# JoelTankard/web-rwkv-gguf

Hardware: AMD Instinct MI355X
Metric: tokens/sec RWKV-7 1.5B Q4_K_M decode @1 GPU; achieved HBM GB/s vs roofline (higher is better)
Workload: dtype f16; 1 GPU; RWKV-7 World 1.5B Q4_K_M (Q4_K matrices, Q6_K head, F16 LoRA) batch=1 greedy decode, fused kernels under hipGraph; decode_engine=on, streams_per_gpu=1, pipelines_per_gpu=1, streams=1, parallelism=single

## Files before the change

### include/wrk_hip.h

```cpp
#ifndef WRK_HIP_H
#define WRK_HIP_H

#include <stddef.h>
#include <stdint.h>

#ifdef __cplusplus
extern "C" {
#endif

#define WRK_ABI_VERSION 1

typedef struct wrk_ctx wrk_ctx;
typedef struct wrk_buf wrk_buf;
typedef struct wrk_matrix wrk_matrix;
typedef struct wrk_program wrk_program;
typedef struct wrk_v7_model wrk_v7_model;
typedef struct wrk_v7_state wrk_v7_state;

enum {
    WRK_OK = 0,
    WRK_E_ARG = 1,
    WRK_E_OOM = 2,
    WRK_E_HIP = 3,
    WRK_E_UNSUPPORTED = 4
// ... 90 lines not shown
int32_t wrk_op_activate(wrk_ctx* ctx, const wrk_tensor* x, uint32_t act);
int32_t wrk_op_control_k_v7(wrk_ctx* ctx, const wrk_buf* p, const wrk_tensor* a, const wrk_tensor* k);
int32_t wrk_op_time_mix_v7(wrk_ctx* ctx, const wrk_buf* cursors, const wrk_tensor* state, const wrk_tensor* r,
                           const wrk_tensor* w, const wrk_tensor* n, const wrk_tensor* x);
int32_t wrk_op_time_first_v7(wrk_ctx* ctx, const wrk_buf* u, const wrk_tensor* r, const wrk_tensor* n, const wrk_tensor* x);
int32_t wrk_op_channel_mix_v7(wrk_ctx* ctx, const wrk_buf* cursors, const wrk_tensor* state, const wrk_tensor* v, const wrk_tensor* x);
int32_t wrk_op_softmax(wrk_ctx* ctx, const wrk_tensor* x);


typedef struct wrk_v7_layer_desc {
    const wrk_buf *ln1_w, *ln1_b, *ln2_w, *ln2_b;
    const wrk_buf *x_r, *x_w, *x_k, *x_v, *x_a, *x_g;
    const wrk_buf *w0, *a0, *v0;
    const wrk_matrix *w1, *w2, *a1, *a2, *g1, *g2, *v1, *v2;
    const wrk_buf *r_k, *k_k, *k_a;
    const wrk_matrix *w_k, *w_v, *w_r, *w_o;
    const wrk_buf *gn_w, *gn_b;
    const wrk_buf* ffn_x_k;
    const wrk_matrix *ffn_w_k, *ffn_w_v;
} wrk_v7_layer_desc;

typedef struct wrk_v7_model_desc {
    uint32_t num_layer, num_emb, num_hidden, num_vocab, num_head;
    uint32_t lora_w, lora_a, lora_g, lora_v;
    uint32_t rescale;
    const wrk_buf *ln0_w, *ln0_b, *ln_out_w, *ln_out_b;
    const wrk_buf* emb_f16;
    const wrk_matrix* head;
    const wrk_v7_layer_desc* layers;
} wrk_v7_model_desc;

int32_t wrk_v7_model_create(wrk_ctx* ctx, const wrk_v7_model_desc* desc, wrk_v7_model** out);
int32_t wrk_v7_model_destroy(wrk_v7_model* model);
size_t wrk_v7_model_token_bytes(const wrk_v7_model* model, uint32_t num_batch);

int32_t wrk_v7_state_create(wrk_ctx* ctx, const wrk_v7_model* model, uint32_t num_batch, wrk_v7_state** out);
int32_t wrk_v7_state_destroy(wrk_v7_state* state);
int32_t wrk_v7_state_load(wrk_ctx* ctx, wrk_v7_state* state, uint32_t batch, const float* src);
int32_t wrk_v7_state_back(wrk_ctx* ctx, const wrk_v7_state* state, uint32_t batch, float* dst);
int32_t wrk_v7_state_read(wrk_ctx* ctx, const wrk_v7_state* state, uint32_t batch, wrk_buf* buf);
int32_t wrk_v7_state_write(wrk_ctx* ctx, wrk_v7_state* state, uint32_t batch, const wrk_buf* buf);

int32_t wrk_v7_infer(wrk_ctx* ctx, wrk_v7_model* model, wrk_v7_state* state,
                     const uint32_t* tokens, const uint16_t* emb_rows, const uint32_t* cursors, uint32_t num_token,
                     const uint32_t* headers, uint32_t num_header, float* logits, uint32_t* argmax, uint32_t mode);

int32_t wrk_v7_model_set_frame_dtype(wrk_ctx* ctx, wrk_v7_model* model, uint32_t dtype);

int32_t wrk_v7_model_engine_status(wrk_ctx* ctx, wrk_v7_model* model, char* why, size_t capacity);

int32_t wrk_v7_infer_layer(wrk_ctx* ctx, wrk_v7_model* model, wrk_v7_state* state, uint32_t layer, const void* x, const void* v_first,
                           const uint32_t* cursors, uint32_t num_token, uint32_t mode);
int32_t wrk_v7_frame_read(wrk_ctx* ctx, wrk_v7_model* model, const char* name, uint32_t num_token, void* dst, size_t capacity, size_t* bytes);

int32_t wrk_v7_generate_greedy(wrk_ctx* ctx, wrk_v7_model* model, wrk_v7_state* state,
                               const uint32_t* first_tokens, uint32_t num_batch, uint32_t steps,
                               uint32_t* out_tokens, float* last_logits_or_null, float* elapsed_ms_or_null, uint32_t mode);

int32_t wrk_sample_logits(wrk_ctx* ctx, const wrk_buf* logits, uint32_t num_vocab, uint32_t row_stride, uint32_t num_rows,
                          const float* temperature, const float* top_p, const uint32_t* seed, uint32_t step, uint32_t* out_tokens);
int32_t wrk_v7_generate_sample(wrk_ctx* ctx, wrk_v7_model* model, wrk_v7_state* state, const uint32_t* first_tokens, uint32_t num_batch,
                               uint32_t steps, const float* temperature, const float* top_p, const uint32_t* seed,
                               uint32_t* out_tokens, float* last_logits_or_null, float* elapsed_ms_or_null, uint32_t mode);
int32_t wrk_sample_logits_filtered(wrk_ctx* ctx, const wrk_buf* logits, uint32_t num_vocab, uint32_t row_stride, uint32_t num_rows,
                                   const float* temperature, const float* top_p, const uint32_t* top_k, const float* min_p,
                                   const uint32_t* seed, uint32_t step, uint32_t* out_tokens);
int32_t wrk_sample_logits_mirostat(wrk_ctx* ctx, const wrk_buf* logits, uint32_t num_vocab, uint32_t row_stride, uint32_t num_rows,
                                   const float* temperature, const float* top_p, const float* tau, const float* eta, float* mu_inout,
                                   const uint32_t* seed, uint32_t step, uint32_t* out_tokens);
int32_t wrk_sample_logits_typical(wrk_ctx* ctx, const wrk_buf* logits, uint32_t num_vocab, uint32_t row_stride, uint32_t num_rows,
                                  const float* temperature, const float* top_p, const float* typical_p, const uint32_t* seed,
                                  uint32_t step, uint32_t* out_tokens);

int32_t wrk_score_logits(wrk_ctx* ctx, const wrk_buf* logits, uint32_t num_vocab, uint32_t row_stride, uint32_t num_rows,
                         const uint32_t* targets, float* logprob, uint32_t* rank);
#define WRK_MAX_TOP_LOGPROBS 20
int32_t wrk_top_logprobs(wrk_ctx* ctx, const wrk_buf* logits, uint32_t num_vocab, uint32_t row_stride, uint32_t num_rows,
                         const uint32_t* tokens, uint32_t num_top, float* logprob, uint32_t* top_ids, float* top_logprobs);
int32_t wrk_v7_score(wrk_ctx* ctx, wrk_v7_model* model, wrk_v7_state* state,
                     const uint32_t* tokens, const uint16_t* emb_rows, const uint32_t* cursors, uint32_t num_token,
                     const uint32_t* headers, uint32_t num_header, const uint32_t* targets, float* logprob, uint32_t* rank, uint32_t mode);

typedef struct wrk_occurrence wrk_occurrence;
int32_t wrk_occurrence_create(wrk_ctx* ctx, uint32_t num_batch, uint32_t num_vocab, wrk_occurrence** out);
int32_t wrk_occurrence_destroy(wrk_occurrence* occ);
int32_t wrk_occurrence_set_weights(wrk_ctx* ctx, wrk_occurrence* occ, const float* weights);
int32_t wrk_occurrence_ban(wrk_ctx* ctx, wrk_occurrence* occ, uint32_t batch, const uint32_t* tokens, uint32_t n, int32_t banned);
int32_t wrk_occurrence_add(wrk_ctx* ctx, wrk_occurrence* occ, uint32_t batch, const uint32_t* tokens, uint32_t n, float decay);
int32_t wrk_occurrence_back(wrk_ctx* ctx, const wrk_occurrence* occ, uint32_t batch, float* counts, uint32_t* flags);
int32_t wrk_occurrence_load(wrk_ctx* ctx, wrk_occurrence* occ, uint32_t batch, const float* counts, const uint32_t* flags);
int32_t wrk_penalize_logits(wrk_ctx* ctx, wrk_buf* logits, uint32_t num_vocab, uint32_t row_stride, uint32_t num_rows,
                            const wrk_occurrence* occ, uint32_t first_batch, const float* presence, const float* frequency);
int32_t wrk_v7_generate_penalized(wrk_ctx* ctx, wrk_v7_model* model, wrk_v7_state* state, const uint32_t* first_tokens, uint32_t num_batch,
                                  uint32_t steps, const float* temperature, const float* top_p, const uint32_t* seed, const float* presence,
                                  const float* frequency, const float* decay, wrk_occurrence* occ, uint32_t* out_tokens,
                                  float* last_logits_or_null, float* elapsed_ms_or_null, uint32_t mode);

#define WRK_GRAMMAR_REJECT 0xFFFFu
#define WRK_MAX_TOKEN_CLASSES 8192
typedef struct wrk_grammar wrk_grammar;
int32_t wrk_grammar_create(wrk_ctx* ctx, uint32_t num_vocab, uint32_t num_states, uint32_t num_classes, const uint16_t* token_class,
                           const uint16_t* transitions, wrk_grammar** out);
int32_t wrk_grammar_destroy(wrk_grammar* grammar);
int32_t wrk_constrain_logits(wrk_ctx* ctx, wrk_buf* logits, uint32_t num_vocab, uint32_t row_stride, uint32_t num_rows,
                             const wrk_grammar* grammar, const uint32_t* states);
int32_t wrk_grammar_advance(wrk_ctx* ctx, const wrk_grammar* grammar, uint32_t* states, const uint32_t* tokens, uint32_t num_rows);
// ... 211 lines not shown
```

### web-rwkv-gguf_amd/csrc/wrk_device.h

```cpp
#pragma once
#include <hip/hip_runtime.h>
#include <stdint.h>

#include "wrk_internal.h"

typedef _Float16 f16;
typedef _Float16 f16x2 __attribute__((ext_vector_type(2)));
typedef _Float16 f16x8 __attribute__((ext_vector_type(8)));
typedef uint32_t u32x4 __attribute__((ext_vector_type(4)));
typedef uint32_t u32x2 __attribute__((ext_vector_type(2)));
typedef float f32x4 __attribute__((ext_vector_type(4)));
typedef float f32x2 __attribute__((ext_vector_type(2)));

#define WAVE 64

__device__ __forceinline__ float r16(float x) { return (float)(f16)x; }

__device__ __forceinline__ size_t dt_index(const DTensor& d, uint32_t c, uint32_t t, uint32_t b) {
    return ((size_t)(b + d.offset[2]) * d.stride[1] + (t + d.offset[1])) * d.stride[0] + c + d.offset[0];
}
__device__ __forceinline__ size_t dt_index4(const DTensor& d, uint32_t c, uint32_t t, uint32_t b, uint32_t w) {
    return (((size_t)(w + d.offset[3]) * d.stride[2] + (b + d.offset[2])) * d.stride[1] + (t + d.offset[1])) * d.stride[0] + c + d.offset[0];
}
__device__ __forceinline__ float dt_load(const DTensor& d, size_t i) {
// ... 6 lines not shown

struct Cursor { uint32_t batch, token, len; };
__device__ __forceinline__ Cursor unpack_cursor(uint32_t x) {
    Cursor c; c.batch = x & 0xffu; c.token = (x >> 8) & 0xffffu; c.len = (x >> 24) & 0xffu; return c;
}

__device__ __forceinline__ float act_sigmoid(float x) { return 1.0f / (1.0f + __expf(-x)); }
__device__ __forceinline__ float act_apply(uint32_t act, float x) {
    switch (act) {
        case WRK_ACT_SQUARED_RELU: { float p = fmaxf(x, 0.0f); return p * p; }
        case WRK_ACT_TANH: return x > 42.0f ? 1.0f : tanhf(x);
        case WRK_ACT_STABLE_EXP: return __expf(-__expf(x));
        case WRK_ACT_OPPOSITE_EXP: return -__expf(x);
        case WRK_ACT_SOFTPLUS: return __logf(1.0f + __expf(x));
        case WRK_ACT_SIGMOID: return act_sigmoid(x);
        case WRK_ACT_SILU: return x / (1.0f + __expf(-x));
        default: return x;
    }
}
__device__ __forceinline__ float wgsl_mix(float x, float y, float a) { return x * (1.0f - a) + y * a; }

template <int CTRL>
__device__ __forceinline__ float dpp_f32(float v) {
    return __builtin_bit_cast(float, __builtin_amdgcn_update_dpp(0, __builtin_bit_cast(int, v), CTRL, 0xf, 0xf, true));
}
__device__ __forceinline__ float wave_sum(float v) {
    v += dpp_f32<0xB1>(v);
    v += dpp_f32<0x4E>(v);
    v += dpp_f32<0x141>(v);
    v += dpp_f32<0x140>(v);
    const int b = __builtin_bit_cast(int, v);
    const float r0 = __builtin_bit_cast(float, __builtin_amdgcn_readlane(b, 0)), r1 = __builtin_bit_cast(float, __builtin_amdgcn_readlane(b, 16));
    const float r2 = __builtin_bit_cast(float, __builtin_amdgcn_readlane(b, 32)), r3 = __builtin_bit_cast(float, __builtin_amdgcn_readlane(b, 48));
    return (r0 + r1) + (r2 + r3);
}
__device__ __forceinline__ float wave_max(float v) {
#pragma unroll
    for (int o = 32; o > 0; o >>= 1) v = fmaxf(v, __shfl_xor(v, o, WAVE));
    return v;
}
template <int NW>
__device__ __forceinline__ float block_sum(float v, float* red) {
    v = wave_sum(v);
    const int wave = threadIdx.x >> 6, lane = threadIdx.x & 63;
    __syncthreads();
    if (lane == 0) red[wave] = v;
    __syncthreads();
    float t = 0.0f;
#pragma unroll
    for (int i = 0; i < NW; ++i) t += red[i];
    return t;
}

#ifdef WRK_TIMING_BUILD
#define WRK_STAMP(p, k)                                                                                       \
    do {                                                                                                      \
        __builtin_amdgcn_sched_barrier(0);                           \
        if ((p) && threadIdx.x == 0 && (blockIdx.x == 0 || blockIdx.x == gridDim.x - 1))                      \
            (p)[(blockIdx.x ? 8 : 0) + (k)] = wall_clock64();                                                 \
        __builtin_amdgcn_sched_barrier(0);                                                                    \
    } while (0)
#else
#define WRK_STAMP(p, k) do { } while (0)
#endif
```

### web-rwkv-gguf_amd/csrc/wrk_dmv.hip

```cpp
#include <cstdlib>

#include "wrk_dmv_body.h"

namespace wrk {

template <int KA, int KB, int XI, int KS>
static dmv_fn pick_dmv_pro(bool r16, int pro) {
#define DMV_P(PRO_) (r16 ? (dmv_fn)dmv_kernel<KA, KB, true, XI, KS, PRO_, 1> : (dmv_fn)dmv_kernel<KA, KB, false, XI, KS, PRO_, 1>)
    if (KS == 4 || pro == 0) return DMV_P(0);
    if (pro == 1) return DMV_P(1);
    if (pro == 2) return DMV_P(2);
    if (KA != KB) return nullptr;
    return pro == 3 ? DMV_P(3) : DMV_P(4);
#undef DMV_P
}

template <int XI, int KS>
static dmv_fn pick_dmv_kind(int ka, bool has_f16, bool r16, int pro) {
#define DMV_K(A)                                                                              \
    if (ka == A) return (has_f16 && KS == 1) ? pick_dmv_pro<A, WRK_MAT_F16, XI, KS>(r16, pro) : pick_dmv_pro<A, A, XI, KS>(r16, pro);
    DMV_K(WRK_MAT_Q4_K)
    DMV_K(WRK_MAT_Q5_K)
    DMV_K(WRK_MAT_Q6_K)
    DMV_K(WRK_MAT_Q8_0)
    DMV_K(WRK_MAT_INT8)
#undef DMV_K
    if (ka == WRK_MAT_F16) return pick_dmv_pro<WRK_MAT_F16, WRK_MAT_F16, XI, KS>(false, pro);
    return nullptr;
}

dmvt_fn pick_dmv_nt2(int ka, int quant2, bool has_f16, bool f16_only, uint32_t xi, int ks, int pro);
dmvt_fn pick_dmv_nt4(int ka, int quant2, bool has_f16, bool f16_only, uint32_t xi, int ks, int pro);
dmvt_fn pick_dmv_tokens(int nt, int ka, int quant2, bool has_f16, bool f16_only, uint32_t xi, int ks, int pro) {
    if (nt == 2) return pick_dmv_nt2(ka, quant2, has_f16, f16_only, xi, ks, pro);
    if (nt == 4) return pick_dmv_nt4(ka, quant2, has_f16, f16_only, xi, ks, pro);
    return nullptr;
}

int launch_dmv(hipStream_t s, const MatvecParams& P, uint32_t total_wg, int quant, bool has_f16, bool r16, bool dry, int quant2) {
    static const bool enabled = [] { const char* e = getenv("WRK_DMV"); return !(e && e[0] == '0'); }();
    if (!enabled) return -1;
    DParams D;
    DParamsT DT;
    uint32_t bounds[7], bmask = 0, xi = 1;
    int pro = -1;
    bool small_wg = true;
    for (int j = 0; j < 7; ++j) bounds[j] = 0xffffffffu;
    auto dense_base = [](const DTensor& t) { return ((size_t)t.offset[2] * t.stride[1] + t.offset[1]) * t.stride[0] + t.offset[0]; };
    auto dense_stack = [](const DTensor& t) { return t.shape[2] == 1 || (t.shape[1] == t.stride[1] && t.offset[1] == 0); };
    const uint32_t ntok = P.jobs[0].in.shape[1] * P.jobs[0].in.shape[2];
    if (ntok == 0 || ntok > 4) return -1;
    const int nt = ntok == 1 ? 1 : (ntok <= 2 ? 2 : 4);
    static const uint32_t max_tok = [] { const char* e = getenv("WRK_DMV_TOKENS"); const int v = e ? atoi(e) : 4; return (uint32_t)(v < 1 ? 1 : v); }();
    if (ntok > max_tok) return -1;
    if (nt > 1 && r16) return -1;
    for (int j = 0; j < P.njobs; ++j) {
        const JobDev& J = P.jobs[j];
        if (J.in.dtype != WRK_F16 || (J.k & 7u) || J.in.shape[1] * J.in.shape[2] != ntok || J.kind == WRK_MAT_NF4) return -1;
        if (nt > 1) {
            if (!dense_stack(J.in) || !dense_stack(J.out) || (J.has_res && !dense_stack(J.res)) || (J.in.stride[0] & 7u)) return -1;
            if (J.kind != WRK_MAT_F16 && J.kind != WRK_MAT_Q4_K && J.kind != WRK_MAT_Q5_K && J.kind != WRK_MAT_Q6_K) return -1;
        }
        if ((J.out.dtype != WRK_F16 && J.out.dtype != WRK_F32) || J.m == 0 || J.rows_per_wg == 0) return -1;
        const size_t ib = dense_base(J.in);
        if (ib & 7u) return -1;
        const int jp = J.pro ? (J.k <= 2048 ? 1 : (J.k <= 4096 ? 2 : 9)) + (J.pro == 2 ? 2 : 0) : 0;
        if (jp >= 9 || (pro >= 0 && jp != pro)) return -1;
        if (J.pro == 2 && (J.k & 63u)) return -1;
        pro = jp;
        if (J.rows_per_wg > 32) small_wg = false;
        const uint32_t kpad = (J.k + 15u) & ~15u;
        uint32_t nch, need;
        if (J.kind == WRK_MAT_F16) { nch = kpad >> 3; need = quant < 0 ? (nch + 63) / 64 : (nch + 255) / 256; bmask |= (quant < 0 ? 0u : 1u << j); }
        else { nch = (J.kind == WRK_MAT_Q8_0 || J.kind == WRK_MAT_INT8) ? (J.k >> 4) : (J.k >> 8) * 8; need = (nch + 63) / 64; }
        xi = need > xi ? need : xi;
        const size_t esz = J.out.dtype == WRK_F32 ? 4 : 2;
        if (J.has_res && J.res.dtype != WRK_F16 && J.res.dtype != WRK_F32) return -1;
        auto fill = [&](auto& d) {
            memset(&d, 0, sizeof d);
            d.w = J.w;
            d.x = (const f16*)J.in.p + ib;
            d.out = (char*)J.out.p + dense_base(J.out) * esz;
            d.flags = J.out.dtype == WRK_F32 ? DJ_OUT32 : 0u;
            if (J.has_res) {
                d.res = (const char*)J.res.p + dense_base(J.res) * (J.res.dtype == WRK_F32 ? 4 : 2);
                d.flags |= DJ_RES | (J.res.dtype == WRK_F32 ? DJ_RES32 : 0u);
            }
            if (J.carry_dst) { d.carry_src = J.carry_src; d.carry_dst = J.carry_dst; d.flags |= DJ_CARRY; }
            if (J.gate) { d.gate = J.gate; d.flags |= DJ_GATE; }
            if (J.amax_val) { d.amax_val = J.amax_val; d.amax_idx = J.amax_idx; d.flags |= DJ_AMAX; }
            if (J.pro) { d.ln_w = J.ln_w; d.ln_b = J.ln_b; d.mixw = J.mixw; d.prev = J.prev; d.ln_out = J.ln_out; d.eps = J.pro_eps; if (J.ln_out) d.flags |= DJ_PUBLISH; }
            d.dbg = J.dbg;
            d.k = J.k; d.m = J.m; d.row_bytes = J.row_bytes; d.rows_per_wg = J.rows_per_wg; d.wg_begin = J.wg_begin; d.act = J.act; d.kind = J.kind;
            d.scale = J.scale;
        };
        if (nt == 1) fill(D.jobs[j]);
        else {
            DJobT& dt = DT.jobs[j];
            fill(dt);
            dt.ntok = ntok; dt.xs = J.in.stride[0]; dt.os = J.out.stride[0]; dt.rs = J.has_res ? J.res.stride[0] : 0;
            dt.mix_s = J.tok_mix_stride; dt.prev_s = J.tok_prev_stride; dt.csrc_s = J.tok_carry_src_stride; dt.cdst_s = J.tok_carry_dst_stride; dt.gate_s = J.tok_gate_stride;
        }
        if (j > 0) bounds[j - 1] = J.wg_begin;
    }
    if (xi > 8) return -1;
    static const size_t max_bytes = [] { const char* e = getenv("WRK_DMV_MAXMB"); return (size_t)(e ? atoi(e) : 24) << 20; }();
    size_t launch_bytes = 0;
    for (int j = 0; j < P.njobs; ++j) launch_bytes += (size_t)P.jobs[j].m * P.jobs[j].row_bytes;
    if (nt == 1 && launch_bytes > max_bytes && xi > 1 && pro != 3 && pro != 4) return -1;
    dmv_fn fn = nullptr;
    const int ka = quant < 0 ? WRK_MAT_F16 : quant;
    const bool mixf = has_f16 && quant >= 0;
    if (nt > 1) {
        int ks = 1;
        uint32_t xk = xi;
        if (quant2 < 0 && !(quant < 0 && xi <= 4) && xi > 2) {
            bool amax = false;
            for (int j = 0; j < P.njobs; ++j) amax = amax || P.jobs[j].amax_val;
            if (mixf || !small_wg || pro != 0 || amax || xi > 8) return -1;
            ks = 4; xk = xi <= 4 ? 1 : 2;
        }
        const dmvt_fn ft = pick_dmv_tokens(nt, ka, quant2, mixf, quant < 0, xk, ks, pro);
        if (!ft) return -1;
        if (!dry) hipLaunchKernelGGL(ft, dim3(total_wg, 1), dim3(256), 0, s, bounds[0], bounds[1], bounds[2], bounds[3], bounds[4], bounds[5], bounds[6], bmask, DT);
        return 0;
    }
    else if (quant2 >= 0) {
        const int k4 = quant == WRK_MAT_Q6_K ? quant2 : quant;
        const int lnpro = xi == 1 ? 1 : 2;
        if ((quant != WRK_MAT_Q6_K && quant2 != WRK_MAT_Q6_K) || (k4 != WRK_MAT_Q4_K && k4 != WRK_MAT_Q5_K) || xi > 2 || (pro != 0 && pro != lnpro)) return -1;
#define DMV3X(A, X, PR) (r16 ? (dmv_fn)dmv3_kernel<A, true, X, PR, 1> : (dmv_fn)dmv3_kernel<A, false, X, PR, 1>)
#define DMV3(A) (xi == 1 ? (pro ? DMV3X(A, 1, 1) : DMV3X(A, 1, 0)) : (pro ? DMV3X(A, 2, 2) : DMV3X(A, 2, 0)))
        fn = k4 == WRK_MAT_Q4_K ? DMV3(WRK_MAT_Q4_K) : DMV3(WRK_MAT_Q5_K);
#undef DMV3
#undef DMV3X
    }
    else if (xi == 1) fn = pick_dmv_kind<1, 1>(ka, mixf, r16, pro);
    else if (xi == 2) fn = pick_dmv_kind<2, 1>(ka, mixf, r16, pro);
    else if (quant < 0 && xi <= 4) fn = pick_dmv_kind<4, 1>(ka, false, false, pro);
    else if (!mixf && small_wg && pro == 0) fn = xi <= 4 ? pick_dmv_kind<1, 4>(ka, false, r16, 0) : pick_dmv_kind<2, 4>(ka, false, r16, 0);
    if (!fn) return -1;
    if (!dry) hipLaunchKernelGGL(fn, dim3(total_wg, 1), dim3(256), 0, s, bounds[0], bounds[1], bounds[2], bounds[3], bounds[4], bounds[5], bounds[6], bmask, D);
    return 0;
}

}
```

### web-rwkv-gguf_amd/csrc/wrk_dmv_body.h

```cpp
#pragma once
#include "wrk_matvec_dev.h"

namespace wrk {

enum { DJ_RES = 1, DJ_RES32 = 2, DJ_CARRY = 4, DJ_GATE = 8, DJ_AMAX = 16, DJ_OUT32 = 32, DJ_PUBLISH = 64 };

#define WRK_DJOB_FIELDS                                                                                                          \
    const uint8_t* w;                                                                                                            \
    const f16* x;                                                                    \
    void* out;                                                       \
    const void* res;                                         \
    const f16* carry_src;                                \
    float* carry_dst;                                                                                                            \
    const f16* gate;                                                                       \
    const f16 *ln_w, *ln_b, *mixw;         \
    const float* prev;                                                                                 \
    f16* ln_out;                                      \
    float* amax_val;                                                                             \
    uint32_t* amax_idx;                                                                                                          \
    unsigned long long* dbg;                                                                                                     \
    uint32_t k, m, row_bytes, rows_per_wg, wg_begin, act, flags, kind;                                                           \
    float scale, eps;
struct DJob {
    WRK_DJOB_FIELDS
};
struct DJobT {
    WRK_DJOB_FIELDS
    uint32_t ntok, xs, os, rs, mix_s, prev_s, csrc_s, cdst_s, gate_s;
};

struct DParams {
    DJob jobs[MAX_JOBS];
};
struct DParamsT {
    DJobT jobs[MAX_JOBS];
};
template <int NT> struct DParamsOf { typedef DParamsT type; };
template <> struct DParamsOf<1> { typedef DParams type; };

template <class JT> struct TokF {
    static __device__ __forceinline__ uint32_t ntok(const JT&) { return 1u; }
    static __device__ __forceinline__ uint32_t xs(const JT&) { return 0u; }
    static __device__ __forceinline__ uint32_t os(const JT&) { return 0u; }
    static __device__ __forceinline__ uint32_t rs(const JT&) { return 0u; }
    static __device__ __forceinline__ uint32_t mix_s(const JT&) { return 0u; }
    static __device__ __forceinline__ uint32_t prev_s(const JT&) { return 0u; }
    static __device__ __forceinline__ uint32_t csrc_s(const JT&) { return 0u; }
    static __device__ __forceinline__ uint32_t cdst_s(const JT&) { return 0u; }
    static __device__ __forceinline__ uint32_t gate_s(const JT&) { return 0u; }
};
template <> struct TokF<DJobT> {
    static __device__ __forceinline__ uint32_t ntok(const DJobT& j) { return j.ntok; }
    static __device__ __forceinline__ uint32_t xs(const DJobT& j) { return j.xs; }
    static __device__ __forceinline__ uint32_t os(const DJobT& j) { return j.os; }
    static __device__ __forceinline__ uint32_t rs(const DJobT& j) { return j.rs; }
    static __device__ __forceinline__ uint32_t mix_s(const DJobT& j) { return j.mix_s; }
    static __device__ __forceinline__ uint32_t prev_s(const DJobT& j) { return j.prev_s; }
    static __device__ __forceinline__ uint32_t csrc_s(const DJobT& j) { return j.csrc_s; }
    static __device__ __forceinline__ uint32_t cdst_s(const DJobT& j) { return j.cdst_s; }
    static __device__ __forceinline__ uint32_t gate_s(const DJobT& j) { return j.gate_s; }
};

template <int KIND, bool R16, int NT, int XI>
__device__ __forceinline__ void dot_raw_tokens(const Raw& r, uint32_t c, const XRegs (&x)[NT][XI], int ci, float (&acc)[NT]) {
    if (KIND == WRK_MAT_F16) {
        const f16x8 wv = __builtin_bit_cast(f16x8, r.w);
#pragma unroll
        for (int t = 0; t < NT; ++t) {
            const f16x8 xv = x[t][ci].v[0];
            float a = 0.0f;
            a = __builtin_amdgcn_fdot2(__builtin_shufflevector(wv, wv, 0, 1), __builtin_shufflevector(xv, xv, 0, 1), a, false);
            a = __builtin_amdgcn_fdot2(__builtin_shufflevector(wv, wv, 2, 3), __builtin_shufflevector(xv, xv, 2, 3), a, false);
            a = __builtin_amdgcn_fdot2(__builtin_shufflevector(wv, wv, 4, 5), __builtin_shufflevector(xv, xv, 4, 5), a, false);
            a = __builtin_amdgcn_fdot2(__builtin_shufflevector(wv, wv, 6, 7), __builtin_shufflevector(xv, xv, 6, 7), a, false);
            acc[t] += a;
        }
        return;
    }
    constexpr bool TWO = KIND != WRK_MAT_Q8_0 && KIND != WRK_MAT_INT8;
    Group lo, hi;
    decode_raw<KIND>(r, c, lo, hi);
    if (R16) { round_group(lo); if (TWO) round_group(hi); }
#pragma unroll
    for (int t = 0; t < NT; ++t) {
        const XRegs& X = x[t][ci];
        float a;
        if (R16) a = dot16r(lo.q, X.v[0], X.v[1]);
        else a = lo.scale * (lo.qmul * dot16r(lo.q, X.v[0], X.v[1]) - lo.off * X.s[0]) - lo.minv * X.s[0];
        if (TWO) {
            if (R16) a += dot16r(hi.q, X.v[2], X.v[3]);
            else a += hi.scale * (hi.qmul * dot16r(hi.q, X.v[2], X.v[3]) - hi.off * X.s[1]) - hi.minv * X.s[1];
        }
        acc[t] += a;
    }
}

template <int KIND, bool R16, int XI, int KS, int PRO, int NT, class JT>
__device__ __forceinline__ void dmv_body(const JT J, unsigned char* smem) {
    typedef TokF<JT> TF;
    constexpr int RB = 4;
    constexpr uint32_t CSTEP = KS == 1 ? 64u : 256u;
    const uint32_t K = J.k, kpad = (K + 15u) & ~15u;
    const uint32_t tid = threadIdx.x, lane = tid & 63;
    const uint32_t wave = (uint32_t)__builtin_amdgcn_readfirstlane((int)(tid >> 6));
    const uint32_t r0 = (blockIdx.x - J.wg_begin) * J.rows_per_wg;
    const uint32_t r1 = min(r0 + J.rows_per_wg, J.m);
    const uint32_t nch = num_chunks<KIND>(K, kpad);
    const uint32_t nrows = KS == 1 ? (r0 + wave < r1 ? (r1 - r0 - wave + 3) >> 2 : 0) : (r1 - r0);
    const uint32_t cbase = KS == 1 ? lane : lane + 64 * wave;
    const uint32_t ntok = NT == 1 ? 1u : TF::ntok(J);
    auto row_of = [&](uint32_t ri) { return KS == 1 ? r0 + wave + 4 * ri : r0 + ri; };
    auto tok_of = [&](uint32_t t) { return NT == 1 ? 0u : min(t, ntok - 1); };
    const uint8_t* __restrict__ W = J.w;
    const uint32_t RBY = J.row_bytes;
    float* part = (float*)smem;
    float* sv = (float*)(smem + 512 * NT);
    uint32_t* si = (uint32_t*)(smem + 528 * NT);
    float* red = (float*)(smem + 544 * NT);
    f16* xs = (f16*)(smem + 576 * NT);

    Raw raw[RB][XI];
    auto issue = [&](uint32_t ri0) {
#pragma unroll
        for (int rb = 0; rb < RB; ++rb) {
            const uint32_t rr = min(row_of(ri0 + rb), r1 - 1);
            const uint32_t phase = KIND == WRK_MAT_INT8 ? (uint32_t)((((size_t)rr * K) >> 4) & 7u) : 0u;
            const uint8_t* rowp = W + (size_t)rr * RBY;
#pragma unroll
            for (int ci = 0; ci < XI; ++ci) raw[rb][ci] = load_raw<KIND>(rowp, K, min(cbase + CSTEP * ci, nch - 1), phase);
        }
    };
    WRK_STAMP(J.dbg, 0);

    const f16* __restrict__ xin = J.x;
    const uint32_t fin_row = min(KS == 1 ? row_of(lane & 3u) : r0 + (tid & 31u), r1 - 1);
    const uint32_t fin_t = NT == 1 ? 0u : (KS == 1 ? (lane >> 2) : (tid >> 5));
    const uint32_t fin_tok = tok_of(fin_t);
    const uint32_t fl = J.flags;
    uint32_t res_bits = 0, carry_bits = 0, gate_bits = 0;
    constexpr int VPT = PRO == 0 ? 1 : ((PRO - 1) % 2 + 1);
    constexpr bool GN = PRO >= 3;
    f16x8 xv[NT][VPT], wv[VPT], bv[VPT], mv[GN ? NT : 1][VPT];
    f32x4 pv[NT][VPT][2];
    f16 c0h[NT];
    XRegs x[NT][XI];
    if (PRO > 0) {
        const uint32_t nvec = K >> 3;
#pragma unroll
        for (int v = 0; v < VPT; ++v) {
            const uint32_t i = min(tid + 256u * v, nvec - 1);
            wv[v] = *(const f16x8*)(J.ln_w + i * 8);
            bv[v] = *(const f16x8*)(J.ln_b + i * 8);
#pragma unroll
            for (int t = 0; t < NT; ++t) {
                const uint32_t tt = tok_of(t);
                xv[t][v] = *(const f16x8*)(xin + (size_t)tt * TF::xs(J) + i * 8);
                if (GN || t == 0) mv[GN ? t : 0][v] = *(const f16x8*)(J.mixw + (size_t)tt * TF::mix_s(J) + i * 8);
                pv[t][v][0] = *(const f32x4*)(J.prev + (size_t)tt * TF::prev_s(J) + i * 8);
                pv[t][v][1] = *(const f32x4*)(J.prev + (size_t)tt * TF::prev_s(J) + i * 8 + 4);
            }
        }
        if (!GN) {
#pragma unroll
            for (int t = 0; t < NT; ++t) c0h[t] = xin[(size_t)tok_of(t) * TF::xs(J)];
        }
    } else {
#pragma unroll
        for (int t = 0; t < NT; ++t)
#pragma unroll
            for (int ci = 0; ci < XI; ++ci) x[t][ci] = load_x<KIND>(xin + (size_t)tok_of(t) * TF::xs(J), min(cbase + CSTEP * ci, nch - 1), true);
    }
    issue(0);
    {
        const bool has_res = (fl & DJ_RES) != 0, has_carry = (fl & DJ_CARRY) != 0, has_gate = (fl & DJ_GATE) != 0;
        const uint16_t* rp = has_res ? (const uint16_t*)J.res : (const uint16_t*)xin;
        const uint32_t re = fin_tok * TF::rs(J) + fin_row;
        const uint32_t ri = has_res ? ((fl & DJ_RES32) ? 2u * re : re) : 0u;
        if (fl & DJ_RES32) res_bits = *(const uint32_t*)(rp + ri);
        else res_bits = rp[ri];
        carry_bits = (has_carry ? (const uint16_t*)J.carry_src : (const uint16_t*)xin)[has_carry ? fin_tok * TF::csrc_s(J) + fin_row : 0u];
        gate_bits = (has_gate ? (const uint16_t*)J.gate : (const uint16_t*)xin)[has_gate ? fin_tok * TF::gate_s(J) + fin_row : 0u];
    }

    if (GN) {
        const uint32_t nvec = K >> 3;
#pragma unroll
        for (int t = 0; t < NT; ++t)
#pragma unroll
            for (int v = 0; v < VPT; ++v) {
                float y[8], s1 = 0.0f;
#pragma unroll
                for (int e = 0; e < 8; ++e) { y[e] = (float)xv[t][v][e]; s1 += y[e]; }
                s1 += dpp_f32<0xB1>(s1); s1 += dpp_f32<0x4E>(s1); s1 += dpp_f32<0x141>(s1);
                const float mean = s1 * (1.0f / 64.0f);
                float s2 = 0.0f;
#pragma unroll
                for (int e = 0; e < 8; ++e) { y[e] -= mean; s2 = __builtin_fmaf(y[e], y[e], s2); }
                s2 += dpp_f32<0xB1>(s2); s2 += dpp_f32<0x4E>(s2); s2 += dpp_f32<0x141>(s2);
                const float dev = 1.0f / sqrtf(s2 * (1.0f / 64.0f) + J.eps);
                f16x8 o;
#pragma unroll
                for (int e = 0; e < 8; ++e) {
                    float u = r16(__builtin_fmaf(y[e] * dev, (float)wv[v][e], (float)bv[v][e]));
                    u = r16(u + pv[t][v][e >> 2][e & 3]);
                    o[e] = (f16)((float)mv[GN ? t : 0][v][e] * u);
                }
                const uint32_t i = tid + 256u * v;
                if (i < nvec) *(f16x8*)(xs + (size_t)t * kpad + i * 8) = o;
            }
        for (uint32_t i = K + tid; i < kpad; i += 256)
#pragma unroll
            for (int t = 0; t < NT; ++t) xs[(size_t)t * kpad + i] = (f16)0.0f;
        __syncthreads();
#pragma unroll
        for (int t = 0; t < NT; ++t)
#pragma unroll
            for (int ci = 0; ci < XI; ++ci) x[t][ci] = load_x<KIND>(xs + (size_t)t * kpad, min(cbase + CSTEP * ci, nch - 1), true);
    }
    if (PRO > 0 && !GN) {
        const uint32_t nvec = K >> 3;
        float s1[NT], s2[NT];
#pragma unroll
        for (int t = 0; t < NT; ++t) {
            const float c0 = (float)c0h[t];
            s1[t] = 0.0f; s2[t] = 0.0f;
#pragma unroll
            for (int v = 0; v < VPT; ++v)
                if (tid + 256u * v < nvec)
#pragma unroll
                    for (int e = 0; e < 8; ++e) { const float dl = (float)xv[t][v][e] - c0; s1[t] += dl; s2[t] = __builtin_fmaf(dl, dl, s2[t]); }
            s1[t] = wave_sum(s1[t]);
            s2[t] = wave_sum(s2[t]);
            if (lane == 0) { red[8 * t + wave] = s1[t]; red[8 * t + 4 + wave] = s2[t]; }
        }
        __syncthreads();
        WRK_STAMP(J.dbg, 4);
        const bool publish = (fl & DJ_PUBLISH) && blockIdx.x == J.wg_begin;
#pragma unroll
        for (int t = 0; t < NT; ++t) {
            const float c0 = (float)c0h[t];
            const float a1 = (red[8 * t + 0] + red[8 * t + 1]) + (red[8 * t + 2] + red[8 * t + 3]);
            const float a2 = (red[8 * t + 4] + red[8 * t + 5]) + (red[8 * t + 6] + red[8 * t + 7]);
            const float md = a1 / (float)K;
            const float mean = c0 + md;
            const float dev = 1.0f / sqrtf(fmaxf(a2 / (float)K - md * md, 0.0f) + J.eps);
#pragma unroll
            for (int v = 0; v < VPT; ++v) {
                const uint32_t i = tid + 256u * v;
                if (i >= nvec) continue;
                f16x8 yv, o;
#pragma unroll
                for (int e = 0; e < 8; ++e) {
                    yv[e] = (f16)__builtin_fmaf(((float)xv[t][v][e] - mean) * dev, (float)wv[v][e], (float)bv[v][e]);
                    o[e] = (f16)wgsl_mix((float)yv[e], pv[t][v][e >> 2][e & 3], (float)mv[0][v][e]);
                }
                *(f16x8*)(xs + (size_t)t * kpad + i * 8) = o;
                if (publish && (uint32_t)t < ntok) *(f16x8*)(J.ln_out + (size_t)t * K + i * 8) = yv;
            }
        }
        for (uint32_t i = K + tid; i < kpad; i += 256)
#pragma unroll
            for (int t = 0; t < NT; ++t) xs[(size_t)t * kpad + i] = (f16)0.0f;
        __syncthreads();
#pragma unroll
        for (int t = 0; t < NT; ++t)
#pragma unroll
            for (int ci = 0; ci < XI; ++ci) x[t][ci] = load_x<KIND>(xs + (size_t)t * kpad, min(cbase + CSTEP * ci, nch - 1), true);
    }
#pragma unroll
    for (int ci = 0; ci < XI; ++ci)
        if (cbase + CSTEP * ci >= nch) {
            const f16x8 z = {0, 0, 0, 0, 0, 0, 0, 0};
// ... 31 lines not shown
#pragma unroll
            for (int t = 0; t < NT; ++t) acc[rb][t] = 0.0f;
#pragma unroll
            for (int ci = 0; ci < XI; ++ci) dot_raw_tokens<KIND, R16, NT, XI>(raw[rb][ci], min(cbase + CSTEP * ci, nch - 1), x, ci, acc[rb]);
        }
        WRK_STAMP(J.dbg, 2);
        float mine_v = 0.0f;
#pragma unroll
        for (int t = 0; t < NT; ++t)
#pragma unroll
            for (int rb = 0; rb < RB; ++rb) {
                const float v = wave_sum(acc[rb][t]);
                if (lane == (uint32_t)(rb + RB * t)) mine_v = v;
            }
        const uint32_t frb = lane & 3u;
        if (KS == 1) {
            if (lane < (uint32_t)(RB * NT) && (NT == 1 || fin_t < ntok) && ri0 + frb < nrows) {
                const uint32_t r = row_of(ri0 + frb);
                uint32_t rbits = res_bits, cbits = carry_bits, gbits = gate_bits;
                if (ri0 != 0) operand_bits(r, fin_t, rbits, cbits, gbits);
                finish(r, fin_t, mine_v, rbits, cbits, gbits);
            }
        } else if (lane < (uint32_t)(RB * NT) && ri0 + frb < nrows) part[(((NT == 1 ? 0u : lane >> 2) * 32u) + ri0 + frb) * 4 + wave] = mine_v;
    }
    if (KS == 4) {
        __syncthreads();
        const uint32_t ri = tid & 31u;
        if (NT == 1 ? tid < nrows : (ri < nrows && fin_t < ntok)) {
            const uint32_t p = NT == 1 ? tid : (fin_t * 32u + ri);
            finish(r0 + ri, fin_t, (part[p * 4] + part[p * 4 + 1]) + (part[p * 4 + 2] + part[p * 4 + 3]), res_bits, carry_bits, gate_bits);
        }
    }
    WRK_STAMP(J.dbg, 3);
    if (fl & DJ_AMAX) {
#pragma unroll
        for (int o = (KS == 1 ? 2 : 32); o > 0; o >>= 1) {
            const float ov = __shfl_xor(best_v, o, WAVE);
            const uint32_t oi = __shfl_xor(best_i, o, WAVE);
            if (ov > best_v || (ov == best_v && oi < best_i)) { best_v = ov; best_i = oi; }
        }
        if (KS == 1 ? ((lane & 3u) == 0 && lane < 4u * NT) : lane == 0) { sv[4 * (KS == 1 ? lane >> 2 : 0) + wave] = best_v; si[4 * (KS == 1 ? lane >> 2 : 0) + wave] = best_i; }
        __syncthreads();
        if (tid < ntok) {
            float bv2 = sv[4 * tid];
            uint32_t bi = si[4 * tid];
            for (int w = 1; w < 4; ++w)
                if (sv[4 * tid + w] > bv2 || (sv[4 * tid + w] == bv2 && si[4 * tid + w] < bi)) { bv2 = sv[4 * tid + w]; bi = si[4 * tid + w]; }
            J.amax_val[(size_t)(blockIdx.x - J.wg_begin) * ntok + tid] = bv2;
            J.amax_idx[(size_t)(blockIdx.x - J.wg_begin) * ntok + tid] = bi;
        }
    }
}

template <int PRO, int NT>
constexpr unsigned dmv_smem_bytes() { return 576u * NT + (PRO > 0 ? (unsigned)((PRO - 1) % 2 + 1) * 4096u * NT : 16u); }

template <int KA, int KB, bool R16, int XI, int KS, int PRO, int NT>
__global__ void __launch_bounds__(256) dmv_kernel(uint32_t b1, uint32_t b2, uint32_t b3, uint32_t b4, uint32_t b5, uint32_t b6, uint32_t b7,
                                                  uint32_t kind_b_mask, const typename DParamsOf<NT>::type P) {
    __shared__ __attribute__((aligned(16))) unsigned char smem[dmv_smem_bytes<PRO, NT>()];
    const uint32_t b = blockIdx.x;
    const uint32_t ji = (b >= b1) + (b >= b2) + (b >= b3) + (b >= b4) + (b >= b5) + (b >= b6) + (b >= b7);
    const auto J = P.jobs[ji];
    if (KA == KB || !((kind_b_mask >> ji) & 1u)) dmv_body<KA, (KA != WRK_MAT_F16) && R16, XI, KS, PRO, NT>(J, smem);
    else dmv_body<KB, (KB != WRK_MAT_F16) && R16, (KB == WRK_MAT_F16 ? 4 * XI : XI), 1, PRO, NT>(J, smem);
}

template <int KA, bool R16, int XI, int PRO, int NT>
__global__ void __launch_bounds__(256) dmv3_kernel(uint32_t b1, uint32_t b2, uint32_t b3, uint32_t b4, uint32_t b5, uint32_t b6, uint32_t b7,
                                                   uint32_t, const typename DParamsOf<NT>::type P) {
    __shared__ __attribute__((aligned(16))) unsigned char smem[dmv_smem_bytes<PRO, NT>()];
    const uint32_t b = blockIdx.x;
    const uint32_t ji = (b >= b1) + (b >= b2) + (b >= b3) + (b >= b4) + (b >= b5) + (b >= b6) + (b >= b7);
    const auto J = P.jobs[ji];
    if (J.kind == (uint32_t)KA) dmv_body<KA, R16, XI, 1, PRO, NT>(J, smem);
    else if (J.kind == WRK_MAT_Q6_K) dmv_body<WRK_MAT_Q6_K, R16, XI, 1, PRO, NT>(J, smem);
    else dmv_body<WRK_MAT_F16, false, 4 * XI, 1, PRO, NT>(J, smem);
}

typedef void (*dmv_fn)(uint32_t, uint32_t, uint32_t, uint32_t, uint32_t, uint32_t, uint32_t, uint32_t, const DParams);
typedef void (*dmvt_fn)(uint32_t, uint32_t, uint32_t, uint32_t, uint32_t, uint32_t, uint32_t, uint32_t, const DParamsT);

dmvt_fn pick_dmv_tokens(int nt, int ka, int quant2, bool has_f16, bool f16_only, uint32_t xi, int ks, int pro);

}
```

### web-rwkv-gguf_amd/csrc/wrk_matjob.h

```cpp
#pragma once
#include <stddef.h>
#include <stdint.h>

#include "wrk_hip.h"

struct DTensor {
    void* p;
    uint32_t dtype;
    uint32_t shape[4];
    uint32_t stride[4];
    uint32_t offset[4];
};

namespace wrk {

struct MatJob {
    const uint8_t* w;
    const uint8_t* aux;
    uint32_t kind, flags;
    uint32_t k, m;
    uint32_t row_bytes;
    DTensor in;
    DTensor out;
    uint32_t act;
    uint32_t sparse;
    uint32_t has_res = 0;
    DTensor res{};
    float* amax_val = nullptr;
    uint32_t* amax_idx = nullptr;
    uint32_t pro = 0;
    float pro_eps = 0.0f;
    const void *ln_w = nullptr, *ln_b = nullptr, *mixw = nullptr;
    const float* prev = nullptr;
    void* ln_out = nullptr;
    const void* carry_src = nullptr;
    float* carry_dst = nullptr;
    float scale = 1.0f;
    const void* gate = nullptr;
    unsigned long long* dbg = nullptr;
    uint32_t tok_prev_stride = 0, tok_mix_stride = 0, tok_carry_src_stride = 0, tok_carry_dst_stride = 0, tok_gate_stride = 0;
    float* ks_part = nullptr;
    uint32_t* ks_cnt = nullptr;
    size_t ks_part_cap = 0;
    uint32_t ks_cnt_cap = 0;
    void* xsum = nullptr;
    size_t xsum_cap = 0;
};

}
```

### web-rwkv-gguf_amd/csrc/wrk_matvec.hip

```cpp
#include <algorithm>
#include <cstdlib>

#include "wrk_matvec_dev.h"

namespace wrk {

static inline size_t align16(size_t x) { return (x + 15) & ~(size_t)15; }

uint32_t int8_row_blocks(uint32_t k) { return (k % 128) ? k / 128 + 2 : k / 128; }

size_t repack_row_bytes(uint32_t kind, uint32_t k) {
    const size_t nb = k / 256;
    switch (kind) {
        case WRK_MAT_F16: return align16((size_t)k * 2);
        case WRK_MAT_Q8_0: return align16((size_t)k + (size_t)(k / 32) * 2);
        case WRK_MAT_Q4_K: return align16(nb * 148);
        case WRK_MAT_Q5_K: return align16(nb * 180);
        case WRK_MAT_Q6_K: return align16(nb * 208 + nb * 2);
        case WRK_MAT_INT8: return (k % 16) ? 0 : align16((size_t)k + (size_t)int8_row_blocks(k) * 4);
        case WRK_MAT_NF4: return (k % 64) ? 0 : align16((size_t)k / 2 + (size_t)(k / 64) * 2);
        default: return 0;
    }
}

// ... 564 lines not shown
        const size_t base = ((size_t)J.in.offset[2] * J.in.stride[1] + J.in.offset[1]) * J.in.stride[0] + J.in.offset[0];
        if (base & 7u) return nullptr;
        const uint32_t kpad = (J.k + 15u) & ~15u;
        uint32_t nch, need;
        if (J.kind == WRK_MAT_F16) { nch = kpad >> 3; need = quant < 0 ? (nch + 63) / 64 : (nch + 255) / 256; }
        else if (J.kind == WRK_MAT_NF4) return nullptr;
        else { nch = (J.kind == WRK_MAT_Q8_0 || J.kind == WRK_MAT_INT8) ? (J.k >> 4) : (J.k >> 8) * 8; need = (nch + 63) / 64; }
        xi = need > xi ? need : xi;
    }
    if (xi > 8) return nullptr;
    bool small_wg = true;
    for (int j = 0; j < P.njobs; ++j) if (P.jobs[j].rows_per_wg > 32) small_wg = false;
    if (quant < 0) {
        if (xi == 1) return (matvec_fn)matvec_reg_kernel<WRK_MAT_F16, WRK_MAT_F16, false, 1, 1>;
        if (xi == 2) return (matvec_fn)matvec_reg_kernel<WRK_MAT_F16, WRK_MAT_F16, false, 2, 1>;
        if (xi <= 4) return (matvec_fn)matvec_reg_kernel<WRK_MAT_F16, WRK_MAT_F16, false, 4, 1>;
        return small_wg ? (matvec_fn)matvec_reg_kernel<WRK_MAT_F16, WRK_MAT_F16, false, 2, 4> : nullptr;
    }
    if (quant2 >= 0) {
        const int ka = quant == WRK_MAT_Q6_K ? quant2 : quant;
        if ((quant != WRK_MAT_Q6_K && quant2 != WRK_MAT_Q6_K) || (ka != WRK_MAT_Q4_K && ka != WRK_MAT_Q5_K) || xi > 2) return nullptr;
        if (ka == WRK_MAT_Q4_K) {
            if (xi == 1) return r16 ? (matvec_fn)matvec_reg3_kernel<WRK_MAT_Q4_K, true, 1> : (matvec_fn)matvec_reg3_kernel<WRK_MAT_Q4_K, false, 1>;
            return r16 ? (matvec_fn)matvec_reg3_kernel<WRK_MAT_Q4_K, true, 2> : (matvec_fn)matvec_reg3_kernel<WRK_MAT_Q4_K, false, 2>;
        }
        if (xi == 1) return r16 ? (matvec_fn)matvec_reg3_kernel<WRK_MAT_Q5_K, true, 1> : (matvec_fn)matvec_reg3_kernel<WRK_MAT_Q5_K, false, 1>;
        return r16 ? (matvec_fn)matvec_reg3_kernel<WRK_MAT_Q5_K, true, 2> : (matvec_fn)matvec_reg3_kernel<WRK_MAT_Q5_K, false, 2>;
    }
    const int kb = has_f16 ? WRK_MAT_F16 : quant;
    if (xi == 1) return pick_reg_kernel<1, 1>(quant, kb, r16);
    if (xi == 2) return pick_reg_kernel<2, 1>(quant, kb, r16);
    if (has_f16 || !small_wg) return nullptr;
    if (xi <= 4) return pick_reg_kernel<1, 4>(quant, quant, r16);
    return pick_reg_kernel<2, 4>(quant, quant, r16);
}

struct KindMix { int quant = -1, quant2 = -1, nquant = 0; bool has_f16 = false, r16 = false, mixed_r16 = false; };
static KindMix classify_kinds(const MatvecParams& P) {
    KindMix c;
    for (int j = 0; j < P.njobs; ++j) {
        const int k = (int)P.jobs[j].kind;
        if (k == WRK_MAT_F16) { c.has_f16 = true; continue; }
        const bool jr = (P.jobs[j].flags & WRK_MATRIX_ROUND_F16) != 0;
        if (c.nquant == 0) { c.quant = k; c.r16 = jr; c.nquant = 1; }
        else {
            if (k != c.quant && k != c.quant2) { c.quant2 = c.quant2 < 0 ? k : c.quant2; c.nquant = (k == c.quant2) ? 2 : 3; }
            if (jr != c.r16) c.mixed_r16 = true;
        }
    }
    return c;
}

template <int NB>
static int launch_matvec(hipStream_t s, const MatvecParams& P, uint32_t total_wg, uint32_t tok_groups, size_t smem, bool dry, bool no_catchall) {
    const KindMix c = classify_kinds(P);
    const int quant = c.quant, quant2 = c.quant2, nquant = c.nquant;
    const bool has_f16 = c.has_f16, r16 = c.r16, mixed_r16 = c.mixed_r16;
    matvec_fn fn = nullptr;
    bool needs_reg = false;
    for (int j = 0; j < P.njobs; ++j) needs_reg = needs_reg || P.jobs[j].pro || P.jobs[j].carry_dst || P.jobs[j].gate;
    if (NB == 1 && tok_groups == 1 && nquant <= 2 && !mixed_r16 && launch_dmv(s, P, total_wg, nquant ? quant : -1, has_f16, r16, dry, nquant == 2 ? quant2 : -1) == 0) return 0;
    if (NB == 1 && tok_groups == 1 && nquant <= 2 && !mixed_r16) {
        fn = pick_reg(P, nquant ? quant : -1, has_f16, r16, nquant == 2 ? quant2 : -1);
        if (fn) {
            if (!dry) hipLaunchKernelGGL(fn, dim3(total_wg, 1), dim3(256), 0, s, P);
            return 0;
        }
    }
    if (needs_reg) return -3;
    if (no_catchall && (nquant >= 2 || mixed_r16)) return -4;
    if (dry) return 0;
    if (nquant >= 2 || mixed_r16) fn = (matvec_fn)matvec_kernel<NB, -1, -1, false>;
    else if (nquant == 0) fn = pick_kernel<NB>(WRK_MAT_F16, WRK_MAT_F16, false);
    else fn = pick_kernel<NB>(quant, has_f16 ? WRK_MAT_F16 : quant, r16);
    if (smem > 64 * 1024) {
        if (hipFuncSetAttribute((const void*)fn, hipFuncAttributeMaxDynamicSharedMemorySize, (int)smem) != hipSuccess) return -1;
    }
    hipLaunchKernelGGL(fn, dim3(total_wg, tok_groups), dim3(256), smem, s, P);
    return 0;
}

static uint32_t matvec_job_rpw(const MatJob* jobs, int njobs, int j, uint32_t rpw) {
    uint32_t min_rb = jobs[0].row_bytes;
    for (int q = 1; q < njobs; ++q) min_rb = jobs[q].row_bytes < min_rb ? jobs[q].row_bytes : min_rb;
    uint32_t r = (uint32_t)((uint64_t)rpw * min_rb / (jobs[j].row_bytes ? jobs[j].row_bytes : 1)) & ~3u;
    return r < 4 ? 4 : r;
}

uint32_t matvec_num_wg(const MatJob* jobs, int njobs, int num_cu, uint32_t* rows_per_wg) {
    uint32_t total_rows = 0;
    for (int j = 0; j < njobs; ++j) total_rows += jobs[j].m;
    static const uint32_t per_cu = [] { const char* e = getenv("WRK_WG_PER_CU"); const int v = e ? atoi(e) : 4; return (uint32_t)(v < 1 ? 1 : (v > 16 ? 16 : v)); }();
    uint32_t rpw = (total_rows + (uint32_t)num_cu * per_cu - 1) / ((uint32_t)num_cu * per_cu);
    rpw = (rpw + 3) & ~3u;
    static const uint32_t rpw_min = [] { const char* e = getenv("WRK_RPW_MIN"); const int v = e ? atoi(e) : 4; return (uint32_t)(v < 4 ? 4 : (v > 32 ? 32 : v)) & ~3u; }();
    rpw = rpw < rpw_min ? rpw_min : (rpw > 32 ? 32 : rpw);
    static const uint32_t pro_rpw = [] { const char* e = getenv("WRK_PRO_RPW"); const int v = e ? atoi(e) : 16; return (uint32_t)(v < 4 ? 4 : (v > 32 ? 32 : v)) & ~3u; }();
    for (int j = 0; j < njobs; ++j)
        if (jobs[j].pro && rpw < pro_rpw) rpw = pro_rpw;
    uint32_t wg = 0;
    for (int j = 0; j < njobs; ++j) { const uint32_t r = matvec_job_rpw(jobs, njobs, j, rpw); wg += (jobs[j].m + r - 1) / r; }
    if (rows_per_wg) *rows_per_wg = rpw;
    return wg;
}

int matvec(hipStream_t s, const MatJob* jobs, int njobs, int num_cu, bool dry_run, bool no_catchall, bool dmv_only) {
    if (njobs <= 0 || njobs > MAX_JOBS) return -1;
    MatvecParams P;
    P.njobs = njobs;
    const uint32_t ntok = jobs[0].in.shape[1] * jobs[0].in.shape[2];
    if (ntok == 0) return 0;
    uint32_t kmax = 0;
    for (int j = 0; j < njobs; ++j) {
        if (jobs[j].in.shape[1] * jobs[j].in.shape[2] != ntok) return -1;
        kmax = jobs[j].k > kmax ? jobs[j].k : kmax;
    }
    uint32_t rpw = 4;
    matvec_num_wg(jobs, njobs, num_cu, &rpw);
    uint32_t wg = 0;
    for (int j = 0; j < njobs; ++j) {
        JobDev& d = P.jobs[j];
        d.w = jobs[j].w; d.aux = (const float*)jobs[j].aux; d.kind = jobs[j].kind; d.flags = jobs[j].flags; d.k = jobs[j].k; d.m = jobs[j].m;
        d.row_bytes = jobs[j].row_bytes; d.act = jobs[j].act; d.rows_per_wg = matvec_job_rpw(jobs, njobs, j, rpw); d.wg_begin = wg;
        d.in = jobs[j].in; d.out = jobs[j].out; d.res = jobs[j].res; d.has_res = jobs[j].has_res;
        d.amax_val = jobs[j].amax_val; d.amax_idx = jobs[j].amax_idx;
        d.pro = jobs[j].pro; d.pro_eps = jobs[j].pro_eps; d.ln_w = (const f16*)jobs[j].ln_w; d.ln_b = (const f16*)jobs[j].ln_b;
        d.mixw = (const f16*)jobs[j].mixw; d.prev = jobs[j].prev; d.ln_out = (f16*)jobs[j].ln_out;
        d.carry_src = (const f16*)jobs[j].carry_src; d.carry_dst = jobs[j].carry_dst; d.gate = (const f16*)jobs[j].gate; d.scale = jobs[j].scale; d.dbg = jobs[j].dbg;
        d.tok_prev_stride = jobs[j].tok_prev_stride; d.tok_mix_stride = jobs[j].tok_mix_stride; d.tok_carry_src_stride = jobs[j].tok_carry_src_stride;
        d.tok_carry_dst_stride = jobs[j].tok_carry_dst_stride; d.tok_gate_stride = jobs[j].tok_gate_stride;
        wg += (jobs[j].m + d.rows_per_wg - 1) / d.rows_per_wg;
    }
    bool f32in = false;
    for (int j = 0; j < njobs; ++j) f32in = f32in || jobs[j].in.dtype == WRK_F32;
    if (f32in) {
        for (int j = 0; j < njobs; ++j)
            if (jobs[j].pro || jobs[j].carry_dst || jobs[j].gate || jobs[j].amax_val) return -3;
        if (dry_run) return 0;
        hipLaunchKernelGGL(matvec_f32in_kernel, dim3(wg, ntok), dim3(256), 0, s, P);
        return 0;
    }
    if (ntok >= 2 && ntok <= 4) {
        const KindMix c = classify_kinds(P);
        if (c.nquant <= 2 && !c.mixed_r16 && launch_dmv(s, P, wg, c.nquant ? c.quant : -1, c.has_f16, c.r16, dry_run, c.nquant == 2 ? c.quant2 : -1) == 0) return 0;
    }
    if (dmv_only && ntok > 1) return -5;
    const uint32_t kpad = (kmax + 15u) & ~15u;
    int nb = ntok >= 8 ? 8 : (ntok >= 4 ? 4 : (ntok >= 2 ? 2 : 1));
    while (nb > 1 && (size_t)nb * kpad * 2 + (size_t)nb * (kpad >> 4) * 4 > 144 * 1024) nb >>= 1;
    size_t smem = (size_t)nb * kpad * 2 + (size_t)nb * (kpad >> 4) * 4 + 64;
    if (smem < 256) smem = 256;
    const uint32_t groups = (ntok + nb - 1) / nb;
    int rc;
    switch (nb) {
        case 8: rc = launch_matvec<8>(s, P, wg, groups, smem, dry_run, no_catchall); break;
        case 4: rc = launch_matvec<4>(s, P, wg, groups, smem, dry_run, no_catchall); break;
        case 2: rc = launch_matvec<2>(s, P, wg, groups, smem, dry_run, no_catchall); break;
        default: rc = launch_matvec<1>(s, P, wg, groups, smem, dry_run, no_catchall); break;
    }
    return rc;
}

int matvec_grouped(hipStream_t s, const MatJob* jobs, int njobs, int num_cu, bool dry_run) {
    if (njobs <= 0 || njobs > MAX_JOBS) return -1;
    uint32_t kinds[MAX_JOBS];
    int nk = 0;
    for (int j = 0; j < njobs; ++j) {
        if (jobs[j].kind == WRK_MAT_F16) continue;
        bool seen = false;
        for (int q = 0; q < nk; ++q) seen = seen || kinds[q] == jobs[j].kind;
        if (!seen) kinds[nk++] = jobs[j].kind;
    }
    if (nk <= 1) return matvec(s, jobs, njobs, num_cu, dry_run);
    {
        const int rc = matvec(s, jobs, njobs, num_cu, dry_run, true);
        if (rc == 0) return 0;
    }
    for (int q = 0; q < nk; ++q) {
        MatJob g[MAX_JOBS];
        int n = 0;
        for (int j = 0; j < njobs; ++j)
            if (jobs[j].kind == kinds[q] || (q == 0 && jobs[j].kind == WRK_MAT_F16)) g[n++] = jobs[j];
        const int rc = matvec(s, g, n, num_cu, dry_run);
        if (rc != 0) return rc;
    }
    return 0;
}

}
```

### web-rwkv-gguf_amd/csrc/wrk_matvec_dev.h

```cpp
#pragma once
#include "wrk_device.h"

namespace wrk {

__device__ __forceinline__ void bytes_to_h2(uint32_t v, f16x2& lo, f16x2& hi) {
    lo = __builtin_bit_cast(f16x2, __builtin_amdgcn_perm(0u, v, 0x0c010c00u));
    hi = __builtin_bit_cast(f16x2, __builtin_amdgcn_perm(0u, v, 0x0c030c02u));
}

__device__ __forceinline__ f16x2 h2(float a) { f16x2 r = {(f16)a, (f16)a}; return r; }

__device__ __forceinline__ float dot16(const f16x2 (&q)[8], const f16* __restrict__ x) {
    const f16x8 xa = *(const f16x8*)x;
    const f16x8 xb = *(const f16x8*)(x + 8);
    float acc = 0.0f;
    acc = __builtin_amdgcn_fdot2(q[0], __builtin_shufflevector(xa, xa, 0, 1), acc, false);
    acc = __builtin_amdgcn_fdot2(q[1], __builtin_shufflevector(xa, xa, 2, 3), acc, false);
    acc = __builtin_amdgcn_fdot2(q[2], __builtin_shufflevector(xa, xa, 4, 5), acc, false);
    acc = __builtin_amdgcn_fdot2(q[3], __builtin_shufflevector(xa, xa, 6, 7), acc, false);
    acc = __builtin_amdgcn_fdot2(q[4], __builtin_shufflevector(xb, xb, 0, 1), acc, false);
    acc = __builtin_amdgcn_fdot2(q[5], __builtin_shufflevector(xb, xb, 2, 3), acc, false);
    acc = __builtin_amdgcn_fdot2(q[6], __builtin_shufflevector(xb, xb, 4, 5), acc, false);
    acc = __builtin_amdgcn_fdot2(q[7], __builtin_shufflevector(xb, xb, 6, 7), acc, false);
    return acc;
// ... 274 lines not shown
    r.v[0] = *(const f16x8*)(x + lo);
    if (KIND != WRK_MAT_F16) r.v[1] = *(const f16x8*)(x + lo + 8);
    if (KIND != WRK_MAT_F16 && KIND != WRK_MAT_Q8_0 && KIND != WRK_MAT_INT8) { r.v[2] = *(const f16x8*)(x + hi); r.v[3] = *(const f16x8*)(x + hi + 8); }
    return r;
}

template <int KIND>
__device__ __forceinline__ void x_sums(XRegs& r) {
    if (KIND != WRK_MAT_F16) r.s[0] = sum8(r.v[0]) + sum8(r.v[1]);
    if (KIND != WRK_MAT_F16 && KIND != WRK_MAT_Q8_0 && KIND != WRK_MAT_INT8) r.s[1] = sum8(r.v[2]) + sum8(r.v[3]);
}

__device__ __forceinline__ float dot16r(const f16x2 (&q)[8], const f16x8 xa, const f16x8 xb) {
    float acc = 0.0f;
    acc = __builtin_amdgcn_fdot2(q[0], __builtin_shufflevector(xa, xa, 0, 1), acc, false);
    acc = __builtin_amdgcn_fdot2(q[1], __builtin_shufflevector(xa, xa, 2, 3), acc, false);
    acc = __builtin_amdgcn_fdot2(q[2], __builtin_shufflevector(xa, xa, 4, 5), acc, false);
    acc = __builtin_amdgcn_fdot2(q[3], __builtin_shufflevector(xa, xa, 6, 7), acc, false);
    acc = __builtin_amdgcn_fdot2(q[4], __builtin_shufflevector(xb, xb, 0, 1), acc, false);
    acc = __builtin_amdgcn_fdot2(q[5], __builtin_shufflevector(xb, xb, 2, 3), acc, false);
    acc = __builtin_amdgcn_fdot2(q[6], __builtin_shufflevector(xb, xb, 4, 5), acc, false);
    acc = __builtin_amdgcn_fdot2(q[7], __builtin_shufflevector(xb, xb, 6, 7), acc, false);
    return acc;
}

template <bool R16>
__device__ __forceinline__ float group_dot_r(Group& g, const f16x8 xa, const f16x8 xb, float xs16) {
    if (R16) {
        round_group(g);
        return dot16r(g.q, xa, xb);
    }
    return g.scale * (g.qmul * dot16r(g.q, xa, xb) - g.off * xs16) - g.minv * xs16;
}

template <int KIND, bool R16>
__device__ __forceinline__ float dot_raw_reg(const Raw& r, uint32_t c, const XRegs& x) {
    if (KIND == WRK_MAT_F16) {
        const f16x8 wv = __builtin_bit_cast(f16x8, r.w);
        float a = 0.0f;
        a = __builtin_amdgcn_fdot2(__builtin_shufflevector(wv, wv, 0, 1), __builtin_shufflevector(x.v[0], x.v[0], 0, 1), a, false);
        a = __builtin_amdgcn_fdot2(__builtin_shufflevector(wv, wv, 2, 3), __builtin_shufflevector(x.v[0], x.v[0], 2, 3), a, false);
        a = __builtin_amdgcn_fdot2(__builtin_shufflevector(wv, wv, 4, 5), __builtin_shufflevector(x.v[0], x.v[0], 4, 5), a, false);
        a = __builtin_amdgcn_fdot2(__builtin_shufflevector(wv, wv, 6, 7), __builtin_shufflevector(x.v[0], x.v[0], 6, 7), a, false);
        return a;
    }
    Group lo, hi;
    decode_raw<KIND>(r, c, lo, hi);
    float a = group_dot_r<R16>(lo, x.v[0], x.v[1], x.s[0]);
    if (KIND != WRK_MAT_Q8_0 && KIND != WRK_MAT_INT8) a += group_dot_r<R16>(hi, x.v[2], x.v[3], x.s[1]);
    return a;
}


int launch_dmv(hipStream_t s, const MatvecParams& P, uint32_t total_wg, int quant, bool has_f16, bool r16, bool dry, int quant2 = -1);

}
```

### web-rwkv-gguf_amd/csrc/wrk_v7.h

```cpp
#pragma once
#include <string>
#include <vector>

#include "wrk_runner.h"

struct V7Scratch : wrk::FrameIo {
    void *input, *x, *att_x, *att_v0, *rx, *wx, *kx, *vx, *ax, *gx, *r, *w, *k, *v, *a, *g, *o, *kk, *vv, *n;
    void *aux_w, *aux_a, *aux_g, *aux_v, *ffn_x, *ffn_kx, *ffn_k, *ffn_v, *ln_tmp, *head_x;
    float* ks_part; uint32_t* ks_cnt; size_t ks_part_cap; uint32_t ks_cnt_cap;
};

struct wrk_v7_model : wrk_frame_common {
    wrk_v7_model_desc d{};
    std::vector<wrk_v7_layer_desc> layers;
    const wrk_buf *ln0_w = nullptr, *ln0_b = nullptr, *ln_out_w = nullptr, *ln_out_b = nullptr, *emb = nullptr;
    const wrk_matrix* head = nullptr;

    V7Scratch s{};

    float* amax_val = nullptr;
    uint32_t* amax_idx = nullptr;
    size_t amax_cap = 0;

    uint32_t layer_begin = 0, layer_end = 0xffffffffu;
    bool skip_embed = false;
    uint32_t act_dtype = WRK_F16;

    std::vector<wrk_v7_model*> lanes;

    struct wrk_v7_engine* engine = nullptr;
    bool engine_tried = false;
    bool engine_skip_once = false;
    bool engine_blocked = false;
    std::string engine_why;
    int32_t ensure_engine();
    bool engine_on() const;
    Facts facts() const override { return {d.num_vocab, d.num_emb, d.num_layer, emb != nullptr}; }
    wrk::FrameIo& io() override { return s; }
    int32_t ensure_frame(uint32_t B, uint32_t mode) override;
    int32_t enqueue_step(wrk_v7_state* st, uint32_t b0, uint32_t B, uint32_t mode, wrk_step_kind kind) override;
    uint32_t key_bits(uint32_t B, uint32_t mode) const override;
    uint32_t max_lanes() const override { return 255; }
    int32_t lane(uint32_t g, uint32_t groups, wrk_frame_common** out) override;
    void before_loop() override;
    int32_t after_loop(uint32_t groups) override;
    int32_t ensure_scratch(uint32_t T, uint32_t NH);
    int32_t enqueue_ops(wrk_v7_state* st, uint32_t T, uint32_t NH, bool identity_headers, bool merged = false);
    int32_t enqueue_fused_decode(wrk_v7_state* st, uint32_t B, uint32_t NH, bool identity_headers, bool from_tokens,
                                 bool want_argmax, bool advance, uint32_t cursor0_batch, bool contiguous);
    void free_fused();
};

bool split_head_env_on();
bool engine_env_on_public();
```

### web-rwkv-gguf_amd/csrc/wrk_v7.hip

```cpp
#include "wrk_internal.h"
#include "wrk_v7.h"
#include "wrk_v7_engine.h"

#define LOCK(ctx) std::lock_guard<std::recursive_mutex> _lk((ctx)->mu)

static constexpr float LN_EPS = 1.0e-5f;
static constexpr float GN_EPS = 64.0e-5f;
static constexpr float L2_EPS = 1.0e-12f;

using wrk::mat_job;

int32_t wrk_v7_model::ensure_scratch(uint32_t T, uint32_t NH) {
    if (T <= scratch_tokens && NH <= scratch_headers && scratch) return WRK_OK;
    if (ctx->capturing_here()) return wrk_fail(ctx, WRK_E_ARG, "scratch must be sized before capture");
    const uint32_t nt = T > scratch_tokens ? T : scratch_tokens;
    const uint32_t nh = NH > scratch_headers ? NH : scratch_headers;
    WRK_HIP(ctx, hipStreamSynchronize(ctx->stream));
    drop_graphs();
    if (scratch) hipFree(scratch);
    scratch = nullptr;
    const size_t D = d.num_emb, F = d.num_hidden, V = d.num_vocab;
    size_t off = 0;
    auto take = [&](size_t bytes) { size_t o = off; off += wrk_up256(bytes); return o; };
    const size_t esz = act_dtype == WRK_F32 ? 4 : 2;
// ... 479 lines not shown
    const int32_t rc = m->ensure_engine();
    if (rc != WRK_OK) return rc;
    if (why && capacity) {
        const std::string w = m->engine ? std::to_string(wrk_v7_engine_waves(m->engine)) + " compute waves"
                                        : (m->engine_tried ? m->engine_why : std::string("disabled (WRK_ENGINE=0 or f32 frames)"));
        snprintf(why, capacity, "%s", w.c_str());
    }
    return m->engine ? 1 : 0;
}

int32_t wrk_v7_infer_layer(wrk_ctx* ctx, wrk_v7_model* m, wrk_v7_state* st, uint32_t layer, const void* x, const void* v_first,
                           const uint32_t* cursors, uint32_t T, uint32_t mode) {
    if (!ctx || !m || !st || !x || !cursors) return WRK_E_ARG;
    LOCK(ctx);
    WRK_HIP(ctx, hipSetDevice(ctx->device));
    WRK_ARG(ctx, !ctx->capturing_here(), "wrk_v7_infer_layer cannot be captured");
    WRK_ARG(ctx, layer < m->d.num_layer, "layer %u out of range", layer);
    WRK_ARG(ctx, T >= 1, "no tokens");
    WRK_ARG(ctx, layer == 0 || v_first, "layers above 0 read the layer-0 value (att_v0)");
    WRK_ARG(ctx, st->num_emb == m->d.num_emb && st->num_layer == m->d.num_layer, "state does not belong to this model");
    wrk_job_shape sh;
    int32_t rc = wrk_job_check(ctx, st, cursors, T, nullptr, 0, nullptr, 0, &sh);
    if (rc == WRK_OK) rc = m->ensure_scratch(T, 1);
    if (rc == WRK_OK && T == 1 && mode == 1) rc = m->ensure_engine();
    if (rc != WRK_OK) return rc;
    const size_t esz = m->act_dtype == WRK_F32 ? 4 : 2;
    rc = wrk_buf_write_raw(ctx, m->s.cursors, cursors, (size_t)T * 4);
    if (rc == WRK_OK) rc = wrk_buf_write_raw(ctx, m->s.x, x, (size_t)T * m->d.num_emb * esz);
    if (rc == WRK_OK && v_first) rc = wrk_buf_write_raw(ctx, m->s.att_v0, v_first, (size_t)T * m->d.num_emb * esz);
    if (rc != WRK_OK) return rc;
    m->layer_begin = layer; m->layer_end = layer + 1; m->skip_embed = true;
    m->wkv_nseq = sh.nseq;
    { const char* ei = getenv("WRK_ENGINE_INSPECT"); m->engine_skip_once = !(ei && ei[0] == '1'); }
    if (mode == 1 && sh.one_token_each && sh.nseq == T && m->act_dtype == WRK_F16) rc = m->enqueue_fused_decode(st, T, 0, true, false, false, false, cursors[0] & 0xff, sh.contiguous);
    else rc = m->enqueue_ops(st, T, 0, true, mode == 1);
    m->layer_begin = 0; m->layer_end = 0xffffffffu; m->skip_embed = false; m->engine_skip_once = false;
    if (rc != WRK_OK) return rc;
    WRK_LAUNCH_CHECK(ctx);
    WRK_HIP(ctx, hipStreamSynchronize(ctx->stream));
    return wrk_v7_engine_check(m->engine);
}

int32_t wrk_v7_frame_read(wrk_ctx* ctx, wrk_v7_model* m, const char* name, uint32_t T, void* dst, size_t capacity, size_t* bytes) {
    if (!ctx || !m || !name || !bytes) return WRK_E_ARG;
    LOCK(ctx);
    WRK_ARG(ctx, m->scratch && T >= 1 && T <= m->scratch_tokens, "no frame of %u tokens has been run", T);
    const uint32_t D = m->d.num_emb, F = m->d.num_hidden;
    const V7Scratch& s = m->s;
    struct { const char* n; const void* p; uint32_t c; } tab[] = {
        {"x", s.x, D}, {"att_x", s.att_x, D}, {"att_v0", s.att_v0, D}, {"att_rx", s.rx, D}, {"att_wx", s.wx, D}, {"att_kx", s.kx, D},
        {"att_vx", s.vx, D}, {"att_ax", s.ax, D}, {"att_gx", s.gx, D}, {"att_r", s.r, D}, {"att_w", s.w, D}, {"att_k", s.k, D}, {"att_v", s.v, D},
        {"att_a", s.a, D}, {"att_g", s.g, D}, {"att_o", s.o, D}, {"att_kk", s.kk, D}, {"att_vv", s.vv, D}, {"att_n", s.n, 4 * D},
        {"aux_w", s.aux_w, m->d.lora_w}, {"aux_a", s.aux_a, m->d.lora_a}, {"aux_g", s.aux_g, m->d.lora_g}, {"aux_v", s.aux_v, m->d.lora_v},
        {"ffn_x", s.ffn_x, D}, {"ffn_kx", s.ffn_kx, D}, {"ffn_k", s.ffn_k, F}, {"ffn_v", s.ffn_v, D}, {"att_x_ln", s.ln_tmp, D}};
    const size_t esz = m->act_dtype == WRK_F32 ? 4 : 2;
    for (auto& e : tab)
        if (strcmp(e.n, name) == 0) {
            const size_t n = (size_t)e.c * T * esz;
            *bytes = n;
            if (!dst) return WRK_OK;
            WRK_ARG(ctx, capacity >= n, "frame buffer %s needs %zu bytes, capacity %zu", name, n, capacity);
            WRK_HIP(ctx, hipSetDevice(ctx->device));
            WRK_HIP(ctx, hipMemcpyAsync(dst, e.p, n, hipMemcpyDeviceToHost, ctx->stream));
            WRK_HIP(ctx, hipStreamSynchronize(ctx->stream));
            return WRK_OK;
        }
    return wrk_fail(ctx, WRK_E_ARG, "no frame buffer named %s", name);
}

}

int32_t wrk_v7_model::enqueue_step(wrk_v7_state* st, uint32_t b0, uint32_t B, uint32_t mode, wrk_step_kind kind) {
    int32_t rc;
    const bool fused = mode == 1 && act_dtype == WRK_F16, head_picks = fused && !kind.sampled() && !kind.constrained && !kind.dry && !kind.biased && kind.tail != wrk_step_kind::BEAM,
               head_advances = head_picks && kind.tail == wrk_step_kind::PLAIN && !kind.logprobs;
    if (fused) rc = enqueue_fused_decode(st, B, B, true, true, head_picks, head_advances, b0, true);
    else {
        wrk::gather_rows_f16(ctx->op_stream(), emb->ptr, s.tokens, s.input, d.num_emb, B);
        rc = enqueue_ops(st, B, B, true);
    }
    if (rc != WRK_OK || head_advances) return rc;
    return wrk_enqueue_pick(*this, B, kind, st, b0, head_picks);
}

int32_t wrk_v7_model::ensure_frame(uint32_t B, uint32_t mode) {
    const int32_t rc = ensure_scratch(B, B);
    return rc == WRK_OK && B == 1 && mode == 1 ? ensure_engine() : rc;
}

uint32_t wrk_v7_model::key_bits(uint32_t B, uint32_t mode) const {
    return mode | (act_dtype == WRK_F32 ? 4u : 0u) | ((B == 1 && mode == 1 && engine_on()) ? 8u : 0u) | (split_head_env_on() ? 0u : 16u);
}

int32_t wrk_v7_model::lane(uint32_t g, uint32_t groups, wrk_frame_common** out) {
    while (lanes.size() + 1 < groups) {
        wrk_v7_model* clone = nullptr;
        const int32_t rc = wrk_v7_model_create(ctx, &d, &clone);
        if (rc != WRK_OK) return rc;
        clone->act_dtype = act_dtype;
        lanes.push_back(clone);
    }
    while (lane_streams.size() < groups) {
        hipStream_t ls = nullptr;
        hipEvent_t e = nullptr;
        WRK_HIP(ctx, hipStreamCreateWithFlags(&ls, hipStreamNonBlocking));
        WRK_HIP(ctx, hipEventCreateWithFlags(&e, hipEventDisableTiming));
        lane_streams.push_back(ls);
        lane_events.push_back(e);
    }
    wrk_v7_model* mdl = g == 0 ? this : lanes[g - 1];
    mdl->engine_blocked = groups > 1;
    *out = mdl;
    return WRK_OK;
}

void wrk_v7_model::before_loop() { wrk::timing_slot(ctx, nullptr); }

int32_t wrk_v7_model::after_loop(uint32_t groups) {
    wrk::timing_report(ctx);
    for (uint32_t g = 0; g < groups; ++g) {
        wrk_v7_engine* e = (g == 0 ? this : lanes[g - 1])->engine;
        wrk_v7_engine_report(e);
        const int32_t rc = wrk_v7_engine_check(e);
        if (rc != WRK_OK) return rc;
    }
    return WRK_OK;
}

extern "C" {

int32_t wrk_v7_generate_greedy(wrk_ctx* ctx, wrk_v7_model* m, wrk_v7_state* st, const uint32_t* first_tokens, uint32_t B,
                               uint32_t steps, uint32_t* out_tokens, float* last_logits, float* elapsed_ms, uint32_t mode_arg) {
    return wrk_generate(ctx, m, st, first_tokens, B, steps, wrk_pick_args{}, out_tokens, last_logits, elapsed_ms, mode_arg);
}

int32_t wrk_v7_generate_sample(wrk_ctx* ctx, wrk_v7_model* m, wrk_v7_state* st, const uint32_t* first_tokens, uint32_t B, uint32_t steps,
                               const float* temperature, const float* top_p, const uint32_t* seed, uint32_t* out_tokens, float* last_logits,
                               float* elapsed_ms, uint32_t mode_arg) {
    wrk_pick_args pick{temperature, top_p, seed};
    pick.need = wrk_pick_args::SAMPLER;
    return wrk_generate(ctx, m, st, first_tokens, B, steps, pick, out_tokens, last_logits, elapsed_ms, mode_arg);
}

int32_t wrk_v7_generate_penalized(wrk_ctx* ctx, wrk_v7_model* m, wrk_v7_state* st, const uint32_t* first_tokens, uint32_t B, uint32_t steps,
                                  const float* temperature, const float* top_p, const uint32_t* seed, const float* presence,
                                  const float* frequency, const float* decay, wrk_occurrence* occ, uint32_t* out_tokens, float* last_logits,
                                  float* elapsed_ms, uint32_t mode_arg) {
    wrk_pick_args pick{temperature, top_p, seed, presence, frequency, decay, occ};
    pick.need = wrk_pick_args::TABLE;
    return wrk_generate(ctx, m, st, first_tokens, B, steps, pick, out_tokens, last_logits, elapsed_ms, mode_arg);
}

int32_t wrk_v7_generate_stop(wrk_ctx* ctx, wrk_v7_model* m, wrk_v7_state* st, const uint32_t* first_tokens, uint32_t B, uint32_t steps,
                             const wrk_generate_options* opt, uint32_t* out_tokens, uint32_t* out_lengths, float* last_logits,
                             uint32_t* steps_run, float* elapsed_ms, uint32_t mode_arg) {
    const wrk_stop_call stop{opt, out_lengths, steps_run};
    return wrk_generate(ctx, m, st, first_tokens, B, steps, opt ? wrk_pick_of(*opt) : wrk_pick_args{}, out_tokens, last_logits, elapsed_ms, mode_arg, &stop);
}

int32_t wrk_v7_generate_queue(wrk_ctx* ctx, wrk_v7_model* m, wrk_v7_state* st, uint32_t B, const wrk_queue_options* opt,
                              const wrk_queue_result* out_arg, float* elapsed_ms, uint32_t mode_arg) {
    return wrk_generate_queue(ctx, m, st, B, opt, out_arg, elapsed_ms, mode_arg, wrk_step_kind::QUEUE, nullptr);
}

int32_t wrk_v7_generate_queue_pool(wrk_ctx* ctx, wrk_v7_model* m, wrk_v7_state* st, uint32_t B, const wrk_queue_options* opt,
                                   const wrk_queue_result* out_arg, float* elapsed_ms, uint32_t mode_arg, const wrk_queue_pool* pool) {
    return wrk_generate_queue(ctx, m, st, B, opt, out_arg, elapsed_ms, mode_arg, wrk_step_kind::QUEUE_POOL, pool);
}

int32_t wrk_v7_generate_beam(wrk_ctx* ctx, wrk_v7_model* m, wrk_v7_state* st, const uint32_t* first_tokens, uint32_t G, uint32_t steps,
                             const wrk_beam_options* opt, const wrk_beam_result* out_arg, float* elapsed_ms, uint32_t mode_arg) {
    return wrk_generate_beam(ctx, m, st, first_tokens, G, steps, opt, out_arg, elapsed_ms, mode_arg);
}

}

static bool engine_env_on() { const char* e = getenv("WRK_ENGINE"); return !(e && e[0] == '0'); }
bool engine_env_on_public() { return engine_env_on(); }
bool wrk_v7_model::engine_on() const { return engine != nullptr && !engine_blocked && engine_env_on() && act_dtype == WRK_F16; }
int32_t wrk_v7_model::ensure_engine() {
    if (engine_tried || !engine_env_on() || act_dtype != WRK_F16) return WRK_OK;
    if (ctx->capturing_here()) return WRK_OK;
    engine_tried = true;
    const std::string keep = ctx->err;
    const int32_t rc = wrk_v7_engine_create(this, &engine);
    if (rc != WRK_OK) { engine = nullptr; engine_why = ctx->err; ctx->err = keep; }
    if (rc != WRK_OK && rc != WRK_E_UNSUPPORTED) return rc;
    return WRK_OK;
}
```

### web-rwkv-gguf_amd/csrc/wrk_v7_engine.h

```cpp
#pragma once
#include <stdint.h>

#include "wrk_internal.h"
#include "wrk_lora2_pack.h"

namespace wrk {

constexpr int ENG_K1_JOBS = 7;
constexpr uint32_t ENG_NO_HEAD = 0xffffffffu;

struct EngJob {
    uint32_t rows, row_bytes, f16;
    uint32_t act, mix;
    uint32_t wg0, nwg, rows_per_wg;
    uint32_t gbase;
    uint32_t headed;
};

struct EngShape {
    uint32_t D, F, H, nwg;
    uint32_t rw, ra, rg, rv;
    uint32_t rb_d, rb_f;
    EngJob k1[ENG_K1_JOBS];
    uint32_t k3_rpw, k5_rpw, k6_rpw;
    uint32_t lds_slot1, lds_slot5, lds_slot6, lds_slot3, lds_xraw0, lds_xraw1, lds_xs, lds_ln, lds_misc, lds_total;
    uint32_t g_x, g_k1, g_o, g_x1, g_k, g_total, g_aux;
    float ln_eps, gn_eps, l2_eps;
    uint32_t layer_begin, layer_end, rescale;
    uint32_t batch, state_rows;
    uint32_t x_from_granules;
};

struct EngLayer {
    const uint8_t *w_r, *w_k, *w_v, *w1, *a1, *g1, *v1;
    const uint8_t *w_o, *ffn_k, *ffn_v;
};
enum { ENG_V_LN1W, ENG_V_LN1B, ENG_V_LN2W, ENG_V_LN2B, ENG_V_MIX0, ENG_V_W0 = ENG_V_MIX0 + 6, ENG_V_A0, ENG_V_V0, ENG_V_RK, ENG_V_KK, ENG_V_KA,
       ENG_V_GNW, ENG_V_GNB, ENG_V_FFNXK, ENG_NV };
enum { ENG_S_O = ENG_K1_JOBS, ENG_S_FK, ENG_S_FV, ENG_NS = 16 };

struct EngArgs {
    EngShape S;
    const EngLayer* layers;
    const void* vecs;
    const uint8_t* l2;
    const float* scal;
    unsigned long long* gran;
    const void* x_in;
    const uint32_t* x_row;
    void* x_out;
    void* v_first;
    float* state;
    uint32_t num_batch;
    uint32_t* fail;
    unsigned long long* stamps;
    uint32_t stamp_layer;
};
constexpr int ENG_STAMPS = 32;

constexpr __host__ __device__ uint32_t eng_wave_pairs(uint32_t pairs, uint32_t ncw, uint32_t wave) {
    const uint32_t simd_rank = (wave + 4u - (ncw + 2u) % 4u) % 4u;
    return pairs / ncw + ((wave / 4u) * 4u + simd_rank < pairs % ncw ? 1u : 0u);
}
constexpr __host__ __device__ uint32_t eng_wave_first_pair(uint32_t pairs, uint32_t ncw, uint32_t wave) {
    const uint32_t extra = pairs % ncw, g4 = (wave / 4u) * 4u;
    uint32_t first = wave * (pairs / ncw) + (extra < g4 ? extra : g4);
    for (uint32_t w = g4; w < wave; ++w) first += eng_wave_pairs(pairs, ncw, w) - pairs / ncw;
    return first;
}
constexpr __host__ __device__ void eng_wave_rows(uint32_t nrows, uint32_t ncw, uint32_t wave, uint32_t& begin, uint32_t& end) {
    const uint32_t pairs = (nrows + 1u) / 2u;
    const uint32_t first = eng_wave_first_pair(pairs, ncw, wave), last = first + eng_wave_pairs(pairs, ncw, wave);
    begin = 2u * first < nrows ? 2u * first : nrows;
    end = 2u * last < nrows ? 2u * last : nrows;
}
constexpr bool eng_wave_rows_ok(uint32_t ncw) {
    for (uint32_t nrows = 0; nrows <= 128; nrows += 2) {
        const uint32_t pairs = nrows / 2, most = (pairs + ncw - 1) / ncw;
        uint32_t next = 0, simd[4] = {0, 0, 0, 0};
        for (uint32_t w = 0; w < ncw; ++w) {
            uint32_t b = 0, e = 0;
            eng_wave_rows(nrows, ncw, w, b, e);
            if (b != next || e < b || (b & 1u) || (e & 1u) || (e - b) / 2 > most || (e - b) / 2 < pairs / ncw) return false;
            simd[w % 4] += (e - b) / 2 - pairs / ncw;
            next = e;
        }
        if (next != nrows) return false;
        const uint32_t s0 = (ncw + 2) % 4;
        for (uint32_t i = 0; i + 1 < 4; ++i) {
            const uint32_t a = simd[(s0 + i) % 4], c = simd[(s0 + i + 1) % 4];
            if (c > a || simd[s0] - simd[(s0 + 3) % 4] > 1) return false;
        }
    }
    return true;
}
static_assert(eng_wave_rows_ok(8) && eng_wave_rows_ok(14), "a row pair without exactly one owner wave, or an uneven schedule");

}

struct wrk_v7_model;
struct wrk_v7_state;
struct wrk_v7_engine;
int32_t wrk_v7_engine_create(wrk_v7_model* m, wrk_v7_engine** out);
void wrk_v7_engine_destroy(wrk_v7_engine* e);
int32_t wrk_v7_engine_enqueue(wrk_v7_engine* e, hipStream_t q, wrk_v7_state* st, uint32_t batch, uint32_t l0, uint32_t l1, const void* x_in,
                              void* x_out, void* v_first, const uint32_t* token = nullptr);
bool wrk_v7_engine_has_table(const wrk_v7_engine* e);
int wrk_v7_engine_waves(const wrk_v7_engine* e);
int32_t wrk_v7_engine_check(wrk_v7_engine* e);
void wrk_v7_engine_report(wrk_v7_engine* e);
```

### web-rwkv-gguf_amd/csrc/wrk_v7_engine.hip

```cpp
#include "wrk_device.h"
#include "wrk_v7.h"
#include "wrk_dmv_body.h"
#include "wrk_v7_engine.h"
#include "wrk_lora_dev.h"

#include <algorithm>
#include <string>

namespace wrk {

#define ENG_LDS __attribute__((address_space(3)))
typedef ENG_LDS unsigned char lds_u8;

#define ENG_BAR() asm volatile("s_waitcnt lgkmcnt(0)\n\ts_barrier" ::: "memory")

constexpr uint32_t ENG_SPIN_MAX = 1u << 21;

__device__ __forceinline__ uint32_t eng_tag(uint32_t layer, uint32_t stage) { return layer * 8u + stage + 1u; }

__device__ __forceinline__ void eng_store_granule(unsigned long long* g, uint32_t tag, uint32_t payload) {
    __hip_atomic_store(g, ((unsigned long long)tag << 32) | payload, __ATOMIC_RELAXED, __HIP_MEMORY_SCOPE_AGENT);
}
__device__ __forceinline__ uint32_t pack_h2(float a, float b) {
    const f16x2 h = {(f16)a, (f16)b};
// ... 739 lines not shown
#pragma unroll
                    for (int rb = 0; rb < 4; ++rb) {
                        float acc[1] = {0.0f};
#pragma unroll
                        for (int ci = 0; ci < XD; ++ci) dot_raw_tokens<QK, R16, 1, XD>(raw[rb][ci], min(cbase + 256u * ci, nch - 1), x, ci, acc);
                        const float pvs = wave_sum(acc[0]);
                        if (lane == 0 && ri + rb < g_e) part[(ri + rb) * 4 + kq] = pvs;
                    }
                }
        }
        ENG_STAMP0(l, 12);
        ENG_BAR();
        if (wave == 0) {
            const bool valid = lane < k6_rows;
            const uint32_t r = k6_row0 + min(lane, k6_rows ? k6_rows - 1 : 0u);
            float o = 0.0f;
            if (k6_rows) {
                const uint32_t p = min(lane, k6_rows - 1);
                o = ((part[p * 4] + part[p * 4 + 1]) + (part[p * 4 + 2] + part[p * 4 + 3])) * sc_fv;
                o = r16(o) + (float)xraw1[r];
                if ((l + 1) % S.rescale == 0) o = r16(o) * 0.5f;
            }
            const float o_next = __shfl_down(o, 1, WAVE);
            if (valid) {
                lst[(size_t)(srows - 1) * D + r] = (float)lnbuf[r];
                if ((lane & 1u) == 0) eng_store_granule(A.gran + S.g_x + (r >> 1), eng_tag(l, 4), pack_h2(o, o_next));
                if (l + 1 == S.layer_end) ((f16*)A.x_out)[r] = (f16)o;
            }
        }
        ENG_STAMP0(l, 13);
        ENG_BAR();
        ENG_FLUSH(l);
    }
    if (A.stamps && wg == 0 && tid_all == 0) {
        unsigned long long* tail = A.stamps + (size_t)S.nwg * 16 * 24;
        tail[0] = __builtin_amdgcn_s_memtime() - clk0;
        tail[1] = __builtin_amdgcn_s_memrealtime() - rt0;
    }
#undef ENG_STAMP
#undef ENG_STAMP0
#undef ENG_FLUSH
}

}

struct wrk_v7_engine {
    wrk_v7_model* m = nullptr;
    wrk::EngShape S{};
    wrk::EngLayer* layers = nullptr;
    void* vecs = nullptr;
    float* scal = nullptr;
    uint32_t* wg_head = nullptr;
    unsigned long long* gran = nullptr;
    uint32_t* fail = nullptr;
    unsigned long long* stamps = nullptr;
    uint8_t* l2pack = nullptr;
    void* emb_ln = nullptr;
    bool r16 = false;
    int xd = 1, ncw = 8;
    uint32_t quant = 0;
};

static uint32_t up(uint32_t v, uint32_t a) { return (v + a - 1) / a * a; }

typedef void (*eng_fn)(const wrk::EngArgs, const uint32_t*);
static eng_fn eng_kernel(int xd, bool r16, int ncw) {
    using namespace wrk;
#define ENG_PICK(XD_, R_) (ncw == 14 ? (eng_fn)v7_engine_kernel<XD_, R_, WRK_MAT_Q4_K, 14> : (eng_fn)v7_engine_kernel<XD_, R_, WRK_MAT_Q4_K, 8>)
    if (xd == 1) return r16 ? ENG_PICK(1, true) : ENG_PICK(1, false);
    return r16 ? ENG_PICK(2, true) : ENG_PICK(2, false);
#undef ENG_PICK
}
static const void* eng_kernel_fn(int xd, bool r16, int ncw) { return (const void*)eng_kernel(xd, r16, ncw); }

int32_t wrk_v7_engine_create(wrk_v7_model* m, wrk_v7_engine** out) {
    using namespace wrk;
    wrk_ctx* ctx = m->ctx;
    *out = nullptr;
    const auto& d = m->d;
    const uint32_t D = d.num_emb, F = d.num_hidden, H = d.num_head, NWG = (uint32_t)ctx->num_cu;
    auto no = [&](const char* why) { return wrk_fail(ctx, WRK_E_UNSUPPORTED, "decode engine: %s", why); };
    if (m->act_dtype != WRK_F16) return no("f32 frames");
    if (H == 0 || D != H * 64 || D % 256 || D > 4096 || F % 1024 || F != 4 * D) return no("shape");
    if (d.lora_w % 8 || d.lora_a % 8 || d.lora_g % 8 || d.lora_v % 8 || d.lora_w < 8 || d.lora_a < 8 || d.lora_g < 8 || d.lora_v < 8 ||
        d.lora_w > 128 || d.lora_a > 128 || d.lora_v > 128 || d.lora_g > 256 || ((d.lora_w + d.lora_a + d.lora_g + d.lora_v) % 16))
        return no("LoRA ranks");
    if (NWG < 2 * H || NWG < 64) return no("too few compute units");
    uint32_t quant = 0xffffffffu, flags = 0xffffffffu;
    for (size_t li = 0; li < m->layers.size(); ++li) {
        const auto& L = m->layers[li];
        const wrk_matrix* big[] = {L.w_r, L.w_k, L.w_v, L.w_o, L.ffn_w_k, L.ffn_w_v};
        for (const wrk_matrix* q : big) {
            if (quant == 0xffffffffu) { quant = q->kind; flags = q->flags; }
            if (q->kind != quant || q->flags != flags) return no("mixed matrix kinds");
        }
        const wrk_matrix* lo[] = {L.w1, L.a1, L.g1, li ? L.v1 : L.a1, L.w2, L.a2, L.g2, li ? L.v2 : L.a2};
        for (const wrk_matrix* q : lo)
            if (!q || q->kind != WRK_MAT_F16) return no("LoRA matrices must be F16");
        if (L.w_r->k != D || L.w_r->m != D || L.ffn_w_k->m != F || L.ffn_w_v->k != F || L.w1->m != d.lora_w || L.a1->m != d.lora_a ||
            L.g1->m != d.lora_g || (li && L.v1->m != d.lora_v) || L.w2->k != d.lora_w || L.a2->k != d.lora_a || L.g2->k != d.lora_g ||
            (li && L.v2->k != d.lora_v) || L.w2->m != D || L.a2->m != D || L.g2->m != D || (li && L.v2->m != D))
            return no("matrix shapes");
    }
    if (quant != WRK_MAT_Q4_K) return no("only Q4_K matrices so far");
    if (m->layers.empty()) return no("no layers");

// ... 90 lines not shown
        o.w_o = L.w_o->data; o.ffn_k = L.ffn_w_k->data; o.ffn_v = L.ffn_w_v->data;
        const wrk_matrix* k1m[ENG_K1_JOBS] = {L.w_r, L.w_k, L.w_v, L.w1, L.a1, L.g1, li ? L.v1 : L.a1};
        float* sc = hs.data() + li * ENG_NS;
        for (int j = 0; j < ENG_K1_JOBS; ++j) sc[j] = k1m[j]->out_scale;
        sc[ENG_S_O] = L.w_o->out_scale; sc[ENG_S_FK] = L.ffn_w_k->out_scale; sc[ENG_S_FV] = L.ffn_w_v->out_scale;
    }
    if ((er = hipMalloc((void**)&e->vecs, hl.size() * ENG_NV * D * 2)) != hipSuccess) return fail_alloc(er);
    for (size_t li = 0; li < m->layers.size(); ++li) {
        const auto& L = m->layers[li];
        const wrk_buf* src[ENG_NV] = {L.ln1_w, L.ln1_b, L.ln2_w, L.ln2_b, L.x_r, L.x_w, L.x_k, L.x_v, L.x_a, L.x_g, L.w0, L.a0, li ? L.v0 : L.w0,
                                      L.r_k, L.k_k, L.k_a, L.gn_w, L.gn_b, L.ffn_x_k};
        for (int i = 0; i < ENG_NV; ++i) {
            if (!src[i] || src[i]->bytes < (size_t)D * 2) { wrk_v7_engine_destroy(e); return no("a layer vector is missing"); }
            if ((er = hipMemcpy((char*)e->vecs + (li * ENG_NV + i) * (size_t)D * 2, src[i]->ptr, (size_t)D * 2, hipMemcpyDeviceToDevice)) != hipSuccess) return fail_alloc(er);
        }
    }
    {
        const EngLora2Ranks R2{S.rw, S.ra, S.rg, S.rv};
        const size_t lb = eng_l2_layer_bytes(R2, H), total_l2 = lb * m->layers.size();
        if ((er = hipMalloc((void**)&e->l2pack, total_l2)) != hipSuccess) {
            (void)hipGetLastError();
            wrk_v7_engine_destroy(e);
            return wrk_fail(ctx, WRK_E_UNSUPPORTED, "decode engine: %zu bytes for the packed LoRA up-projections refused (%s)", total_l2, hipGetErrorString(er));
        }
        std::vector<uint8_t> img(lb), rows[4];
        for (size_t li = 0; li < m->layers.size(); ++li) {
            const auto& L = m->layers[li];
            const wrk_matrix* mats[4] = {L.w2, L.a2, L.g2, li ? L.v2 : nullptr};
            const uint8_t* src[4] = {nullptr, nullptr, nullptr, nullptr};
            size_t rbs[4] = {0, 0, 0, 0};
            for (int i = 0; i < 4; ++i) {
                if (!mats[i]) continue;
                rbs[i] = mats[i]->row_bytes;
                if (rbs[i] < (size_t)eng_l2_rank(R2, i) * 2) { wrk_v7_engine_destroy(e); return no("a LoRA up-projection's rows are shorter than its rank"); }
                rows[i].resize((size_t)D * rbs[i]);
                if ((er = hipMemcpy(rows[i].data(), mats[i]->data, rows[i].size(), hipMemcpyDeviceToHost)) != hipSuccess) return fail_alloc(er);
                src[i] = rows[i].data();
            }
            eng_l2_pack_layer(R2, H, src, rbs, img.data());
            if ((er = hipMemcpy(e->l2pack + li * lb, img.data(), lb, hipMemcpyHostToDevice)) != hipSuccess) return fail_alloc(er);
        }
    }
    if ((er = hipMalloc((void**)&e->scal, hs.size() * 4)) != hipSuccess) return fail_alloc(er);
    if ((er = hipMemcpy(e->scal, hs.data(), hs.size() * 4, hipMemcpyHostToDevice)) != hipSuccess) return fail_alloc(er);
    if ((er = hipMalloc((void**)&e->layers, hl.size() * sizeof(EngLayer))) != hipSuccess) return fail_alloc(er);
    if ((er = hipMemcpy(e->layers, hl.data(), hl.size() * sizeof(EngLayer), hipMemcpyHostToDevice)) != hipSuccess) return fail_alloc(er);
    std::vector<uint32_t> hh(2 * NWG, ENG_NO_HEAD);
    for (uint32_t h = 0; h < H; ++h) hh[2 * ((size_t)h * NWG / H)] = h;
    for (uint32_t w = 0, r = 0; w < NWG; ++w)
        if (hh[2 * w] == ENG_NO_HEAD) hh[2 * w + 1] = r++;
    if ((er = hipMalloc((void**)&e->wg_head, hh.size() * 4)) != hipSuccess) return fail_alloc(er);
    if ((er = hipMemcpy(e->wg_head, hh.data(), hh.size() * 4, hipMemcpyHostToDevice)) != hipSuccess) return fail_alloc(er);
    if ((er = hipMalloc((void**)&e->gran, (size_t)S.g_total * 8)) != hipSuccess) return fail_alloc(er);
    if ((er = hipMalloc((void**)&e->fail, 256)) != hipSuccess) return fail_alloc(er);
    if ((er = hipMemset(e->fail, 0, 256)) != hipSuccess) return fail_alloc(er);
    const char* tm = getenv("WRK_TIMING");
    if (tm && tm[0] == '1') {
        const size_t n = (size_t)NWG * 16 * 24 * 8 + 64;
        if ((er = hipMalloc((void**)&e->stamps, n)) != hipSuccess) return fail_alloc(er);
        hipMemset(e->stamps, 0, n);
    }
    { const char* ev = getenv("WRK_ENGINE_WAVES"); e->ncw = (ev && atoi(ev) == 14) ? 14 : 8; }
    const void* fn = eng_kernel_fn(e->xd, e->r16, e->ncw);
    if ((er = hipFuncSetAttribute(fn, hipFuncAttributeMaxDynamicSharedMemorySize, (int)S.lds_total)) != hipSuccess) {
        wrk_v7_engine_destroy(e);
        return wrk_fail(ctx, WRK_E_UNSUPPORTED, "decode engine: %u bytes of LDS refused (%s)", S.lds_total, hipGetErrorString(er));
    }
    {
        hipFuncAttributes fa{};
        const int waves = e->ncw + 2, per_simd = (waves + 3) / 4;
        if (hipFuncGetAttributes(&fa, fn) == hipSuccess && fa.numRegs > 0) {
            const int alloc = (fa.numRegs + 7) / 8 * 8;
            if (per_simd * alloc > 512 || fa.maxThreadsPerBlock < waves * 64 || (size_t)fa.sharedSizeBytes + S.lds_total > 160 * 1024) {
                const int regs = fa.numRegs;
                wrk_v7_engine_destroy(e);
                return wrk_fail(ctx, WRK_E_UNSUPPORTED, "decode engine: a workgroup of %d waves x %d registers + %u bytes of LDS does not fit a CU", waves, regs,
                                S.lds_total);
            }
        }
        (void)hipGetLastError();
    }
    {
        const char* te = getenv("WRK_ENGINE_TABLE");
        if (!(te && te[0] == '0') && m->emb && m->ln0_w && m->ln0_b) {
            const size_t bytes = (size_t)d.num_vocab * D * 2;
            if (hipMalloc(&e->emb_ln, bytes) == hipSuccess) {
                LnMixParams P{};
                P.src = (const f16*)m->emb->ptr; P.ln_w = (const f16*)m->ln0_w->ptr; P.ln_b = (const f16*)m->ln0_b->ptr; P.eps = 1.0e-5f;
                P.d = D; P.nmix = 0; P.ln_out = (f16*)e->emb_ln;
                if (ln_mix(ctx->stream, P, d.num_vocab) != 0 || hipStreamSynchronize(ctx->stream) != hipSuccess) { hipFree(e->emb_ln); e->emb_ln = nullptr; }
            } else e->emb_ln = nullptr;
            (void)hipGetLastError();
        }
    }
    *out = e;
    return WRK_OK;
}

bool wrk_v7_engine_has_table(const wrk_v7_engine* e) { return e && e->emb_ln; }
int wrk_v7_engine_waves(const wrk_v7_engine* e) { return e ? e->ncw : 0; }

void wrk_v7_engine_destroy(wrk_v7_engine* e) {
    if (!e) return;
    if (e->emb_ln) hipFree(e->emb_ln);
    if (e->l2pack) hipFree(e->l2pack);
    if (e->layers) hipFree(e->layers);
    if (e->vecs) hipFree(e->vecs);
    if (e->scal) hipFree(e->scal);
    if (e->wg_head) hipFree(e->wg_head);
    if (e->gran) hipFree(e->gran);
    if (e->fail) hipFree(e->fail);
    if (e->stamps) hipFree(e->stamps);
    delete e;
}

int32_t wrk_v7_engine_enqueue(wrk_v7_engine* e, hipStream_t q, wrk_v7_state* st, uint32_t batch, uint32_t l0, uint32_t l1, const void* x_in, void* x_out,
                              void* v_first, const uint32_t* token) {
    using namespace wrk;
    wrk_ctx* ctx = e->m->ctx;
    EngArgs A{};
    A.S = e->S;
    A.S.layer_begin = l0; A.S.layer_end = l1; A.S.batch = batch;
    A.layers = e->layers; A.vecs = e->vecs; A.l2 = e->l2pack; A.scal = e->scal; A.gran = e->gran; A.x_in = x_in; A.x_out = x_out; A.v_first = v_first;
    if (token && e->emb_ln && l0 == 0) { A.x_in = e->emb_ln; A.x_row = token; }
    A.state = st->data; A.num_batch = st->num_batch; A.fail = e->fail; A.stamps = e->stamps; A.stamp_layer = std::min(5u, l1 - 1);
    WRK_HIP(ctx, hipMemsetAsync(e->gran, 0, (size_t)e->S.g_total * 8, q));
    const dim3 grid(e->S.nwg), block((e->ncw + 2) * 64);
    hipLaunchKernelGGL(eng_kernel(e->xd, e->r16, e->ncw), grid, block, e->S.lds_total, q, A, (const uint32_t*)e->wg_head);
    WRK_LAUNCH_CHECK(ctx);
    return WRK_OK;
}

int32_t wrk_v7_engine_check(wrk_v7_engine* e) {
    if (!e) return WRK_OK;
    wrk_ctx* ctx = e->m->ctx;
    uint32_t f = 0;
    WRK_HIP(ctx, hipMemcpy(&f, e->fail, 4, hipMemcpyDeviceToHost));
    if (f) {
        hipMemset(e->fail, 0, 4);
        return wrk_fail(ctx, WRK_E_HIP, "decode engine: a hand-off wait gave up (stage mask 0x%x): workgroups not co-resident or a producer died", f);
    }
    return WRK_OK;
}

void wrk_v7_engine_report(wrk_v7_engine* e) {
    using namespace wrk;
    if (!e || !e->stamps) return;
    const uint32_t NWG = e->S.nwg, NW = (uint32_t)e->ncw + 2;
    std::vector<unsigned long long> h((size_t)NWG * NW * 24);
    if (hipMemcpy(h.data(), e->stamps, h.size() * 8, hipMemcpyDeviceToHost) != hipSuccess) return;
    unsigned long long t0 = ~0ull;
    for (auto v : h) if (v && v < t0) t0 = v;
    std::vector<char> is_head(NWG, 0);
    for (uint32_t hd = 0; hd < e->S.H; ++hd) is_head[(size_t)hd * NWG / e->S.H] = 1;
    auto col = [&](int wave, uint32_t k, const char* label, int cls = -1) {
        std::vector<double> v;
        for (uint32_t w = 0; w < NWG; ++w) {
            if (cls >= 0 && is_head[w] != cls) continue;
            unsigned long long x = 0;
            if (wave >= 0) x = h[((size_t)w * NW + wave) * 24 + k];
            else for (int cw = 0; cw < e->ncw; ++cw) x = std::max(x, h[((size_t)w * NW + cw) * 24 + k]);
            if (x) v.push_back((double)(x - t0) * 0.01);
        }
        if (v.empty()) return;
        std::sort(v.begin(), v.end());
        fprintf(stderr, "  %-62s %4zu WGs  first %7.2f  median %7.2f  last %7.2f us\n", label, v.size(), v.front(), v[v.size() / 2], v.back());
    };
    {
        unsigned long long tail[2] = {0, 0};
        if (hipMemcpy(tail, e->stamps + (size_t)NWG * 16 * 24, 16, hipMemcpyDeviceToHost) == hipSuccess && tail[1])
            fprintf(stderr, "[WRK_TIMING] decode engine: shader clock over the last launch %.0f MHz (%llu cycles in %.1f us)\n",
                    (double)tail[0] / ((double)tail[1] * 0.01), tail[0], (double)tail[1] * 0.01);
    }
    const int G = e->ncw, Ld = e->ncw + 1;
    fprintf(stderr, "[WRK_TIMING] decode engine (%d compute waves), one layer of the last token; us since the layer's first stamp\n", e->ncw);
    col(G, 0, "gather: layer input complete, workgroups without a head", 0);
    col(G, 0, "gather: layer input complete, head workgroups", 1);
    col(-1, 19, "operand requests issued, slowest wave, head workgroups", 1);
    col(0, 1, "K1 start (input + weights in LDS), wave 0, no head", 0);
    col(0, 1, "K1 start (input in LDS), wave 0, head workgroups", 1);
    col(0, 2, "K1 LN + shift done, wave 0");
    col(0, 3, "K1 rows published, wave 0, no head", 0);
// ... 26 lines not shown
```

### web-rwkv-gguf_amd/csrc/wrk_v7_fused.hip

```cpp
#include "wrk_device.h"
#include "wrk_v7.h"
#include "wrk_v7_engine.h"
#include "wrk_lora_dev.h"

namespace wrk {

__global__ void advance_tokens_kernel(const uint32_t* __restrict__ argmax, uint32_t* __restrict__ tokens,
                                      uint32_t* __restrict__ history, uint32_t* __restrict__ counter, uint32_t b) {
    const uint32_t step = *counter;
    const uint32_t i = threadIdx.x;
    if (i < b) {
        const uint32_t t = argmax[i];
        tokens[i] = t;
        history[(size_t)step * b + i] = t;
    }
    __syncthreads();
    if (i == 0) *counter = step + 1;
}

void advance_tokens(hipStream_t s, const uint32_t* argmax, uint32_t* tokens, uint32_t* history, uint32_t* counter, uint32_t b) {
    advance_tokens_kernel<<<1, 256, 0, s>>>(argmax, tokens, history, counter, b);
}

template <int VPT, int NMIX>
// ... 283 lines not shown
                v = r16(wgsl_mix(v, vfirst, vv));
            }
            sh_v[row16] = v;
            sh_g[row16] = r16(dg);
        }
    }
    if (P.shift_src && tid < C) P.state[(size_t)batch * (S + 2) * D + cq + tid] = shift;
    WRK_STAMP(P.dbg, 1);
    __syncthreads();
    if (wave == 0) {
        const float kkv = sh_kk[lane];
        const float nrm = 1.0f / sqrtf(wave_sum(kkv * kkv) + P.l2_eps);
        const float kkn = r16(kkv * nrm);
        const float a = sh_a[lane];
        sh_a[lane] = -kkn;
        sh_b[lane] = kkn * a;
        const float xx = wave_sum(sh_rkr[lane]);
        if (lane == 0) sh_xx = xx;
    }
    __syncthreads();
    WRK_STAMP(P.dbg, 2);
    {
        const float aj = sh_a[lane], bj = sh_b[lane], wj = sh_w[lane], kj = sh_k[lane], rj = sh_r[lane];
        float sa[4], y[4];
#pragma unroll
        for (int c = 0; c < 4; ++c) sa[c] = wave_sum(Sv[c] * aj);
#pragma unroll
        for (int c = 0; c < 4; ++c) {
            const float s = Sv[c] * wj + kj * sh_v[4 * wave + c] + sa[c] * bj;
            Sv[c] = s;
            y[c] = rj * s;
        }
        *(f32x4*)st = Sv;
#pragma unroll
        for (int c = 0; c < 4; ++c) y[c] = wave_sum(y[c]);
        WRK_STAMP(P.dbg, 3);
        if (lane < 4) {
            const float yv = lane == 0 ? y[0] : (lane == 1 ? y[1] : (lane == 2 ? y[2] : y[3]));
            const uint32_t i = 4 * wave + lane;
            const size_t o = (size_t)t * D + cq + i;
            P.out[o] = (f16)yv;
            tt_out[o] = sh_xx * sh_v[i];
            g_out[o] = (f16)sh_g[i];
        }
    }
    WRK_STAMP(P.dbg, 4);
}

__global__ void __launch_bounds__(256) argmax_finish_kernel(const float* __restrict__ pv, const uint32_t* __restrict__ pi, uint32_t nwg,
                                                             uint32_t ntok, uint32_t* __restrict__ argmax, uint32_t* __restrict__ tokens,
                                                             uint32_t* __restrict__ history, uint32_t* __restrict__ counter) {
    __shared__ float sv[4];
    __shared__ uint32_t si[4];
    const uint32_t step = counter ? *counter : 0;
    for (uint32_t n = 0; n < ntok; ++n) {
        float bv = -3.0e38f;
        uint32_t bi = 0xffffffffu;
        for (uint32_t w = threadIdx.x; w < nwg; w += 256) {
            const float v = pv[(size_t)w * ntok + n];
            const uint32_t i2 = pi[(size_t)w * ntok + n];
            if (v > bv || (v == bv && i2 < bi)) { bv = v; bi = i2; }
        }
#pragma unroll
        for (int o = 32; o > 0; o >>= 1) {
            const float ov = __shfl_xor(bv, o, WAVE);
            const uint32_t oi = __shfl_xor(bi, o, WAVE);
            if (ov > bv || (ov == bv && oi < bi)) { bv = ov; bi = oi; }
        }
        __syncthreads();
        if ((threadIdx.x & 63) == 0) { sv[threadIdx.x >> 6] = bv; si[threadIdx.x >> 6] = bi; }
        __syncthreads();
        if (threadIdx.x == 0) {
            for (int k = 1; k < 4; ++k)
                if (sv[k] > bv || (sv[k] == bv && si[k] < bi)) { bv = sv[k]; bi = si[k]; }
            if (bi == 0xffffffffu) bi = 0;
            argmax[n] = bi;
            if (tokens) { tokens[n] = bi; history[(size_t)step * ntok + n] = bi; }
        }
    }
    if (counter && threadIdx.x == 0) *counter = step + 1;
}

void argmax_finish(hipStream_t s, const float* pv, const uint32_t* pi, uint32_t nwg, uint32_t ntok, uint32_t* argmax, uint32_t* tokens,
                   uint32_t* history, uint32_t* counter) {
    argmax_finish_kernel<<<1, 256, 0, s>>>(pv, pi, nwg, ntok, argmax, tokens, history, counter);
}

}

static constexpr uint32_t TIMED_LAYER = 5;
namespace {
struct TimingState {
    unsigned long long* dev = nullptr;
    std::vector<std::string> labels;
    bool enabled = false, init = false;
} g_timing;
}
unsigned long long* wrk::timing_slot(wrk_ctx* ctx, const char* label) {
    if (!g_timing.init) { const char* e = getenv("WRK_TIMING"); g_timing.enabled = e && e[0] == '1'; g_timing.init = true; }
    if (!g_timing.enabled) return nullptr;
    if (!g_timing.dev) {
        if (hipMalloc((void**)&g_timing.dev, 64 * 16 * 8) != hipSuccess) return nullptr;
        hipMemset(g_timing.dev, 0, 64 * 16 * 8);
    }
    if (!label) return nullptr;
    for (size_t i = 0; i < g_timing.labels.size(); ++i)
        if (g_timing.labels[i] == label) return g_timing.dev + i * 16;
    if (g_timing.labels.size() >= 64) return nullptr;
    g_timing.labels.push_back(label);
    return g_timing.dev + (g_timing.labels.size() - 1) * 16;
}
void wrk::timing_report(wrk_ctx* ctx) {
    if (!g_timing.enabled || !g_timing.dev || g_timing.labels.empty()) return;
    std::vector<unsigned long long> h(64 * 16);
    hipMemcpy(h.data(), g_timing.dev, h.size() * 8, hipMemcpyDeviceToHost);
    unsigned long long t0 = ~0ull;
    for (size_t i = 0; i < g_timing.labels.size() * 16; ++i) if (h[i] && h[i] < t0) t0 = h[i];
    fprintf(stderr, "[WRK_TIMING] layer %u of the last decode step; ns since the first stamp (100 MHz clock); first WG | last WG\n", TIMED_LAYER);
    for (size_t i = 0; i < g_timing.labels.size(); ++i) {
        fprintf(stderr, "  %-40s", g_timing.labels[i].c_str());
        for (int w = 0; w < 2; ++w) {
            for (int k = 0; k < 5; ++k) {
                const unsigned long long v = h[i * 16 + w * 8 + k];
                if (v) fprintf(stderr, " %6llu", (v - t0) * 10); else fprintf(stderr, "      -");
            }
            if (w == 0) fprintf(stderr, "  |");
        }
        fprintf(stderr, "\n");
    }
}

void wrk_v7_model::free_fused() {
    if (amax_val) hipFree(amax_val);
    if (amax_idx) hipFree(amax_idx);
    amax_val = nullptr; amax_idx = nullptr; amax_cap = 0;
}

int32_t wrk_v7_model::enqueue_fused_decode(wrk_v7_state* st, uint32_t T, uint32_t NH, bool identity_headers, bool from_tokens,
                                            bool want_argmax, bool advance, uint32_t cursor0_batch, bool contiguous) {
    using namespace wrk;
    hipStream_t q = ctx->op_stream();
    const uint32_t D = d.num_emb, F = d.num_hidden, H = d.num_head, S = D / H, V = d.num_vocab;
    bool ok = (D % 8 == 0) && D <= 8192 && d.lora_w % 8 == 0 && d.lora_a % 8 == 0 && d.lora_g % 8 == 0 && d.lora_v % 8 == 0 &&
              d.lora_w <= 128 && d.lora_a <= 128 && d.lora_v <= 128 && d.lora_g <= 512;
    for (auto& L : layers) {
        const wrk_matrix* ms[] = {L.w2, L.a2, L.g2, L.v2};
        for (const wrk_matrix* m : ms)
            if (m && m->kind != WRK_MAT_F16) ok = false;
    }
    if (!ok) {
        if (from_tokens) gather_rows_f16(q, emb->ptr, s.tokens, s.input, D, T);
        int32_t rc = enqueue_ops(st, T, NH, identity_headers);
        if (rc != WRK_OK) return rc;
        if (want_argmax && NH) {
            argmax_rows(q, s.head_o, V, V, NH, s.argmax);
            if (advance) advance_tokens(q, s.argmax, s.tokens, history.tokens, s.counter, NH);
        }
        return WRK_OK;
    }
    auto vec = [&](void* p, uint32_t c = 0) { return make_dense(p, WRK_F16, c ? c : D, T); };
    bool single = false;
    const KsScratch ks{s.ks_part, s.ks_cnt, s.ks_part_cap, s.ks_cnt_cap};
    const T3Scratch t3{ctx->gemm_scratch, ctx->gemm_scratch_cap};
    auto run_jobs = [&](MatJob* jobs, int n) -> int {
        if (single) return matvec_grouped(q, jobs, n, ctx->num_cu);
        return matmul_jobs(q, jobs, n, T, ctx->num_cu, &ks, &t3, FewTokens::matvec_grouped);
    };
#define LN(P, n)                                                                             \
    do {                                                                                     \
        if (ln_mix(q, P, n) != 0) return wrk_fail(ctx, WRK_E_UNSUPPORTED, "ln_mix shape");   \
    } while (0)

    if (T >= 2 && s.ks_cnt && s.ks_cnt_cap) WRK_HIP(ctx, hipMemsetAsync(s.ks_cnt, 0, (size_t)s.ks_cnt_cap * 4, q));
    const bool eng_embeds = T == 1 && from_tokens && !skip_embed && layer_begin == 0 && engine_on() && !engine_skip_once && wrk_v7_engine_has_table(engine) &&
                            d.num_layer > 0;
    if (!skip_embed && !eng_embeds) {
        LnMixParams P{};
        if (from_tokens) { P.src = (const f16*)emb->ptr; P.ids = s.tokens; }
        else P.src = (const f16*)s.input;
        P.ln_w = (const f16*)ln0_w->ptr; P.ln_b = (const f16*)ln0_b->ptr; P.eps = 1.0e-5f;
        P.d = D; P.nmix = 0; P.ln_out = (f16*)s.x;
        LN(P, T);
    }
    uint32_t first_launch_layer = layer_begin;
    if (T == 1 && engine_on() && !engine_skip_once) {
        const uint32_t l1 = std::min<uint32_t>(d.num_layer, layer_end);
        if (layer_begin < l1) {
            const int32_t rc = wrk_v7_engine_enqueue(engine, q, st, cursor0_batch, layer_begin, l1, s.x, s.x, s.att_v0, eng_embeds ? s.tokens : nullptr);
            if (rc != WRK_OK) return rc;
        }
        first_launch_layer = l1;
    }
    for (uint32_t li = first_launch_layer; li < d.num_layer && li < layer_end; ++li) {
        const wrk_v7_layer_desc& L = layers[li];
        float* lst = st->layer_ptr(li);
        static const bool fuse_ln = [] { const char* e = getenv("WRK_FUSE_LN"); return !(e && e[0] == '0'); }();
        static const uint32_t few_max = [] { const char* e = getenv("WRK_DMV_TOKENS"); const int v = e ? atoi(e) : 4; return (uint32_t)(v < 1 ? 1 : (v > 4 ? 4 : v)); }();
        single = fuse_ln && (T == 1 || (T <= few_max && contiguous)) && D <= 4096;
        if (single) {
            MatJob k1[7] = {mat_job(L.w_r, vec(s.x), vec(s.r), 0), mat_job(L.w_k, vec(s.x), vec(s.k), 0), mat_job(L.w_v, vec(s.x), vec(s.v), 0),
                            mat_job(L.w1, vec(s.x), vec(s.aux_w, d.lora_w), 0), mat_job(L.a1, vec(s.x), vec(s.aux_a, d.lora_a), 0),
                            mat_job(L.g1, vec(s.x), vec(s.aux_g, d.lora_g), 0), mat_job(li ? L.v1 : L.a1, vec(s.x), vec(s.aux_v, d.lora_v), 0)};
            for (MatJob& j : k1) j.pro = 1;
            MatJob k5 = mat_job(L.ffn_w_k, vec(s.x), vec(s.ffn_k, F), 0);
            k5.pro = 1;
            MatJob k6 = mat_job(L.ffn_w_v, vec(s.ffn_k, F), vec(s.x), 0);
            k6.has_res = 1; k6.res = vec(s.x);
            k6.carry_dst = (float*)s.x;
            single = matvec_grouped(q, k1, li ? 7 : 6, ctx->num_cu, true) == 0 && matvec(q, &k5, 1, ctx->num_cu, true) == 0 &&
                     matvec(q, &k6, 1, ctx->num_cu, true) == 0;
        }
        const bool want_split = split_head_env_on() && !(T == 1 && engine != nullptr && engine_env_on_public() && !engine_skip_once);
        const uint32_t state_stride = (S + 2) * D;
        bool split_head = want_split && single && d.lora_w >= 8 && d.lora_a >= 8 && d.lora_g >= 8 && d.lora_v >= 8 && d.lora_g <= 512;
        if (split_head) {
            MatJob k3 = mat_job(L.w_o, vec(s.att_x), vec(s.x), 0);
            k3.has_res = 1; k3.res = vec(s.x);
            k3.pro = 2; k3.ln_w = L.gn_w->ptr; k3.ln_b = L.gn_b->ptr; k3.mixw = s.g; k3.prev = (const float*)s.n;
            split_head = matvec(q, &k3, 1, ctx->num_cu, true) == 0;
        }
        uint32_t batch0 = 0;
        if (single) batch0 = cursor0_batch;
        float* row0 = lst + (size_t)batch0 * (S + 2) * D;
        if (!single) {
            LnMixParams P{};
            P.src = (const f16*)s.x; P.ln_w = (const f16*)L.ln1_w->ptr; P.ln_b = (const f16*)L.ln1_b->ptr; P.eps = 1.0e-5f;
            P.d = D; P.nmix = 6;
            const wrk_buf* mx[6] = {L.x_r, L.x_w, L.x_k, L.x_v, L.x_a, L.x_g};
            void* outs[6] = {s.rx, s.wx, s.kx, s.vx, s.ax, s.gx};
            for (int i = 0; i < 6; ++i) { P.mix[i] = (const f16*)mx[i]->ptr; P.out[i] = (f16*)outs[i]; }
            P.state_row = lst; P.state_stride = (size_t)(S + 2) * D; P.cursors = s.cursors; P.batch1 = contiguous ? cursor0_batch + 1 : 0;
            LN(P, T);
        }
        {
            MatJob jobs[7] = {mat_job(L.w_r, vec(s.rx), vec(s.r), WRK_ACT_NONE), mat_job(L.w_k, vec(s.kx), vec(s.k), WRK_ACT_NONE),
                              mat_job(L.w_v, vec(s.vx), vec(s.v), WRK_ACT_NONE),
                              mat_job(L.w1, vec(s.wx), vec(s.aux_w, d.lora_w), WRK_ACT_TANH),
                              mat_job(L.a1, vec(s.ax), vec(s.aux_a, d.lora_a), WRK_ACT_NONE),
                              mat_job(L.g1, vec(s.gx), vec(s.aux_g, d.lora_g), WRK_ACT_SIGMOID),
                              mat_job(li ? L.v1 : L.a1, vec(s.vx), vec(s.aux_v, d.lora_v), WRK_ACT_NONE)};
            if (single) {
                const wrk_buf* mx[7] = {L.x_r, L.x_k, L.x_v, L.x_w, L.x_a, L.x_g, L.x_v};
// ... 21 lines not shown
            P.aux_w = (const f16*)s.aux_w; P.aux_a = (const f16*)s.aux_a; P.aux_g = (const f16*)s.aux_g; P.aux_v = (const f16*)s.aux_v;
            P.r = (const f16*)s.r; P.k = (const f16*)s.k; P.v = (const f16*)s.v;
            P.v_first = (f16*)s.att_v0; P.out = (f16*)s.att_x;
            P.state = lst; P.cursors = s.cursors; P.gn_eps = 64.0e-5f; P.l2_eps = 1.0e-12f;
            P.shift_src = single ? (const f16*)s.ln_tmp : nullptr;
            P.batch1 = (single || contiguous) ? cursor0_batch + 1 : 0;
            P.dbg = li == TIMED_LAYER ? wrk::timing_slot(ctx, "K2 head: LoRA-2 + WKV7 + group norm") : nullptr;
            if (split_head) {
                if (d.lora_g <= 256) head_split_kernel<2><<<dim3(H * 4, T), 256, 0, q>>>(P, (float*)s.n, (f16*)s.g, H);
                else head_split_kernel<4><<<dim3(H * 4, T), 256, 0, q>>>(P, (float*)s.n, (f16*)s.g, H);
            }
            else if (d.lora_g <= 256) head_kernel<8><<<dim3(H, T), 256, 0, q>>>(P);
            else head_kernel<16><<<dim3(H, T), 256, 0, q>>>(P);
        }
        {
            MatJob j = mat_job(L.w_o, vec(s.att_x), vec(s.x), WRK_ACT_NONE);
            j.has_res = 1; j.res = vec(s.x);
            if (split_head) {
                j.pro = 2; j.pro_eps = 64.0e-5f; j.ln_w = L.gn_w->ptr; j.ln_b = L.gn_b->ptr; j.mixw = s.g; j.prev = (const float*)s.n;
                j.tok_mix_stride = D; j.tok_prev_stride = D;
            }
            if (li == TIMED_LAYER) j.dbg = wrk::timing_slot(ctx, "K3 w_o + residual");
            if (run_jobs(&j, 1) != 0) return wrk_fail(ctx, WRK_E_ARG, "fused K3 rejected");
        }
        float* rowf = lst + ((size_t)batch0 * (S + 2) + (S + 1)) * D;
        if (!single) {
            LnMixParams P{};
            P.src = (const f16*)s.x; P.ln_w = (const f16*)L.ln2_w->ptr; P.ln_b = (const f16*)L.ln2_b->ptr; P.eps = 1.0e-5f;
            P.d = D; P.nmix = 1; P.mix[0] = (const f16*)L.ffn_x_k->ptr; P.out[0] = (f16*)s.ffn_kx;
            P.state_row = lst + (size_t)(S + 1) * D; P.state_stride = (size_t)(S + 2) * D; P.cursors = s.cursors; P.batch1 = contiguous ? cursor0_batch + 1 : 0;
            LN(P, T);
        }
        {
            MatJob j = mat_job(L.ffn_w_k, vec(s.ffn_kx), vec(s.ffn_k, F), WRK_ACT_SQUARED_RELU);
            if (single) {
                j.in = vec(s.x);
                j.pro = 1; j.pro_eps = 1.0e-5f; j.ln_w = L.ln2_w->ptr; j.ln_b = L.ln2_b->ptr; j.mixw = L.ffn_x_k->ptr; j.prev = rowf;
                j.tok_prev_stride = state_stride;
                j.ln_out = s.ffn_x;
            }
            if (li == TIMED_LAYER) j.dbg = wrk::timing_slot(ctx, "K5 ffn key (LN2 prologue)");
            if (run_jobs(&j, 1) != 0) return wrk_fail(ctx, WRK_E_ARG, "fused K5 rejected");
        }
        {
            MatJob j = mat_job(L.ffn_w_v, vec(s.ffn_k, F), vec(s.x), WRK_ACT_NONE);
            j.has_res = 1; j.res = vec(s.x);
            if (single) { j.carry_src = s.ffn_x; j.carry_dst = rowf; j.tok_carry_src_stride = D; j.tok_carry_dst_stride = state_stride; }
            if (li == TIMED_LAYER) j.dbg = wrk::timing_slot(ctx, "K6 ffn value + residual");
            if (run_jobs(&j, 1) != 0) return wrk_fail(ctx, WRK_E_ARG, "fused K6 rejected");
        }
        if ((li + 1) % d.rescale == 0) wrk::affine(q, vec(s.x), 0.5f, 0.0f);
    }
    if (NH > 0) {
        LnMixParams P{};
        P.src = (const f16*)s.x; P.ids = identity_headers ? nullptr : s.headers;
        P.ln_w = (const f16*)ln_out_w->ptr; P.ln_b = (const f16*)ln_out_b->ptr; P.eps = 1.0e-5f;
        P.d = D; P.nmix = 0; P.ln_out = (f16*)s.head_x;
        LN(P, NH);
        MatJob j = mat_job(head, make_dense(s.head_x, WRK_F16, D, NH), make_dense(s.head_o, WRK_F32, V, NH), WRK_ACT_NONE);
        uint32_t nwg = 0;
        bool head_mv = NH < gemm_min_tokens();
        if (!head_mv && NH <= 4) {
            MatJob probe = j;
            if (want_argmax) { probe.amax_val = amax_val; probe.amax_idx = amax_idx; }
            head_mv = (size_t)matvec_num_wg(&j, 1, ctx->num_cu, nullptr) * NH <= amax_cap && matvec(q, &probe, 1, ctx->num_cu, true, false, true) == 0;
        }
        if (!head_mv && matmul_mfma(q, j, ctx->num_cu) == 0) {
            if (want_argmax) {
                wrk::argmax_rows(q, (const float*)s.head_o, V, V, NH, s.argmax);
                if (advance) wrk::advance_tokens(q, s.argmax, s.tokens, history.tokens, s.counter, NH);
            }
        } else {
            if (want_argmax) {
                nwg = matvec_num_wg(&j, 1, ctx->num_cu, nullptr);
                if ((size_t)nwg * NH > amax_cap) return wrk_fail(ctx, WRK_E_ARG, "arg-max scratch too small");
                j.amax_val = amax_val; j.amax_idx = amax_idx;
            }
            if (matvec(q, &j, 1, ctx->num_cu) != 0) return wrk_fail(ctx, WRK_E_ARG, "fused head rejected");
            if (want_argmax)
                argmax_finish(q, amax_val, amax_idx, nwg, NH, s.argmax, advance ? s.tokens : nullptr, history.tokens, advance ? s.counter : nullptr);
        }
    }
#undef LN
    WRK_LAUNCH_CHECK(ctx);
    return WRK_OK;
}
```

### web-rwkv-gguf_amd/wrk/__init__.py

```python
from __future__ import annotations

import ctypes as C
import os
from typing import Dict, List, Optional, Sequence

import numpy as np

_HERE = os.path.dirname(os.path.abspath(__file__))
_LIBDIR = os.environ.get("WRK_LIB_DIR") or os.path.join(os.path.dirname(_HERE), "lib")
LIB_HIP = os.path.join(_LIBDIR, "libwrk_hip.so")
LIB_RT = os.path.join(_LIBDIR, "libwrk_runtime.so")


class WrkError(RuntimeError):
    def __init__(self, code: int, msg: str):
        super().__init__(f"[{STATUS.get(code, code)}] {msg}")
        self.code = code


OK, E_ARG, E_OOM, E_HIP, E_UNSUPPORTED = 0, 1, 2, 3, 4
STATUS = {0: "WRK_OK", 1: "WRK_E_ARG", 2: "WRK_E_OOM", 3: "WRK_E_HIP", 4: "WRK_E_UNSUPPORTED"}
F16, F32, U8, U32 = 0, 1, 2, 3
ACT = {"none": 0, "squared_relu": 1, "tanh": 2, "stable_exp": 3, "opposite_exp": 4, "softplus": 5, "sigmoid": 6, "silu": 7}
MAT = {"F32": 0, "F16": 1, "Q8_0": 8, "Q4_K": 12, "Q5_K": 13, "Q6_K": 14, "INT8": 100, "NF4": 101}
# ... 112 lines not shown
    "wrk_ctx_create": (C.c_int32, [C.c_int32, C.POINTER(_P)]),
    "wrk_ctx_destroy": (C.c_int32, [_P]),
    "wrk_last_error": (C.c_char_p, [_P]),
    "wrk_ctx_sync": (C.c_int32, [_P]),
    "wrk_ctx_stream": (_P, [_P]),
    "wrk_buf_create": (C.c_int32, [_P, C.c_size_t, _P, C.POINTER(_P)]),
    "wrk_buf_retain": (C.c_int32, [_P]),
    "wrk_buf_release": (C.c_int32, [_P]),
    "wrk_buf_size": (C.c_size_t, [_P]),
    "wrk_buf_device_ptr": (_P, [_P]),
    "wrk_buf_write": (C.c_int32, [_P, _P, C.c_size_t, _P, C.c_size_t]),
    "wrk_buf_read": (C.c_int32, [_P, _P, C.c_size_t, _P, C.c_size_t]),
    "wrk_buf_copy": (C.c_int32, [_P, _P, C.c_size_t, _P, C.c_size_t, C.c_size_t]),
    "wrk_capture_begin": (C.c_int32, [_P]),
    "wrk_capture_end": (C.c_int32, [_P, C.POINTER(_P)]),
    "wrk_program_launch": (C.c_int32, [_P, _P]),
    "wrk_program_destroy": (C.c_int32, [_P]),
    "wrk_matrix_create": (C.c_int32, [_P, C.c_uint32, C.c_uint32, C.c_uint32, _P, C.c_size_t, C.c_uint32, C.POINTER(_P)]),
    "wrk_matrix_quantize": (C.c_int32, [_P, C.c_uint32, C.c_uint32, C.c_uint32, _P, C.POINTER(C.c_float), C.POINTER(_P)]),
    "wrk_matrix_export": (C.c_int32, [_P, _P, C.c_size_t, C.POINTER(C.c_size_t)]),
    "wrk_matrix_set_scale": (C.c_int32, [_P, C.c_float]),
    "wrk_matrix_release": (C.c_int32, [_P]),
    "wrk_matrix_stream_bytes": (C.c_size_t, [_P]),
    "wrk_op_matmul": (C.c_int32, [_P, _P, _TP, _TP, C.c_uint32, C.c_int32, C.c_int32]),
    "wrk_op_layer_norm": (C.c_int32, [_P, _P, _P, _TP, C.c_float]),
    "wrk_op_group_norm": (C.c_int32, [_P, _P, _P, _TP, C.c_float]),
    "wrk_op_l2_norm": (C.c_int32, [_P, _TP, C.c_float]),
    "wrk_op_token_shift": (C.c_int32, [_P, _P, _TP, _TP, _TP, _TP, C.c_int32]),
    "wrk_op_add": (C.c_int32, [_P, _TP, _TP, C.c_uint32, C.c_uint32, C.c_uint32]),
    "wrk_op_mul": (C.c_int32, [_P, _TP, _TP, C.c_uint32, C.c_uint32, C.c_uint32]),
    "wrk_op_lerp": (C.c_int32, [_P, _TP, _TP, _TP, C.c_int32]),
    "wrk_op_blit": (C.c_int32, [_P, _TP, _TP]),
    "wrk_op_affine": (C.c_int32, [_P, _TP, C.c_float, C.c_float]),
    "wrk_op_activate": (C.c_int32, [_P, _TP, C.c_uint32]),
    "wrk_op_control_k_v7": (C.c_int32, [_P, _P, _TP, _TP]),
    "wrk_op_time_mix_v7": (C.c_int32, [_P, _P, _TP, _TP, _TP, _TP, _TP]),
    "wrk_op_time_first_v7": (C.c_int32, [_P, _P, _TP, _TP, _TP]),
    "wrk_op_channel_mix_v7": (C.c_int32, [_P, _P, _TP, _TP, _TP]),
    "wrk_op_softmax": (C.c_int32, [_P, _TP]),
    "wrk_v7_model_create": (C.c_int32, [_P, _P, C.POINTER(_P)]),
    "wrk_v7_model_destroy": (C.c_int32, [_P]),
    "wrk_v7_model_token_bytes": (C.c_size_t, [_P, C.c_uint32]),
    "wrk_v7_state_create": (C.c_int32, [_P, _P, C.c_uint32, C.POINTER(_P)]),
    "wrk_v7_state_destroy": (C.c_int32, [_P]),
    "wrk_v7_state_load": (C.c_int32, [_P, _P, C.c_uint32, _f32p]),
    "wrk_v7_state_read": (C.c_int32, [_P, _P, C.c_uint32, _P]),
    "wrk_v7_state_write": (C.c_int32, [_P, _P, C.c_uint32, _P]),
    "wrk_v7_state_back": (C.c_int32, [_P, _P, C.c_uint32, _f32p]),
    "wrk_v7_infer": (C.c_int32, [_P, _P, _P, _u32p, C.POINTER(C.c_uint16), _u32p, C.c_uint32, _u32p, C.c_uint32, _f32p, _u32p, C.c_uint32]),
    "wrk_v7_model_set_frame_dtype": (C.c_int32, [_P, _P, C.c_uint32]),
    "wrk_v7_model_engine_status": (C.c_int32, [_P, _P, C.c_char_p, C.c_size_t]),
    "wrk_v7_infer_layer": (C.c_int32, [_P, _P, _P, C.c_uint32, _P, _P, _u32p, C.c_uint32, C.c_uint32]),
    "wrk_v7_frame_read": (C.c_int32, [_P, _P, C.c_char_p, C.c_uint32, _P, C.c_size_t, C.POINTER(C.c_size_t)]),
    "wrk_v7_generate_greedy": (C.c_int32, [_P, _P, _P, _u32p, C.c_uint32, C.c_uint32, _u32p, _f32p, _f32p, C.c_uint32]),
    "wrk_op_transpose": (C.c_int32, [_P, _TP, _TP]),
    "wrk_op_time_mix_v6": (C.c_int32, [_P, _P, _TP, _P, _TP, _TP, _TP, _TP, _TP]),
    "wrk_op_channel_mix": (C.c_int32, [_P, _P, _TP, _TP, _TP, _TP]),
    "wrk_v6_model_create": (C.c_int32, [_P, _P, C.POINTER(_P)]),
    "wrk_v6_model_destroy": (C.c_int32, [_P]),
    "wrk_v6_model_token_bytes": (C.c_size_t, [_P, C.c_uint32]),
    "wrk_v6_state_create": (C.c_int32, [_P, _P, C.c_uint32, C.POINTER(_P)]),
    "wrk_v6_infer": (C.c_int32, [_P, _P, _P, _u32p, C.POINTER(C.c_uint16), _u32p, C.c_uint32, _u32p, C.c_uint32, _f32p, _u32p, C.c_uint32]),
    "wrk_v6_generate_greedy": (C.c_int32, [_P, _P, _P, _u32p, C.c_uint32, C.c_uint32, _u32p, _f32p, _f32p, C.c_uint32]),
    "wrk_sample_logits": (C.c_int32, [_P, _P, C.c_uint32, C.c_uint32, C.c_uint32, _f32p, _f32p, _u32p, C.c_uint32, _u32p]),
    "wrk_sample_logits_filtered": (C.c_int32, [_P, _P, C.c_uint32, C.c_uint32, C.c_uint32, _f32p, _f32p, _u32p, _f32p, _u32p, C.c_uint32,
                                               _u32p]),
    "wrk_sample_logits_mirostat": (C.c_int32, [_P, _P, C.c_uint32, C.c_uint32, C.c_uint32, _f32p, _f32p, _f32p, _f32p, _f32p, _u32p, C.c_uint32,
                                               _u32p]),
    "wrk_sample_logits_typical": (C.c_int32, [_P, _P, C.c_uint32, C.c_uint32, C.c_uint32, _f32p, _f32p, _f32p, _u32p, C.c_uint32, _u32p]),
    "wrk_v7_generate_sample": (C.c_int32, [_P, _P, _P, _u32p, C.c_uint32, C.c_uint32, _f32p, _f32p, _u32p, _u32p, _f32p, _f32p,
                                           C.c_uint32]),
    "wrk_v6_generate_sample": (C.c_int32, [_P, _P, _P, _u32p, C.c_uint32, C.c_uint32, _f32p, _f32p, _u32p, _u32p, _f32p, _f32p,
                                           C.c_uint32]),
    "wrk_score_logits": (C.c_int32, [_P, _P, C.c_uint32, C.c_uint32, C.c_uint32, _u32p, _f32p, _u32p]),
    "wrk_top_logprobs": (C.c_int32, [_P, _P, C.c_uint32, C.c_uint32, C.c_uint32, _u32p, C.c_uint32, _f32p, _u32p, _f32p]),
    "wrk_v7_score": (C.c_int32, [_P, _P, _P, _u32p, C.POINTER(C.c_uint16), _u32p, C.c_uint32, _u32p, C.c_uint32, _u32p, _f32p, _u32p,
                                 C.c_uint32]),
    "wrk_v6_score": (C.c_int32, [_P, _P, _P, _u32p, C.POINTER(C.c_uint16), _u32p, C.c_uint32, _u32p, C.c_uint32, _u32p, _f32p, _u32p,
                                 C.c_uint32]),
    "wrk_occurrence_create": (C.c_int32, [_P, C.c_uint32, C.c_uint32, C.POINTER(_P)]),
    "wrk_occurrence_destroy": (C.c_int32, [_P]),
    "wrk_occurrence_set_weights": (C.c_int32, [_P, _P, _f32p]),
    "wrk_occurrence_ban": (C.c_int32, [_P, _P, C.c_uint32, _u32p, C.c_uint32, C.c_int32]),
    "wrk_occurrence_add": (C.c_int32, [_P, _P, C.c_uint32, _u32p, C.c_uint32, C.c_float]),
    "wrk_occurrence_back": (C.c_int32, [_P, _P, C.c_uint32, _f32p, _u32p]),
    "wrk_occurrence_load": (C.c_int32, [_P, _P, C.c_uint32, _f32p, _u32p]),
    "wrk_penalize_logits": (C.c_int32, [_P, _P, C.c_uint32, C.c_uint32, C.c_uint32, _P, C.c_uint32, _f32p, _f32p]),
    "wrk_v7_generate_penalized": (C.c_int32, [_P, _P, _P, _u32p, C.c_uint32, C.c_uint32, _f32p, _f32p, _u32p, _f32p, _f32p, _f32p, _P,
                                              _u32p, _f32p, _f32p, C.c_uint32]),
    "wrk_v6_generate_penalized": (C.c_int32, [_P, _P, _P, _u32p, C.c_uint32, C.c_uint32, _f32p, _f32p, _u32p, _f32p, _f32p, _f32p, _P,
                                              _u32p, _f32p, _f32p, C.c_uint32]),
    "wrk_grammar_create": (C.c_int32, [_P, C.c_uint32, C.c_uint32, C.c_uint32, _u16p, _u16p, C.POINTER(_P)]),
    "wrk_grammar_destroy": (C.c_int32, [_P]),
    "wrk_constrain_logits": (C.c_int32, [_P, _P, C.c_uint32, C.c_uint32, C.c_uint32, _P, _u32p]),
    "wrk_grammar_advance": (C.c_int32, [_P, _P, _u32p, _u32p, C.c_uint32]),
    "wrk_logit_bias_create": (C.c_int32, [_P, C.c_uint32, C.c_uint32, _u32p, _u32p, _f32p, C.POINTER(_P)]),
    "wrk_logit_bias_destroy": (C.c_int32, [_P]),
    "wrk_bias_logits": (C.c_int32, [_P, _P, C.c_uint32, C.c_uint32, C.c_uint32, _P, _u32p]),
    "wrk_token_window_create": (C.c_int32, [_P, C.c_uint32, C.c_uint32, C.c_uint32, C.POINTER(_P)]),
    "wrk_token_window_destroy": (C.c_int32, [_P]),
    "wrk_token_window_add": (C.c_int32, [_P, _P, C.c_uint32, _u32p, C.c_uint32]),
    "wrk_token_window_back": (C.c_int32, [_P, _P, C.c_uint32, _u32p, _u32p]),
    "wrk_token_window_load": (C.c_int32, [_P, _P, C.c_uint32, _u32p, C.c_uint32]),
    "wrk_dry_logits": (C.c_int32, [_P, _P, C.c_uint32, C.c_uint32, C.c_uint32, _P, C.c_uint32, _f32p, _f32p, _u32p, _u32p, _u32p, C.c_uint32]),
    "wrk_stop_sequences_advance": (C.c_int32, [_P, C.c_uint32, C.c_uint32, _u32p, _u32p, _u32p, _u32p, _u32p, _u32p, _u32p, _u32p]),
    "wrk_v7_generate_stop": (C.c_int32, [_P, _P, _P, _u32p, C.c_uint32, C.c_uint32, C.POINTER(GenerateOptions), _u32p, _u32p, _f32p, _u32p,
# ... 798 lines not shown

class Matrix:

    def __init__(self, ctx: Context, kind: str, k: int, m: int, data: np.ndarray, flags: int = MATRIX_EXACT):
        a = np.ascontiguousarray(data)
        h = _P()
        ctx.check(hip.wrk_matrix_create(ctx.h, MAT[kind], k, m, a.ctypes.data_as(_P), a.nbytes, flags, C.byref(h)))
        self.ctx, self.h, self.k, self.m, self.kind = ctx, h, k, m, kind

    @classmethod
    def _quant(cls, kind: str, matrix: "Buffer", k: int, m: int, levels=None) -> "Matrix":
        ctx = matrix.ctx
        h = _P()
        lv = None
        if levels is not None:
            lv = np.ascontiguousarray(levels, np.float32)
            assert lv.size == 16
            lv = lv.ctypes.data_as(C.POINTER(C.c_float))
        ctx.check(hip.wrk_matrix_quantize(ctx.h, MAT[kind], k, m, matrix.h, lv, C.byref(h)))
        self = cls.__new__(cls)
        self.ctx, self.h, self.k, self.m, self.kind = ctx, h, k, m, kind
        return self

    @classmethod
    def quant_u8(cls, matrix: "Buffer", k: int, m: int) -> "Matrix":
        return cls._quant("INT8", matrix, k, m)

    @classmethod
    def quant_nf4(cls, matrix: "Buffer", k: int, m: int) -> "Matrix":
        return cls._quant("NF4", matrix, k, m)

    @classmethod
    def quant_sf4(cls, matrix: "Buffer", k: int, m: int, levels) -> "Matrix":
        return cls._quant("NF4", matrix, k, m, levels)

    def export(self) -> np.ndarray:
        n = C.c_size_t()
        self.ctx.check(hip.wrk_matrix_export(self.h, None, 0, C.byref(n)))
        out = np.empty(n.value, np.uint8)
        self.ctx.check(hip.wrk_matrix_export(self.h, out.ctypes.data_as(_P), out.nbytes, C.byref(n)))
        return out

    def set_scale(self, scale: float):
        self.ctx.check(hip.wrk_matrix_set_scale(self.h, scale))

    @property
    def stream_bytes(self) -> int:
        return hip.wrk_matrix_stream_bytes(self.h)

    def matmul_op(self, inp: Tensor, out: Tensor, act: str = "none", turbo: bool = False, sparse: bool = False):
        di, do = inp.desc(), out.desc()
        self.ctx.check(hip.wrk_op_matmul(self.ctx.h, self.h, C.byref(di), C.byref(do), ACT[act], int(turbo), int(sparse)))

    def __del__(self):
        try:
            if self.h and self.ctx.h:
                hip.wrk_matrix_release(self.h)
        except Exception:
            pass
        self.h = None


class TensorOp:

    @staticmethod
    def _c(t: Tensor):
        return t.ctx

    @staticmethod
    def layer_norm(w: Buffer, b: Buffer, x: Tensor, eps: float):
        d = x.desc(); x.ctx.check(hip.wrk_op_layer_norm(x.ctx.h, w.h, b.h, C.byref(d), eps))

    @staticmethod
    def group_norm(w: Buffer, b: Buffer, x: Tensor, eps: float):
        d = x.desc(); x.ctx.check(hip.wrk_op_group_norm(x.ctx.h, w.h, b.h, C.byref(d), eps))

    @staticmethod
    def l2_norm(x: Tensor, eps: float):
        d = x.desc(); x.ctx.check(hip.wrk_op_l2_norm(x.ctx.h, C.byref(d), eps))

    @staticmethod
    def token_shift(cursors: Buffer, time_mix: Tensor, state: Tensor, inp: Tensor, out: Tensor, reversed_: bool):
        m, s, i, o = time_mix.desc(), state.desc(), inp.desc(), out.desc()
        inp.ctx.check(hip.wrk_op_token_shift(inp.ctx.h, cursors.h, C.byref(m), C.byref(s), C.byref(i), C.byref(o), int(reversed_)))

    @staticmethod
    def transpose(inp: Tensor, out: Tensor):
        i, o = inp.desc(), out.desc()
        out.ctx.check(hip.wrk_op_transpose(out.ctx.h, C.byref(i), C.byref(o)))

    @staticmethod
    def time_mix_v6(cursors: Buffer, time_decay: Tensor, time_first: Buffer, state: Tensor, k: Tensor, v: Tensor, r: Tensor, x: Tensor):
        dd, ds, dk, dv, dr, dx = time_decay.desc(), state.desc(), k.desc(), v.desc(), r.desc(), x.desc()
        x.ctx.check(hip.wrk_op_time_mix_v6(x.ctx.h, cursors.h, C.byref(dd), time_first.h, C.byref(ds), C.byref(dk), C.byref(dv), C.byref(dr), C.byref(dx)))

    @staticmethod
    def channel_mix(cursors: Buffer, state: Tensor, r: Tensor, v: Tensor, x: Tensor):
        ds, dr, dv, dx = state.desc(), r.desc(), v.desc(), x.desc()
        x.ctx.check(hip.wrk_op_channel_mix(x.ctx.h, cursors.h, C.byref(ds), C.byref(dr), C.byref(dv), C.byref(dx)))

    @staticmethod
    def add_activate(inp: Tensor, out: Tensor, act_x="none", act_y="none", act_out="none"):
        i, o = inp.desc(), out.desc()
        out.ctx.check(hip.wrk_op_add(out.ctx.h, C.byref(i), C.byref(o), ACT[act_x], ACT[act_y], ACT[act_out]))

    add = add_activate
# ... 639 lines not shown
```

Before: 1889 tokens/s.

## Fold engine granule zeroing into the head matvec tail for single-token decode

Adds a PRO==5 'tail' variant of the dense matvec kernel for the LM head. Its workgroups also zero the decode engine's granule buffer, so the separate memset that runs after the engine layers is no longer needed each step. A GranClean tracker and a HEAD_TAIL mask (read from the environment) decide whether the head, a memset, or nobody does the zeroing. It also adds a standalone wrk_op_head_tail API for testing. The cost is more template instantiations, plus extra stores inside the head kernel that compete with the weight stream.

```diff
diff --git a/include/wrk_hip.h b/include/wrk_hip.h
--- a/include/wrk_hip.h
+++ b/include/wrk_hip.h
@@ -166,6 +166,8 @@
 int32_t wrk_v7_infer_layer(wrk_ctx* ctx, wrk_v7_model* model, wrk_v7_state* state, uint32_t layer, const void* x, const void* v_first,
                            const uint32_t* cursors, uint32_t num_token, uint32_t mode);
 int32_t wrk_v7_frame_read(wrk_ctx* ctx, wrk_v7_model* model, const char* name, uint32_t num_token, void* dst, size_t capacity, size_t* bytes);
+int32_t wrk_op_head_tail(wrk_ctx* ctx, const wrk_matrix* mat, const wrk_buf* ln_w, const wrk_buf* ln_b, const wrk_buf* x, wrk_buf* head_x,
+                         wrk_buf* logits, wrk_buf* zero, uint32_t* picked);
 
 int32_t wrk_v7_generate_greedy(wrk_ctx* ctx, wrk_v7_model* model, wrk_v7_state* state,
                                const uint32_t* first_tokens, uint32_t num_batch, uint32_t steps,
diff --git a/web-rwkv-gguf_amd/csrc/wrk_device.h b/web-rwkv-gguf_amd/csrc/wrk_device.h
--- a/web-rwkv-gguf_amd/csrc/wrk_device.h
+++ b/web-rwkv-gguf_amd/csrc/wrk_device.h
@@ -82,6 +82,37 @@
     return t;
 }
 
+__device__ __forceinline__ void argmax_partials_finish(const float* pv, const uint32_t* pi, uint32_t nwg, uint32_t ntok, uint32_t* argmax,
+                                                       uint32_t* tokens, uint32_t* history, uint32_t* counter, float* sv, uint32_t* si) {
+    const uint32_t step = counter ? *counter : 0;
+    for (uint32_t n = 0; n < ntok; ++n) {
+        float bv = -3.0e38f;
+        uint32_t bi = 0xffffffffu;
+        for (uint32_t w = threadIdx.x; w < nwg; w += 256) {
+            const float v = pv[(size_t)w * ntok + n];
+            const uint32_t i2 = pi[(size_t)w * ntok + n];
+            if (v > bv || (v == bv && i2 < bi)) { bv = v; bi = i2; }
+        }
+#pragma unroll
+        for (int o = 32; o > 0; o >>= 1) {
+            const float ov = __shfl_xor(bv, o, WAVE);
+            const uint32_t oi = __shfl_xor(bi, o, WAVE);
+            if (ov > bv || (ov == bv && oi < bi)) { bv = ov; bi = oi; }
+        }
+        __syncthreads();
+        if ((threadIdx.x & 63) == 0) { sv[threadIdx.x >> 6] = bv; si[threadIdx.x >> 6] = bi; }
+        __syncthreads();
+        if (threadIdx.x == 0) {
+            for (int k = 1; k < 4; ++k)
+                if (sv[k] > bv || (sv[k] == bv && si[k] < bi)) { bv = sv[k]; bi = si[k]; }
+            if (bi == 0xffffffffu) bi = 0;
+            argmax[n] = bi;
+            if (tokens) { tokens[n] = bi; history[(size_t)step * ntok + n] = bi; }
+        }
+    }
+    if (counter && threadIdx.x == 0) *counter = step + 1;
+}
+
 #ifdef WRK_TIMING_BUILD
 #define WRK_STAMP(p, k)                                                                                       \
     do {                                                                                                      \
diff --git a/web-rwkv-gguf_amd/csrc/wrk_dmv.hip b/web-rwkv-gguf_amd/csrc/wrk_dmv.hip
--- a/web-rwkv-gguf_amd/csrc/wrk_dmv.hip
+++ b/web-rwkv-gguf_amd/csrc/wrk_dmv.hip
@@ -7,6 +7,10 @@
 template <int KA, int KB, int XI, int KS>
 static dmv_fn pick_dmv_pro(bool r16, int pro) {
 #define DMV_P(PRO_) (r16 ? (dmv_fn)dmv_kernel<KA, KB, true, XI, KS, PRO_, 1> : (dmv_fn)dmv_kernel<KA, KB, false, XI, KS, PRO_, 1>)
+    if (pro == 5) {
+        if constexpr (KA != KB || KS != 1) return nullptr;
+        else return DMV_P(5);
+    }
     if (KS == 4 || pro == 0) return DMV_P(0);
     if (pro == 1) return DMV_P(1);
     if (pro == 2) return DMV_P(2);
@@ -37,7 +41,7 @@
     return nullptr;
 }
 
-int launch_dmv(hipStream_t s, const MatvecParams& P, uint32_t total_wg, int quant, bool has_f16, bool r16, bool dry, int quant2) {
+int launch_dmv(hipStream_t s, const MatvecParams& P, uint32_t total_wg, int quant, bool has_f16, bool r16, bool dry, int quant2, const HeadTail* tail) {
     static const bool enabled = [] { const char* e = getenv("WRK_DMV"); return !(e && e[0] == '0'); }();
     if (!enabled) return -1;
     DParams D;
@@ -64,7 +68,7 @@
         if ((J.out.dtype != WRK_F16 && J.out.dtype != WRK_F32) || J.m == 0 || J.rows_per_wg == 0) return -1;
         const size_t ib = dense_base(J.in);
         if (ib & 7u) return -1;
-        const int jp = J.pro ? (J.k <= 2048 ? 1 : (J.k <= 4096 ? 2 : 9)) + (J.pro == 2 ? 2 : 0) : 0;
+        const int jp = J.pro ? (tail ? 9 : (J.k <= 2048 ? 1 : (J.k <= 4096 ? 2 : 9)) + (J.pro == 2 ? 2 : 0)) : (tail ? 5 : 0);
         if (jp >= 9 || (pro >= 0 && jp != pro)) return -1;
         if (J.pro == 2 && (J.k & 63u)) return -1;
         pro = jp;
@@ -104,6 +108,17 @@
         if (j > 0) bounds[j - 1] = J.wg_begin;
     }
     if (xi > 8) return -1;
+    if (pro == 5) {
+        if (nt != 1 || P.njobs != 1 || quant2 >= 0 || (has_f16 && quant >= 0) || !(xi <= 2 || (quant < 0 && xi <= 4))) return -1;
+        DJob& d = D.jobs[0];
+        memset(&D.tail, 0, sizeof D.tail);
+        D.tail.nwg = total_wg;
+        if (tail && tail->zero && tail->zero_bytes) {
+            if ((tail->zero_bytes & 15u) || ((uintptr_t)tail->zero & 15u) || (tail->zero_bytes >> 4) > 0xffffffffu) return -1;
+            d.flags |= DJ_ZERO;
+            D.tail.zero = (u32x4*)tail->zero; D.tail.zero_vec = (uint32_t)(tail->zero_bytes >> 4);
+        }
+    }
     static const size_t max_bytes = [] { const char* e = getenv("WRK_DMV_MAXMB"); return (size_t)(e ? atoi(e) : 24) << 20; }();
     size_t launch_bytes = 0;
     for (int j = 0; j < P.njobs; ++j) launch_bytes += (size_t)P.jobs[j].m * P.jobs[j].row_bytes;
diff --git a/web-rwkv-gguf_amd/csrc/wrk_dmv_body.h b/web-rwkv-gguf_amd/csrc/wrk_dmv_body.h
--- a/web-rwkv-gguf_amd/csrc/wrk_dmv_body.h
+++ b/web-rwkv-gguf_amd/csrc/wrk_dmv_body.h
@@ -3,7 +3,8 @@
 
 namespace wrk {
 
-enum { DJ_RES = 1, DJ_RES32 = 2, DJ_CARRY = 4, DJ_GATE = 8, DJ_AMAX = 16, DJ_OUT32 = 32, DJ_PUBLISH = 64 };
+enum { DJ_RES = 1, DJ_RES32 = 2, DJ_CARRY = 4, DJ_GATE = 8, DJ_AMAX = 16, DJ_OUT32 = 32, DJ_PUBLISH = 64,
+       DJ_ZERO = 128 };
 
 #define WRK_DJOB_FIELDS                                                                                                          \
     const uint8_t* w;                                                                                                            \
@@ -29,8 +30,13 @@
     uint32_t ntok, xs, os, rs, mix_s, prev_s, csrc_s, cdst_s, gate_s;
 };
 
+struct DTail {
+    u32x4* zero;
+    uint32_t zero_vec, nwg;
+};
 struct DParams {
     DJob jobs[MAX_JOBS];
+    DTail tail;
 };
 struct DParamsT {
     DJobT jobs[MAX_JOBS];
@@ -96,7 +102,7 @@
 }
 
 template <int KIND, bool R16, int XI, int KS, int PRO, int NT, class JT>
-__device__ __forceinline__ void dmv_body(const JT J, unsigned char* smem) {
+__device__ __forceinline__ void dmv_body(const JT J, const DTail TL, unsigned char* smem) {
     typedef TokF<JT> TF;
     constexpr int RB = 4;
     constexpr uint32_t CSTEP = KS == 1 ? 64u : 256u;
@@ -138,13 +144,19 @@
     const uint32_t fin_tok = tok_of(fin_t);
     const uint32_t fl = J.flags;
     uint32_t res_bits = 0, carry_bits = 0, gate_bits = 0;
-    constexpr int VPT = PRO == 0 ? 1 : ((PRO - 1) % 2 + 1);
-    constexpr bool GN = PRO >= 3;
+    constexpr int VPT = (PRO == 0 || PRO == 5) ? 1 : ((PRO - 1) % 2 + 1);
+    constexpr bool GN = PRO == 3 || PRO == 4;
+    constexpr bool TAIL = PRO == 5;
+    static_assert(!TAIL || (NT == 1 && KS == 1), "the head tail exists for one input vector and one wave per row");
+    if (TAIL && (fl & DJ_ZERO)) {
+        const u32x4 z = {0u, 0u, 0u, 0u};
+        for (uint32_t i = (blockIdx.x - J.wg_begin) * 256u + tid; i < TL.zero_vec; i += TL.nwg * 256u) TL.zero[i] = z;
+    }
     f16x8 xv[NT][VPT], wv[VPT], bv[VPT], mv[GN ? NT : 1][VPT];
     f32x4 pv[NT][VPT][2];
     f16 c0h[NT];
     XRegs x[NT][XI];
-    if (PRO > 0) {
+    if (PRO > 0 && !TAIL) {
         const uint32_t nvec = K >> 3;
 #pragma unroll
         for (int v = 0; v < VPT; ++v) {
@@ -217,7 +229,7 @@
 #pragma unroll
             for (int ci = 0; ci < XI; ++ci) x[t][ci] = load_x<KIND>(xs + (size_t)t * kpad, min(cbase + CSTEP * ci, nch - 1), true);
     }
-    if (PRO > 0 && !GN) {
+    if (PRO > 0 && !GN && !TAIL) {
         const uint32_t nvec = K >> 3;
         float s1[NT], s2[NT];
 #pragma unroll
@@ -355,8 +367,14 @@
     }
 }
 
+template <int PRO, class PT>
+__device__ __forceinline__ DTail dmv_tail(const PT& P) {
+    if constexpr (PRO == 5) return P.tail;
+    else return DTail{};
+}
+
 template <int PRO, int NT>
-constexpr unsigned dmv_smem_bytes() { return 576u * NT + (PRO > 0 ? (unsigned)((PRO - 1) % 2 + 1) * 4096u * NT : 16u); }
+constexpr unsigned dmv_smem_bytes() { return 576u * NT + ((PRO > 0 && PRO < 5) ? (unsigned)((PRO - 1) % 2 + 1) * 4096u * NT : 16u); }
 
 template <int KA, int KB, bool R16, int XI, int KS, int PRO, int NT>
 __global__ void __launch_bounds__(256) dmv_kernel(uint32_t b1, uint32_t b2, uint32_t b3, uint32_t b4, uint32_t b5, uint32_t b6, uint32_t b7,
@@ -365,8 +383,9 @@
     const uint32_t b = blockIdx.x;
     const uint32_t ji = (b >= b1) + (b >= b2) + (b >= b3) + (b >= b4) + (b >= b5) + (b >= b6) + (b >= b7);
     const auto J = P.jobs[ji];
-    if (KA == KB || !((kind_b_mask >> ji) & 1u)) dmv_body<KA, (KA != WRK_MAT_F16) && R16, XI, KS, PRO, NT>(J, smem);
-    else dmv_body<KB, (KB != WRK_MAT_F16) && R16, (KB == WRK_MAT_F16 ? 4 * XI : XI), 1, PRO, NT>(J, smem);
+    const DTail TL = dmv_tail<PRO>(P);
+    if (KA == KB || !((kind_b_mask >> ji) & 1u)) dmv_body<KA, (KA != WRK_MAT_F16) && R16, XI, KS, PRO, NT>(J, TL, smem);
+    else dmv_body<KB, (KB != WRK_MAT_F16) && R16, (KB == WRK_MAT_F16 ? 4 * XI : XI), 1, PRO, NT>(J, TL, smem);
 }
 
 template <int KA, bool R16, int XI, int PRO, int NT>
@@ -376,9 +395,9 @@
     const uint32_t b = blockIdx.x;
     const uint32_t ji = (b >= b1) + (b >= b2) + (b >= b3) + (b >= b4) + (b >= b5) + (b >= b6) + (b >= b7);
     const auto J = P.jobs[ji];
-    if (J.kind == (uint32_t)KA) dmv_body<KA, R16, XI, 1, PRO, NT>(J, smem);
-    else if (J.kind == WRK_MAT_Q6_K) dmv_body<WRK_MAT_Q6_K, R16, XI, 1, PRO, NT>(J, smem);
-    else dmv_body<WRK_MAT_F16, false, 4 * XI, 1, PRO, NT>(J, smem);
+    if (J.kind == (uint32_t)KA) dmv_body<KA, R16, XI, 1, PRO, NT>(J, DTail{}, smem);
+    else if (J.kind == WRK_MAT_Q6_K) dmv_body<WRK_MAT_Q6_K, R16, XI, 1, PRO, NT>(J, DTail{}, smem);
+    else dmv_body<WRK_MAT_F16, false, 4 * XI, 1, PRO, NT>(J, DTail{}, smem);
 }
 
 typedef void (*dmv_fn)(uint32_t, uint32_t, uint32_t, uint32_t, uint32_t, uint32_t, uint32_t, uint32_t, const DParams);
diff --git a/web-rwkv-gguf_amd/csrc/wrk_gran_clean.h b/web-rwkv-gguf_amd/csrc/wrk_gran_clean.h
--- /dev/null
+++ b/web-rwkv-gguf_amd/csrc/wrk_gran_clean.h
@@ -0,0 +1,37 @@
+#pragma once
+#include <stdint.h>
+
+namespace wrk {
+
+enum : uint32_t {
+    HEAD_TAIL_LN = 1,
+    HEAD_TAIL_ARGMAX = 2,
+    HEAD_TAIL_ZERO = 4,
+    HEAD_TAIL_ALL = 7
+};
+inline uint32_t head_tail_parse(const char* text) {
+    if (!text || !text[0]) return HEAD_TAIL_ALL;
+    uint32_t v = 0;
+    for (const char* p = text; *p >= '0' && *p <= '9'; ++p) v = v * 10u + (uint32_t)(*p - '0');
+    return v & HEAD_TAIL_ALL;
+}
+
+struct GranClean {
+    bool clean = false;
+    void created() { clean = true; }
+    bool engine_needs_leading_memset(uint32_t head_tail_mask) {
+        const bool need = !clean || !(head_tail_mask & HEAD_TAIL_ZERO);
+        clean = false;
+        return need;
+    }
+    void zeroed_behind() { clean = true; }
+};
+
+enum GranZeroBy { GRAN_ZERO_NOBODY, GRAN_ZERO_HEAD, GRAN_ZERO_MEMSET };
+inline GranZeroBy gran_after_engine(GranClean& g, uint32_t head_tail_mask, bool head_can_zero) {
+    if (!(head_tail_mask & HEAD_TAIL_ZERO)) return GRAN_ZERO_NOBODY;
+    g.zeroed_behind();
+    return head_can_zero ? GRAN_ZERO_HEAD : GRAN_ZERO_MEMSET;
+}
+
+}
diff --git a/web-rwkv-gguf_amd/csrc/wrk_matjob.h b/web-rwkv-gguf_amd/csrc/wrk_matjob.h
--- a/web-rwkv-gguf_amd/csrc/wrk_matjob.h
+++ b/web-rwkv-gguf_amd/csrc/wrk_matjob.h
@@ -14,6 +14,11 @@
 
 namespace wrk {
 
+struct HeadTail {
+    void* zero = nullptr;
+    size_t zero_bytes = 0;
+};
+
 struct MatJob {
     const uint8_t* w;
     const uint8_t* aux;
@@ -29,6 +34,7 @@
     float* amax_val = nullptr;
     uint32_t* amax_idx = nullptr;
     uint32_t pro = 0;
+    const HeadTail* tail = nullptr;
     float pro_eps = 0.0f;
     const void *ln_w = nullptr, *ln_b = nullptr, *mixw = nullptr;
     const float* prev = nullptr;
diff --git a/web-rwkv-gguf_amd/csrc/wrk_matvec.hip b/web-rwkv-gguf_amd/csrc/wrk_matvec.hip
--- a/web-rwkv-gguf_amd/csrc/wrk_matvec.hip
+++ b/web-rwkv-gguf_amd/csrc/wrk_matvec.hip
@@ -640,14 +640,15 @@
 }
 
 template <int NB>
-static int launch_matvec(hipStream_t s, const MatvecParams& P, uint32_t total_wg, uint32_t tok_groups, size_t smem, bool dry, bool no_catchall) {
+static int launch_matvec(hipStream_t s, const MatvecParams& P, uint32_t total_wg, uint32_t tok_groups, size_t smem, bool dry, bool no_catchall, const HeadTail* tail) {
     const KindMix c = classify_kinds(P);
     const int quant = c.quant, quant2 = c.quant2, nquant = c.nquant;
     const bool has_f16 = c.has_f16, r16 = c.r16, mixed_r16 = c.mixed_r16;
     matvec_fn fn = nullptr;
     bool needs_reg = false;
     for (int j = 0; j < P.njobs; ++j) needs_reg = needs_reg || P.jobs[j].pro || P.jobs[j].carry_dst || P.jobs[j].gate;
-    if (NB == 1 && tok_groups == 1 && nquant <= 2 && !mixed_r16 && launch_dmv(s, P, total_wg, nquant ? quant : -1, has_f16, r16, dry, nquant == 2 ? quant2 : -1) == 0) return 0;
+    if (NB == 1 && tok_groups == 1 && nquant <= 2 && !mixed_r16 && launch_dmv(s, P, total_wg, nquant ? quant : -1, has_f16, r16, dry, nquant == 2 ? quant2 : -1, tail) == 0) return 0;
+    if (tail) return -3;
     if (NB == 1 && tok_groups == 1 && nquant <= 2 && !mixed_r16) {
         fn = pick_reg(P, nquant ? quant : -1, has_f16, r16, nquant == 2 ? quant2 : -1);
         if (fn) {
@@ -699,8 +700,11 @@
     const uint32_t ntok = jobs[0].in.shape[1] * jobs[0].in.shape[2];
     if (ntok == 0) return 0;
     uint32_t kmax = 0;
+    const HeadTail* tail = jobs[0].tail;
+    if (tail && (njobs != 1 || ntok != 1)) return -3;
     for (int j = 0; j < njobs; ++j) {
         if (jobs[j].in.shape[1] * jobs[j].in.shape[2] != ntok) return -1;
+        if (j > 0 && jobs[j].tail) return -3;
         kmax = jobs[j].k > kmax ? jobs[j].k : kmax;
     }
     uint32_t rpw = 4;
@@ -723,7 +727,7 @@
     for (int j = 0; j < njobs; ++j) f32in = f32in || jobs[j].in.dtype == WRK_F32;
     if (f32in) {
         for (int j = 0; j < njobs; ++j)
-            if (jobs[j].pro || jobs[j].carry_dst || jobs[j].gate || jobs[j].amax_val) return -3;
+            if (jobs[j].pro || jobs[j].carry_dst || jobs[j].gate || jobs[j].amax_val || jobs[j].tail) return -3;
         if (dry_run) return 0;
         hipLaunchKernelGGL(matvec_f32in_kernel, dim3(wg, ntok), dim3(256), 0, s, P);
         return 0;
@@ -741,10 +745,10 @@
     const uint32_t groups = (ntok + nb - 1) / nb;
     int rc;
     switch (nb) {
-        case 8: rc = launch_matvec<8>(s, P, wg, groups, smem, dry_run, no_catchall); break;
-        case 4: rc = launch_matvec<4>(s, P, wg, groups, smem, dry_run, no_catchall); break;
-        case 2: rc = launch_matvec<2>(s, P, wg, groups, smem, dry_run, no_catchall); break;
-        default: rc = launch_matvec<1>(s, P, wg, groups, smem, dry_run, no_catchall); break;
+        case 8: rc = launch_matvec<8>(s, P, wg, groups, smem, dry_run, no_catchall, tail); break;
+        case 4: rc = launch_matvec<4>(s, P, wg, groups, smem, dry_run, no_catchall, tail); break;
+        case 2: rc = launch_matvec<2>(s, P, wg, groups, smem, dry_run, no_catchall, tail); break;
+        default: rc = launch_matvec<1>(s, P, wg, groups, smem, dry_run, no_catchall, tail); break;
     }
     return rc;
 }
diff --git a/web-rwkv-gguf_amd/csrc/wrk_matvec_dev.h b/web-rwkv-gguf_amd/csrc/wrk_matvec_dev.h
--- a/web-rwkv-gguf_amd/csrc/wrk_matvec_dev.h
+++ b/web-rwkv-gguf_amd/csrc/wrk_matvec_dev.h
@@ -350,6 +350,6 @@
 }
 
 
-int launch_dmv(hipStream_t s, const MatvecParams& P, uint32_t total_wg, int quant, bool has_f16, bool r16, bool dry, int quant2 = -1);
-
-}
+int launch_dmv(hipStream_t s, const MatvecParams& P, uint32_t total_wg, int quant, bool has_f16, bool r16, bool dry, int quant2 = -1, const HeadTail* tail = nullptr);
+
+}
diff --git a/web-rwkv-gguf_amd/csrc/wrk_v7.h b/web-rwkv-gguf_amd/csrc/wrk_v7.h
--- a/web-rwkv-gguf_amd/csrc/wrk_v7.h
+++ b/web-rwkv-gguf_amd/csrc/wrk_v7.h
@@ -53,3 +53,4 @@
 
 bool split_head_env_on();
 bool engine_env_on_public();
+uint32_t head_tail_mask();
diff --git a/web-rwkv-gguf_amd/csrc/wrk_v7.hip b/web-rwkv-gguf_amd/csrc/wrk_v7.hip
--- a/web-rwkv-gguf_amd/csrc/wrk_v7.hip
+++ b/web-rwkv-gguf_amd/csrc/wrk_v7.hip
@@ -555,7 +555,8 @@
         {"att_vx", s.vx, D}, {"att_ax", s.ax, D}, {"att_gx", s.gx, D}, {"att_r", s.r, D}, {"att_w", s.w, D}, {"att_k", s.k, D}, {"att_v", s.v, D},
         {"att_a", s.a, D}, {"att_g", s.g, D}, {"att_o", s.o, D}, {"att_kk", s.kk, D}, {"att_vv", s.vv, D}, {"att_n", s.n, 4 * D},
         {"aux_w", s.aux_w, m->d.lora_w}, {"aux_a", s.aux_a, m->d.lora_a}, {"aux_g", s.aux_g, m->d.lora_g}, {"aux_v", s.aux_v, m->d.lora_v},
-        {"ffn_x", s.ffn_x, D}, {"ffn_kx", s.ffn_kx, D}, {"ffn_k", s.ffn_k, F}, {"ffn_v", s.ffn_v, D}, {"att_x_ln", s.ln_tmp, D}};
+        {"ffn_x", s.ffn_x, D}, {"ffn_kx", s.ffn_kx, D}, {"ffn_k", s.ffn_k, F}, {"ffn_v", s.ffn_v, D}, {"att_x_ln", s.ln_tmp, D},
+        {"head_x", s.head_x, D}};
     const size_t esz = m->act_dtype == WRK_F32 ? 4 : 2;
     for (auto& e : tab)
         if (strcmp(e.n, name) == 0) {
@@ -592,7 +593,7 @@
 }
 
 uint32_t wrk_v7_model::key_bits(uint32_t B, uint32_t mode) const {
-    return mode | (act_dtype == WRK_F32 ? 4u : 0u) | ((B == 1 && mode == 1 && engine_on()) ? 8u : 0u) | (split_head_env_on() ? 0u : 16u);
+    return mode | (act_dtype == WRK_F32 ? 4u : 0u) | ((B == 1 && mode == 1 && engine_on()) ? 8u : 0u) | (split_head_env_on() ? 0u : 16u) ;
 }
 
 int32_t wrk_v7_model::lane(uint32_t g, uint32_t groups, wrk_frame_common** out) {
@@ -680,6 +681,10 @@
 
 static bool engine_env_on() { const char* e = getenv("WRK_ENGINE"); return !(e && e[0] == '0'); }
 bool engine_env_on_public() { return engine_env_on(); }
+uint32_t head_tail_mask() {
+    static const uint32_t mask = wrk::head_tail_parse(getenv("WRK_HEAD_TAIL"));
+    return mask;
+}
 bool wrk_v7_model::engine_on() const { return engine != nullptr && !engine_blocked && engine_env_on() && act_dtype == WRK_F16; }
 int32_t wrk_v7_model::ensure_engine() {
     if (engine_tried || !engine_env_on() || act_dtype != WRK_F16) return WRK_OK;
diff --git a/web-rwkv-gguf_amd/csrc/wrk_v7_engine.h b/web-rwkv-gguf_amd/csrc/wrk_v7_engine.h
--- a/web-rwkv-gguf_amd/csrc/wrk_v7_engine.h
+++ b/web-rwkv-gguf_amd/csrc/wrk_v7_engine.h
@@ -1,6 +1,7 @@
 #pragma once
 #include <stdint.h>
 
+#include "wrk_gran_clean.h"
 #include "wrk_internal.h"
 #include "wrk_lora2_pack.h"
 
@@ -104,7 +105,10 @@
 int32_t wrk_v7_engine_create(wrk_v7_model* m, wrk_v7_engine** out);
 void wrk_v7_engine_destroy(wrk_v7_engine* e);
 int32_t wrk_v7_engine_enqueue(wrk_v7_engine* e, hipStream_t q, wrk_v7_state* st, uint32_t batch, uint32_t l0, uint32_t l1, const void* x_in,
-                              void* x_out, void* v_first, const uint32_t* token = nullptr);
+                              void* x_out, void* v_first, const uint32_t* token = nullptr, uint32_t head_tail_mask = 0);
+void* wrk_v7_engine_granules(const wrk_v7_engine* e, size_t* bytes);
+wrk::GranClean& wrk_v7_engine_gran_clean(wrk_v7_engine* e);
+int32_t wrk_v7_engine_zero_behind(wrk_v7_engine* e, hipStream_t q);
 bool wrk_v7_engine_has_table(const wrk_v7_engine* e);
 int wrk_v7_engine_waves(const wrk_v7_engine* e);
 int32_t wrk_v7_engine_check(wrk_v7_engine* e);
diff --git a/web-rwkv-gguf_amd/csrc/wrk_v7_engine.hip b/web-rwkv-gguf_amd/csrc/wrk_v7_engine.hip
--- a/web-rwkv-gguf_amd/csrc/wrk_v7_engine.hip
+++ b/web-rwkv-gguf_amd/csrc/wrk_v7_engine.hip
@@ -815,6 +815,7 @@
     float* scal = nullptr;
     uint32_t* wg_head = nullptr;
     unsigned long long* gran = nullptr;
+    wrk::GranClean gran_clean;
     uint32_t* fail = nullptr;
     unsigned long long* stamps = nullptr;
     uint8_t* l2pack = nullptr;
@@ -1011,6 +1012,8 @@
     if ((er = hipMalloc((void**)&e->wg_head, hh.size() * 4)) != hipSuccess) return fail_alloc(er);
     if ((er = hipMemcpy(e->wg_head, hh.data(), hh.size() * 4, hipMemcpyHostToDevice)) != hipSuccess) return fail_alloc(er);
     if ((er = hipMalloc((void**)&e->gran, (size_t)S.g_total * 8)) != hipSuccess) return fail_alloc(er);
+    if ((er = hipMemset(e->gran, 0, (size_t)S.g_total * 8)) != hipSuccess) return fail_alloc(er);
+    e->gran_clean.created();
     if ((er = hipMalloc((void**)&e->fail, 256)) != hipSuccess) return fail_alloc(er);
     if ((er = hipMemset(e->fail, 0, 256)) != hipSuccess) return fail_alloc(er);
     const char* tm = getenv("WRK_TIMING");
@@ -1074,7 +1077,7 @@
 }
 
 int32_t wrk_v7_engine_enqueue(wrk_v7_engine* e, hipStream_t q, wrk_v7_state* st, uint32_t batch, uint32_t l0, uint32_t l1, const void* x_in, void* x_out,
-                              void* v_first, const uint32_t* token) {
+                              void* v_first, const uint32_t* token, uint32_t head_tail_mask) {
     using namespace wrk;
     wrk_ctx* ctx = e->m->ctx;
     EngArgs A{};
@@ -1083,10 +1086,20 @@
     A.layers = e->layers; A.vecs = e->vecs; A.l2 = e->l2pack; A.scal = e->scal; A.gran = e->gran; A.x_in = x_in; A.x_out = x_out; A.v_first = v_first;
     if (token && e->emb_ln && l0 == 0) { A.x_in = e->emb_ln; A.x_row = token; }
     A.state = st->data; A.num_batch = st->num_batch; A.fail = e->fail; A.stamps = e->stamps; A.stamp_layer = std::min(5u, l1 - 1);
-    WRK_HIP(ctx, hipMemsetAsync(e->gran, 0, (size_t)e->S.g_total * 8, q));
+    if (e->gran_clean.engine_needs_leading_memset(head_tail_mask)) WRK_HIP(ctx, hipMemsetAsync(e->gran, 0, (size_t)e->S.g_total * 8, q));
     const dim3 grid(e->S.nwg), block((e->ncw + 2) * 64);
     hipLaunchKernelGGL(eng_kernel(e->xd, e->r16, e->ncw), grid, block, e->S.lds_total, q, A, (const uint32_t*)e->wg_head);
     WRK_LAUNCH_CHECK(ctx);
+    return WRK_OK;
+}
+
+void* wrk_v7_engine_granules(const wrk_v7_engine* e, size_t* bytes) {
+    *bytes = (size_t)e->S.g_total * 8;
+    return e->gran;
+}
+wrk::GranClean& wrk_v7_engine_gran_clean(wrk_v7_engine* e) { return e->gran_clean; }
+int32_t wrk_v7_engine_zero_behind(wrk_v7_engine* e, hipStream_t q) {
+    WRK_HIP(e->m->ctx, hipMemsetAsync(e->gran, 0, (size_t)e->S.g_total * 8, q));
     return WRK_OK;
 }
 
diff --git a/web-rwkv-gguf_amd/csrc/wrk_v7_fused.hip b/web-rwkv-gguf_amd/csrc/wrk_v7_fused.hip
--- a/web-rwkv-gguf_amd/csrc/wrk_v7_fused.hip
+++ b/web-rwkv-gguf_amd/csrc/wrk_v7_fused.hip
@@ -359,33 +359,7 @@
                                                              uint32_t* __restrict__ history, uint32_t* __restrict__ counter) {
     __shared__ float sv[4];
     __shared__ uint32_t si[4];
-    const uint32_t step = counter ? *counter : 0;
-    for (uint32_t n = 0; n < ntok; ++n) {
-        float bv = -3.0e38f;
-        uint32_t bi = 0xffffffffu;
-        for (uint32_t w = threadIdx.x; w < nwg; w += 256) {
-            const float v = pv[(size_t)w * ntok + n];
-            const uint32_t i2 = pi[(size_t)w * ntok + n];
-            if (v > bv || (v == bv && i2 < bi)) { bv = v; bi = i2; }
-        }
-#pragma unroll
-        for (int o = 32; o > 0; o >>= 1) {
-            const float ov = __shfl_xor(bv, o, WAVE);
-            const uint32_t oi = __shfl_xor(bi, o, WAVE);
-            if (ov > bv || (ov == bv && oi < bi)) { bv = ov; bi = oi; }
-        }
-        __syncthreads();
-        if ((threadIdx.x & 63) == 0) { sv[threadIdx.x >> 6] = bv; si[threadIdx.x >> 6] = bi; }
-        __syncthreads();
-        if (threadIdx.x == 0) {
-            for (int k = 1; k < 4; ++k)
-                if (sv[k] > bv || (sv[k] == bv && si[k] < bi)) { bv = sv[k]; bi = si[k]; }
-            if (bi == 0xffffffffu) bi = 0;
-            argmax[n] = bi;
-            if (tokens) { tokens[n] = bi; history[(size_t)step * ntok + n] = bi; }
-        }
-    }
-    if (counter && threadIdx.x == 0) *counter = step + 1;
+    argmax_partials_finish(pv, pi, nwg, ntok, argmax, tokens, history, counter, sv, si);
 }
 
 void argmax_finish(hipStream_t s, const float* pv, const uint32_t* pi, uint32_t nwg, uint32_t ntok, uint32_t* argmax, uint32_t* tokens,
@@ -443,6 +417,64 @@
     amax_val = nullptr; amax_idx = nullptr; amax_cap = 0;
 }
 
+static bool head_tail_job(hipStream_t q, int num_cu, uint32_t ht, const wrk::MatJob& j, const wrk::HeadTail& want, wrk::MatJob& jt, wrk::HeadTail& tail) {
+    using namespace wrk;
+    jt = j;
+    tail = HeadTail{};
+    if ((ht & HEAD_TAIL_ZERO) && want.zero) { tail.zero = want.zero; tail.zero_bytes = want.zero_bytes; }
+    if (tail.zero) jt.tail = &tail;
+    if (jt.tail && matvec(q, &jt, 1, num_cu, true) == 0) return true;
+    jt = j;
+    tail = HeadTail{};
+    return false;
+}
+
+extern "C" int32_t wrk_op_head_tail(wrk_ctx* ctx, const wrk_matrix* mat, const wrk_buf* ln_w, const wrk_buf* ln_b, const wrk_buf* x, wrk_buf* head_x,
+                                    wrk_buf* logits, wrk_buf* zero, uint32_t* picked) {
+    using namespace wrk;
+    if (!ctx) return WRK_E_ARG;
+    std::lock_guard<std::recursive_mutex> lk(ctx->mu);
+    WRK_ARG(ctx, mat && ln_w && ln_b && x && head_x && logits && picked, "head_tail: null argument");
+    const uint32_t K = mat->k, M = mat->m;
+    WRK_ARG(ctx, (K & 7u) == 0 && K <= 8192 && ln_w->bytes >= (size_t)K * 2 && ln_b->bytes >= (size_t)K * 2 && x->bytes >= (size_t)K * 2 &&
+                     head_x->bytes >= (size_t)K * 2 && logits->bytes >= (size_t)M * 4, "head_tail: buffers too small for a %u x %u head", M, K);
+    WRK_ARG(ctx, !zero || (zero->bytes & 15u) == 0, "head_tail: the buffer to zero must be a multiple of 16 bytes");
+    WRK_ARG(ctx, !ctx->capturing_here(), "head_tail: not inside a capture");
+    WRK_HIP(ctx, hipSetDevice(ctx->device));
+    hipStream_t q = ctx->op_stream();
+    const MatJob j = mat_job(mat, make_dense(head_x->ptr, WRK_F16, K, 1), make_dense(logits->ptr, WRK_F32, M, 1), WRK_ACT_NONE);
+    const uint32_t nwg = matvec_num_wg(&j, 1, ctx->num_cu, nullptr);
+    uint32_t* scratch = nullptr;
+    WRK_HIP(ctx, hipMalloc((void**)&scratch, ((size_t)nwg * 2 + 2) * 4));
+    float* av = (float*)scratch;
+    uint32_t *ai = scratch + nwg, *rsv = scratch + 2 * (size_t)nwg, *am = rsv + 1;
+    int32_t rc = WRK_OK;
+    auto run = [&]() -> int32_t {
+        WRK_HIP(ctx, hipMemsetAsync(rsv, 0, 8, q));
+        HeadTail want{}, tail{};
+        if (zero) { want.zero = zero->ptr; want.zero_bytes = zero->bytes; }
+        MatJob jt, ja = j;
+        ja.amax_val = av; ja.amax_idx = ai;
+        head_tail_job(q, ctx->num_cu, head_tail_mask(), ja, want, jt, tail);
+        LnMixParams P{};
+        P.src = (const f16*)x->ptr; P.ln_w = (const f16*)ln_w->ptr; P.ln_b = (const f16*)ln_b->ptr; P.eps = 1.0e-5f;
+        P.d = K; P.nmix = 0; P.ln_out = (f16*)head_x->ptr;
+        if (ln_mix(q, P, 1) != 0) return wrk_fail(ctx, WRK_E_UNSUPPORTED, "head_tail: ln_mix shape");
+        if (matvec(q, &jt, 1, ctx->num_cu) != 0) return wrk_fail(ctx, WRK_E_ARG, "head_tail: head rejected");
+        argmax_finish(q, av, ai, nwg, 1, am, nullptr, nullptr, nullptr);
+        if (zero && !tail.zero) WRK_HIP(ctx, hipMemsetAsync(zero->ptr, 0, zero->bytes, q));
+        uint32_t back[2] = {0, 0};
+        WRK_HIP(ctx, hipMemcpyAsync(back, rsv, 8, hipMemcpyDeviceToHost, q));
+        WRK_HIP(ctx, hipStreamSynchronize(q));
+        picked[0] = back[1]; picked[1] = back[0];
+        return WRK_OK;
+    };
+    rc = run();
+    if (rc != WRK_OK) (void)hipStreamSynchronize(q);
+    (void)hipFree(scratch);
+    return rc;
+}
+
 int32_t wrk_v7_model::enqueue_fused_decode(wrk_v7_state* st, uint32_t T, uint32_t NH, bool identity_headers, bool from_tokens,
                                             bool want_argmax, bool advance, uint32_t cursor0_batch, bool contiguous) {
     using namespace wrk;
@@ -490,11 +522,37 @@
         LN(P, T);
     }
     uint32_t first_launch_layer = layer_begin;
-    if (T == 1 && engine_on() && !engine_skip_once) {
+    const bool engine_layers = T == 1 && engine_on() && !engine_skip_once;
+    const bool engine_runs = engine_layers && layer_begin < std::min<uint32_t>(d.num_layer, layer_end);
+    const uint32_t ht = head_tail_mask();
+    HeadTail tail{};
+    MatJob head_j{}, head_jt{};
+    bool head_mv = false;
+    if (NH > 0) {
+        head_j = mat_job(head, make_dense(s.head_x, WRK_F16, D, NH), make_dense(s.head_o, WRK_F32, V, NH), WRK_ACT_NONE);
+        head_jt = head_j;
+        head_mv = NH < gemm_min_tokens();
+        if (NH == 1 && identity_headers && head_mv) {
+            HeadTail want{};
+            if (engine_runs) want.zero = wrk_v7_engine_granules(engine, &want.zero_bytes);
+            MatJob ja = head_j;
+            if (want_argmax) { ja.amax_val = amax_val; ja.amax_idx = amax_idx; }
+            if (!head_tail_job(q, ctx->num_cu, ht, ja, want, head_jt, tail)) head_jt = head_j;
+            else { head_jt.amax_val = nullptr; head_jt.amax_idx = nullptr; }
+        }
+    }
+    struct ZeroGuard {
+        wrk_v7_engine* e; hipStream_t q; bool owes;
+        ~ZeroGuard() { if (owes) (void)wrk_v7_engine_zero_behind(e, q); }
+    } head_owes{engine, q, false};
+    if (engine_layers) {
         const uint32_t l1 = std::min<uint32_t>(d.num_layer, layer_end);
-        if (layer_begin < l1) {
-            const int32_t rc = wrk_v7_engine_enqueue(engine, q, st, cursor0_batch, layer_begin, l1, s.x, s.x, s.att_v0, eng_embeds ? s.tokens : nullptr);
+        if (engine_runs) {
+            int32_t rc = wrk_v7_engine_enqueue(engine, q, st, cursor0_batch, layer_begin, l1, s.x, s.x, s.att_v0, eng_embeds ? s.tokens : nullptr, ht);
             if (rc != WRK_OK) return rc;
+            const GranZeroBy by = gran_after_engine(wrk_v7_engine_gran_clean(engine), ht, tail.zero != nullptr);
+            if (by == GRAN_ZERO_MEMSET && (rc = wrk_v7_engine_zero_behind(engine, q)) != WRK_OK) return rc;
+            head_owes.owes = by == GRAN_ZERO_HEAD;
         }
         first_launch_layer = l1;
     }
@@ -622,14 +680,14 @@
         if ((li + 1) % d.rescale == 0) wrk::affine(q, vec(s.x), 0.5f, 0.0f);
     }
     if (NH > 0) {
+        const MatJob& j = head_j;
+        MatJob& jt = head_jt;
         LnMixParams P{};
         P.src = (const f16*)s.x; P.ids = identity_headers ? nullptr : s.headers;
         P.ln_w = (const f16*)ln_out_w->ptr; P.ln_b = (const f16*)ln_out_b->ptr; P.eps = 1.0e-5f;
         P.d = D; P.nmix = 0; P.ln_out = (f16*)s.head_x;
         LN(P, NH);
-        MatJob j = mat_job(head, make_dense(s.head_x, WRK_F16, D, NH), make_dense(s.head_o, WRK_F32, V, NH), WRK_ACT_NONE);
         uint32_t nwg = 0;
-        bool head_mv = NH < gemm_min_tokens();
         if (!head_mv && NH <= 4) {
             MatJob probe = j;
             if (want_argmax) { probe.amax_val = amax_val; probe.amax_idx = amax_idx; }
@@ -644,9 +702,10 @@
             if (want_argmax) {
                 nwg = matvec_num_wg(&j, 1, ctx->num_cu, nullptr);
                 if ((size_t)nwg * NH > amax_cap) return wrk_fail(ctx, WRK_E_ARG, "arg-max scratch too small");
-                j.amax_val = amax_val; j.amax_idx = amax_idx;
-            }
-            if (matvec(q, &j, 1, ctx->num_cu) != 0) return wrk_fail(ctx, WRK_E_ARG, "fused head rejected");
+                jt.amax_val = amax_val; jt.amax_idx = amax_idx;
+            }
+            if (matvec(q, &jt, 1, ctx->num_cu) != 0) return wrk_fail(ctx, WRK_E_ARG, "fused head rejected");
+            head_owes.owes = false;
             if (want_argmax)
                 argmax_finish(q, amax_val, amax_idx, nwg, NH, s.argmax, advance ? s.tokens : nullptr, history.tokens, advance ? s.counter : nullptr);
         }
diff --git a/web-rwkv-gguf_amd/wrk/__init__.py b/web-rwkv-gguf_amd/wrk/__init__.py
--- a/web-rwkv-gguf_amd/wrk/__init__.py
+++ b/web-rwkv-gguf_amd/wrk/__init__.py
@@ -188,6 +188,7 @@
     "wrk_v7_model_engine_status": (C.c_int32, [_P, _P, C.c_char_p, C.c_size_t]),
     "wrk_v7_infer_layer": (C.c_int32, [_P, _P, _P, C.c_uint32, _P, _P, _u32p, C.c_uint32, C.c_uint32]),
     "wrk_v7_frame_read": (C.c_int32, [_P, _P, C.c_char_p, C.c_uint32, _P, C.c_size_t, C.POINTER(C.c_size_t)]),
+    "wrk_op_head_tail": (C.c_int32, [_P, _P, _P, _P, _P, _P, _P, _P, C.POINTER(C.c_uint32)]),
     "wrk_v7_generate_greedy": (C.c_int32, [_P, _P, _P, _u32p, C.c_uint32, C.c_uint32, _u32p, _f32p, _f32p, C.c_uint32]),
     "wrk_op_transpose": (C.c_int32, [_P, _TP, _TP]),
     "wrk_op_time_mix_v6": (C.c_int32, [_P, _P, _TP, _P, _TP, _TP, _TP, _TP, _TP]),
@@ -1092,6 +1093,11 @@
         di, do = inp.desc(), out.desc()
         self.ctx.check(hip.wrk_op_matmul(self.ctx.h, self.h, C.byref(di), C.byref(do), ACT[act], int(turbo), int(sparse)))
 
+    def head_tail_op(self, ln_w: "Buffer", ln_b: "Buffer", x: "Buffer", head_x: "Buffer", logits: "Buffer", zero: "Buffer" = None):
+        picked = (C.c_uint32 * 2)()
+        self.ctx.check(hip.wrk_op_head_tail(self.ctx.h, self.h, ln_w.h, ln_b.h, x.h, head_x.h, logits.h, zero.h if zero is not None else None, picked))
+        return int(picked[0]), int(picked[1])
+
     def __del__(self):
         try:
             if self.h and self.ctx.h:
```

Result: slower. 1869 tokens/s (-1.1%).
